# facebookresearch/unbiased-teacher-v2

Hardware: AMD Instinct MI355X
Metric: images/sec/node (labeled+unlabeled) UTv2 step, R50-FPN 1333x800 (higher is better)
Workload: dtype f16

## Files before the change

### include/utv2.h

```cpp
#ifndef UTV2_H
#define UTV2_H
#include <stdint.h>
#ifdef __cplusplus
extern "C" {
#endif

typedef struct ihipStream_t* utv2_stream_t;

int utv2_conv2d_nhwc_fwd(const float* x, const float* w, float* y, const float* scale, const float* bias,
                         const float* residual, int N, int H, int W, int C, int K, int KH, int KW, int stride, int pad,
                         int in_dil, int OH, int OW, int relu, int accumulate, int Kred, utv2_stream_t stream);
int utv2_conv2d_stem_fwd(const float* x, const float* w, void* y, int y_dtype, const float* scale, const float* bias, int N,
                         int H, int W, int K, int KH, int KW, int stride, int pad, int OH, int OW, int relu, int Kred,
                         utv2_stream_t stream);
int utv2_conv2d_wgrad_splits(int N, int OH, int OW, int K, int Kred);
int64_t utv2_conv2d_wgrad_workspace_floats(int N, int OH, int OW, int K, int Kred);
int utv2_conv2d_nhwc_wgrad(const float* x, const float* dy, float* dw, float* ws, int N, int H, int W, int C, int K,
                           int KH, int KW, int stride, int pad, int OH, int OW, int accumulate, utv2_stream_t stream);
int utv2_colsum(const float* g, float* db, float* ws, int M, int C, int accumulate, utv2_stream_t stream);
int utv2_weight_flip_transpose(const float* w, float* wt, int K, int KH, int KW, int C, utv2_stream_t stream);

int utv2_conv2d_ml_fwd(const float* x, const float* w, float* y, const float* scale, const float* bias,
                       const float* residual, int nlev, const int* H_host, const int* W_host, int N, int C, int K, int KH,
                       int KW, int pad, int relu, int accumulate, utv2_stream_t stream);
int utv2_conv2d_ml_wgrad(const float* x, const float* dy, float* dw, float* ws, int nlev, const int* H_host,
                         const int* W_host, int N, int C, int K, int KH, int KW, int pad, int accumulate,
                         utv2_stream_t stream);

#define UTV2_F32 0
#define UTV2_BF16 1
int utv2_conv2d_bf16_supported(int C, int KH, int KW);

int utv2_conv_clock_probe(double* ghz, double* lifetime_us);
int utv2_conv2d_nhwc_fwd_bf16(const void* x, int x_dtype, const void* w16, void* y, int y_dtype, const float* scale,
                              const float* bias, const void* residual, const void* mask, const void* post_mask, int N, int H, int W, int C, int K,
                              int KH, int KW, int stride, int pad, int in_dil, int OH, int OW, int relu, int accumulate,
                              utv2_stream_t stream);
int utv2_conv2d_nhwc_fwd_bf16_ri(const void* x, int x_dtype, const void* w16, void* y, int y_dtype, const float* scale,
                                 const float* bias, const void* residual, const void* mask, const void* post_mask, int N, int H, int W, int C,
                                 int K, int KH, int KW, int stride, int pad, int in_dil, int OH, int OW, int relu, int accumulate,
                                 const int* rowinfo, utv2_stream_t stream);
int utv2_conv2d_nhwc_fwd_bf16_bits(const void* x, int x_dtype, const void* w16, void* y, int y_dtype, const float* scale,
                                   const float* bias, const void* residual, const void* mask, const void* post_mask, int N, int H, int W,
                                   int C, int K, int KH, int KW, int stride, int pad, int in_dil, int OH, int OW, int relu, int accumulate,
                                   const int* rowinfo, void* relu_bits, const void* mask_bits, const void* post_mask_bits,
                                   utv2_stream_t stream);
int utv2_conv2d_ml_fwd_bf16(const void* x, int x_dtype, const void* w16, void* y, int y_dtype, const float* scale,
                            const float* bias, const void* residual, int nlev, const int* H_host, const int* W_host, int N,
                            int C, int K, int KH, int KW, int pad, int relu, int accumulate, utv2_stream_t stream);
int utv2_conv2d_ml_fwd_bf16_g(const void* x, int x_dtype, int x_pitch, const void* w16, void* y, int y_dtype, int y_pitch,
                              const float* scale, const float* bias, const void* residual, int nlev, const int* H_host,
                              const int* W_host, int N, int C, int K, int KH, int KW, int pad, int relu, int accumulate, int groups,
                              float* gn_part, const int* rowinfo, utv2_stream_t stream);
int utv2_conv2d_ml_fwd_bf16_gnb(const void* x, int x_pitch, const void* w16, void* y, int nlev, const int* H_host, const int* W_host, int N,
                                int C, int K, int KH, int KW, int pad, int groups, const int* rowinfo, const void* mask_bits,
                                const void* gnb_x, float* gnb_part, utv2_stream_t stream);
int utv2_conv2d_wgrad_bf16_splits(int M, int K, int Kred);
int64_t utv2_conv2d_wgrad_bf16_workspace_floats(int M, int K, int Kred);
int utv2_conv2d_wgrad_bf16(const void* x, int x_dtype, const void* dy, int dy_dtype, float* dw, float* db, float* ws,
                           const int* rowinfo, const float* rowscale, int M, int C, int K, int KH, int KW, int accumulate,
                           utv2_stream_t stream);
int utv2_conv2d_wgrad_bf16_g(const void* x, int x_dtype, int x_pitch, const void* dy, int dy_dtype, int dy_pitch, float* dw, float* db,
                             float* ws, const int* rowinfo, const float* rowscale, int M, int C, int K, int KH, int KW, int accumulate,
                             int groups, utv2_stream_t stream);
int utv2_conv2d_wgrad_bf16_d(const void* x, int x_dtype, int x_pitch, const void* dy, int dy_dtype, int dy_pitch, float* dw, float* db,
                             float* ws, const int* rowinfo, const float* rowscale, int M, int C, int K, int KH, int KW, int accumulate,
                             int groups, void* pending, utv2_stream_t stream);
int64_t utv2_wgrad_fold_table_bytes(void);
int utv2_wgrad_fold_pending(const void* pending);
int utv2_wgrad_fold_flush(void* pending, utv2_stream_t stream);
int utv2_conv2d_stem_fwd_bf16(const void* xpad16, const void* w16s, void* y, int y_dtype, const float* scale,
                              const float* bias, int N, int H, int W, int K, int OH, int OW, int relu, utv2_stream_t stream);
int utv2_rowinfo_nhwc(int* out, int N, int H, int W, int OH, int OW, int stride, int pad, int KH, int KW, int64_t start,
                      utv2_stream_t stream);
int utv2_f32_to_bf16(const float* src, void* dst16, int64_t n, utv2_stream_t stream);
int utv2_weight_flip_transpose_bf16(const float* w, void* wt16, const float* scale, int K, int KH, int KW, int C,
                                    utv2_stream_t stream);
int utv2_pad_cols_bf16(const void* src, int src_dtype, void* dst16, int64_t rows, int c, int cpad, utv2_stream_t stream);
int utv2_weight_flip_transpose_bf16_batched(const float* arena, const float* scales, void* bank, const void* table, int nlayers,
                                            utv2_stream_t stream);

int utv2_ema_axpby(float* teacher, const float* student, int64_t n, double keep_rate, utv2_stream_t stream);
int utv2_sgd_momentum(float* param, float* grad, float* mom_buf, int64_t n, float lr, float momentum, float weight_decay,
                      float grad_scale, int zero_grad, utv2_stream_t stream);
int utv2_amp_found_inf(const float* grad, int64_t n, float* state, utv2_stream_t stream);
int utv2_sgd_momentum_amp(float* param, const float* grad, float* mom_buf, int64_t n, float lr, float momentum, float weight_decay,
                          float grad_scale, const float* state, utv2_stream_t stream);
int utv2_amp_update_scale(float* state, float growth_factor, float backoff_factor, int growth_interval, utv2_stream_t stream);
int utv2_ema_axpby_m16(float* teacher, const float* student, void* mirror16, int64_t n, double keep_rate, utv2_stream_t stream);
int utv2_sgd_momentum_m16(float* param, float* grad, float* mom_buf, void* mirror16, int64_t n, float lr, float momentum, float weight_decay,
                          float grad_scale, int zero_grad, utv2_stream_t stream);
int utv2_sgd_momentum_amp_m16(float* param, const float* grad, float* mom_buf, void* mirror16, int64_t n, float lr, float momentum,
                              float weight_decay, float grad_scale, const float* state, utv2_stream_t stream);

int utv2_relu_bwd_scale(const void* dy, const void* y, const float* scale, void* out, int64_t M, int C, int dtype,
                        utv2_stream_t stream);
int utv2_add(const float* a, const float* b, float* out, int64_t n, utv2_stream_t stream);
int utv2_maxpool3x3s2_nhwc(const void* x, int x_dtype, void* y, int y_dtype, int N, int H, int W, int C, int OH, int OW,
                           utv2_stream_t stream);
int utv2_maxpool3x3s2_bwd_nhwc(const void* x, int x_dtype, const void* dpool, void* dx, int g_dtype, int N, int H, int W, int C, int OH,
                               int OW, int relu, utv2_stream_t stream);
int utv2_upsample2x_add_nhwc(const void* lateral, const void* top, void* out, int N, int H, int W, int C, int dtype,
                             utv2_stream_t stream);
int utv2_downsample2x_sum_nhwc(const void* g, void* dtop, int N, int TH, int TW, int C, int accumulate, int dtype,
                               utv2_stream_t stream);
int utv2_zero_interleave2x_nhwc(const void* src, const void* mask, void* dst, int N, int H, int W, int C, int dtype, utv2_stream_t stream);
int utv2_zero_interleave2x_add_nhwc(const void* src, const void* mask, const void* mask_bits, const void* add, void* dst, int N, int H, int W,
                                    int C, utv2_stream_t stream);
int utv2_preprocess_image(const void* src, int is_u8, float* dst, int H, int W, int Hp, int Wp,
                          const float* mean3_host, const float* std3_host, utv2_stream_t stream);
int utv2_preprocess_image_bf16pad(const void* src, int is_u8, void* dst16, int H, int W, int Hp, int Wp,
                                  const float* mean3_host, const float* std3_host, utv2_stream_t stream);
int utv2_preprocess_images_bf16pad(const void* const* src_host, int is_u8, void* dst16, const int* H_host, const int* W_host, int N,
                                   int Hp, int Wp, const float* mean3_host, const float* std3_host, utv2_stream_t stream);
int utv2_frozenbn_fold(const float* w, const float* b, const float* mean, const float* var, float* scale, float* shift,
                       int n, float eps, utv2_stream_t stream);
int64_t utv2_groupnorm_seg_workspace_floats(int nseg, const int* seg_rows_host, int C);
int utv2_groupnorm_relu_seg_fwd(const void* x, const float* gamma, const float* beta, void* y, float* mean, float* rstd,
                                float* ws, int nseg, const int* seg_rows_host, int C, int G, float eps, int relu, int dtype,
                                utv2_stream_t stream);
int utv2_groupnorm_relu_seg_fwd_p32(const void* x, const float* gamma, const float* beta, void* y, float* mean, float* rstd,
                                    const float* part32, int nseg, const int* seg_rows_host, int C, int G, float eps, int relu,
                                    utv2_stream_t stream);
int utv2_groupnorm_relu_seg_fwd_p32b(const void* x, const float* gamma, const float* beta, void* y, float* mean, float* rstd,
                                     const float* part32, int nseg, const int* seg_rows_host, int C, int G, float eps, int relu,
                                     void* relu_bits, utv2_stream_t stream);
int utv2_groupnorm_relu_seg_bwd(const void* dy, const void* y, const void* x, const float* mean, const float* rstd,
                                const float* gamma, const float* beta, void* dx, float* dgamma, float* dbeta, float* ws,
                                int nseg, const int* seg_rows_host, int C, int G, int relu, int dtype, utv2_stream_t stream);
int64_t utv2_groupnorm_seg_chunks(int nseg, const int* seg_rows_host);
int utv2_groupnorm_relu_seg_bwd_colsum(const void* dy, const void* y, const void* x, const float* mean, const float* rstd,
                                       const float* gamma, const float* beta, void* dx, float* dgamma, float* dbeta, float* ws,
                                       int nseg, const int* seg_rows_host, int C, int G, int relu, int dtype, float* colsum_part,
                                       utv2_stream_t stream);
int utv2_groupnorm_seg_bwd_p64(const void* g, const void* x, const float* mean, const float* rstd, const float* gamma, void* dx,
                               float* dgamma, float* dbeta, float* ws, int nseg, const int* seg_rows_host, int C, int G,
                               const float* part64, float* colsum_part, utv2_stream_t stream);
int utv2_colsum_partials(const float* partial, float* db, int nb, int K, int accumulate, utv2_stream_t stream);
int64_t utv2_groupnorm_workspace_floats(int N, int HW, int C);
int utv2_groupnorm_relu_fwd(const float* x, const float* gamma, const float* beta, float* y, float* mean, float* rstd,
                            float* ws, int N, int HW, int C, int G, float eps, int relu, utv2_stream_t stream);
int utv2_groupnorm_relu_bwd(const float* dy, const float* y, const float* x, const float* mean, const float* rstd,
                            const float* gamma, float* dx, float* dgamma, float* dbeta, float* ws, int N, int HW, int C,
                            int G, int relu, utv2_stream_t stream);

int utv2_fcos_targets(int num_levels, const int* H_host, const int* W_host, const int* strides_host,
                      const float* soi_host, int N, int MAXG, const float* gt_boxes, const int* gt_classes,
                      const unsigned char* gt_valid, const float* gt_std, int num_classes, int drop_empty,
                      float center_radius, const unsigned char* img_active, int* labels, float* reg_targets, float* bvars,
                      int* gt_inds, utv2_stream_t stream);
int utv2_fcos_targets_range(int num_levels, const int* H_host, const int* W_host, const int* strides_host, const float* soi_host, int N,
                            int MAXG, const float* gt_boxes, const int* gt_classes, const unsigned char* gt_valid, const float* gt_std,
                            int gt_img0, int gt_imgs, int num_classes, int drop_empty, float center_radius,
                            const unsigned char* img_active, int* labels, float* reg_targets, float* bvars, int* gt_inds,
                            utv2_stream_t stream);
int utv2_sigmoid_focal_fwd(const float* logits, const int* labels, int64_t P, int C, float alpha, float gamma,
                           float* loss_sum, float* ws, utv2_stream_t stream);
int utv2_sigmoid_focal_bwd(const float* logits, const int* labels, int64_t P, int C, float alpha, float gamma,
                           const float* coef, float* dlogits, utv2_stream_t stream);
int utv2_fcos_loc_terms_fwd(const int* labels, const float* box, int box_stride, const float* reg_targets,
                            const float* bvars, int64_t P, int num_classes, int reg_max, float ts_better, float ts_cert,
                            int flags, float* sums, float* ws, utv2_stream_t stream);
int utv2_fcos_loc_terms_bwd(const int* labels, const float* box, int box_stride, const float* reg_targets,
                            const float* bvars, int64_t P, int num_classes, int reg_max, float ts_better, float ts_cert,
                            int flags, const float* coef, float* dbox, utv2_stream_t stream);
int utv2_sigmoid_focal_bwd_acc(const float* logits, const int* labels, int64_t P, int C, float alpha, float gamma, const float* coef,
                               const float* gscale, float* dlogits, int accumulate, utv2_stream_t stream);
int utv2_fcos_loc_terms_bwd_acc(const int* labels, const float* box, int box_stride, const float* reg_targets, const float* bvars,
                                int64_t P, int num_classes, int reg_max, float ts_better, float ts_cert, int flags, const float* coef8,
                                const float* gscale, float* dbox, int accumulate, utv2_stream_t stream);
int utv2_fcos_loss_combine(const float* focal_sup, const float* sums_sup, const float* focal_cls, const float* sums_cls,
                           const float* sums_reg, const float* norm, float world, int flags, float kl_weight, const float* wmul_host,
                           const float* wdiv_host, float* rec, float* coef, utv2_stream_t stream);
int utv2_fcos_rank_keys(const float* logits, const float* box, int box_stride, int reg_max, int N, int HW, int C,
                        float thr, int method, long long* keys, int64_t key_row_stride, utv2_stream_t stream);
int64_t utv2_topk_rows_workspace_bytes(int rows, int k);
int utv2_topk_rows_i64(const long long* keys, const long long* row_off, int rows, int64_t max_width, int k, long long* out,
                       void* ws, utv2_stream_t stream);
int utv2_fcos_decode(const long long* topkeys, int K, const float* logits, const float* box, int box_stride, int reg_max,
                     int N, int HW, int Wl, int C, int stride, int level, int method, int MAXC, int slot0, float* oboxes,
                     float* oscores, int* ocls, float* oloc, float* octr, float* oconf, float* ostd, int* olevel,
                     unsigned char* ovalid, utv2_stream_t stream);
int utv2_scale_cols(float* y, int64_t rows, int row_stride, int ncols, const float* s, utv2_stream_t stream);
int utv2_scale_cols_bwd(float* g, const float* ypost, int64_t rows, int row_stride, int ncols, const float* s, float* dsum,
                        float* ws, utv2_stream_t stream);
int utv2_scale_cols_ml(float* y, int nlev, const int64_t* row0_host, int row_stride, int ncols, const float* const* s_host,
                       utv2_stream_t stream);
int utv2_scale_cols_bwd_ml(float* g, const float* ypost, int nlev, const int64_t* row0_host, int row_stride, int ncols,
                           const float* const* s_host, float* const* sgrad_host, float* ws, utv2_stream_t stream);
int utv2_scale_cols_bwd_ml_pad16(const float* g, const float* ypost, int nlev, const int64_t* row0_host, int row_stride, int ncols,
                                 const float* const* s_host, float* const* sgrad_host, float* ws, void* out16, int cpad, utv2_stream_t stream);

int utv2_nms_mpad(int M);
int64_t utv2_nms_workspace_bytes(int N, int M);
int utv2_nms_batched(const float* boxes, const float* scores, const int* cls, const unsigned char* valid, int N, int M,
                     float iou_thr, int class_aware, int post_topk, int max_out, int* keep, int* keep_count, void* ws,
                     utv2_stream_t stream);
int utv2_box_iou(const float* a, const float* b, int A, int B, float* out, utv2_stream_t stream);

int utv2_match_boxes(const float* boxes, int64_t box_img_stride, int N, int P, const float* gt_boxes,
                     const unsigned char* gt_valid, int G, float* max_iou, int* arg, unsigned* gt_max_bits,
                     utv2_stream_t stream);
int utv2_match_lowq(const float* boxes, int64_t box_img_stride, int N, int P, const float* gt_boxes,
                    const unsigned char* gt_valid, int G, const unsigned* gt_max_bits, unsigned char* lowq,
                    utv2_stream_t stream);
int utv2_roi_align_fwd(int num_levels, int min_level, const void* const* feats_host, const int* H_host,
                       const int* W_host, const float* scales_host, const float* rois, const int* roi_batch,
                       const unsigned char* roi_valid, int R, int C, int PH, int PW, void* out, int dtype,
                       utv2_stream_t stream);
int utv2_roi_align_bwd(int num_levels, int min_level, float* const* dfeats_host, const int* H_host, const int* W_host,
                       const float* scales_host, const float* rois, const int* roi_batch, const unsigned char* roi_valid,
                       int R, int C, int PH, int PW, const void* dy, int dtype, utv2_stream_t stream);
int utv2_roi_align_bwd_tiled(int num_levels, int min_level, void* const* dfeats_host, const int* H_host, const int* W_host,
                             const float* scales_host, const float* rois, const unsigned char* roi_valid, int N, int rois_per_image,
                             int C, int PH, int PW, const void* dy, int dy_dtype, int out_dtype, utv2_stream_t stream);
int utv2_rpn_rank_keys(const float* head, int num_levels, const int* hw_host, int N, int A, int ch, int64_t* keys, utv2_stream_t stream);
int utv2_rpn_decode(const int64_t* top, int maxk, const float* head, const float* anchors, const float* image_hw, int num_levels,
                    const int* hw_host, const int* k_host, int N, int A, int ch, const float* weights_host, float scale_clamp,
                    float min_size, float* boxes, float* scores, int* lvls, unsigned char* keep, utv2_stream_t stream);
int utv2_nms_pack(const int* kidx, const int* cnt, const float* boxes, const float* scores, int N, int M, int D, float* oboxes, float* oscores,
                  unsigned char* ovalid, utv2_stream_t stream);
int utv2_roi_infer_keys(const float* probs, const float* deltas, const float* prop, const unsigned char* valid, const float* whwh, int N, int P,
                        int K, float wx, float wy, float scale_clamp, float thr, float* boxes, int64_t* keys, utv2_stream_t stream);
int utv2_roi_infer_gather(const int64_t* top, const float* boxes, int N, int P, int K, int k, float thr, float* sc, int64_t* rows, int* cls,
                          float* cb, unsigned char* valid, utv2_stream_t stream);
int utv2_roi_infer_pack(const int* kidx, const int* cnt, const float* cb, const float* sc, const int* cls, const int64_t* rows, const float* stdl,
                        int N, int P, int k, int D, float* oboxes, float* oscores, int* ocls, float* ostd, int64_t* orows, unsigned char* ovalid,
                        utv2_stream_t stream);
int utv2_rpn_loss_fwd(const float* obj, const float* deltas, int head, int num_levels, const int* hw_host, int N, int A, int ch, int R,
                      const float* anchors, const int64_t* pos_idx, const unsigned char* pos_valid, int npos, const int64_t* neg_idx,
                      const unsigned char* neg_valid, int nneg, const int* matched, const unsigned char* has_gt, const float* gt_boxes,
                      const float* gt_scores, int G, const float* weights_host, float* sums, float* gobj, float* gdl, utv2_stream_t stream);
int utv2_rpn_loss_bwd(const float* gobj, const float* gdl, const float* gout_cls, const float* gout_loc, int head, int num_levels,
                      const int* hw_host, int N, int A, int ch, int R, const int64_t* pos_idx, const unsigned char* pos_valid, int npos,
                      const int64_t* neg_idx, const unsigned char* neg_valid, int nneg, float* grad_obj, float* grad_deltas,
                      utv2_stream_t stream);
int utv2_rpn_loss_fwd_range(const float* obj, const float* deltas, int head, int num_levels, const int* hw_host, int N, int batch, int img0,
                            int A, int ch, int R, const float* anchors, const int64_t* pos_idx, const unsigned char* pos_valid, int npos,
                            const int64_t* neg_idx, const unsigned char* neg_valid, int nneg, const int* matched,
                            const unsigned char* has_gt, const float* gt_boxes, const float* gt_scores, int G, const float* weights_host,
                            float* sums, float* gobj, float* gdl, utv2_stream_t stream);
int utv2_rpn_loss_bwd_range(const float* gobj, const float* gdl, const float* gout_cls, const float* gout_loc, int head, int num_levels,
                            const int* hw_host, int N, int batch, int img0, int A, int ch, int R, const int64_t* pos_idx,
                            const unsigned char* pos_valid, int npos, const int64_t* neg_idx, const unsigned char* neg_valid, int nneg,
                            float* grad_obj, float* grad_deltas, utv2_stream_t stream);
int utv2_rpn_sample_keys(const float* max_iou, const unsigned char* lowq, const unsigned char* gt_valid, int G, const float* keys, int N,
                         int R, float lo, float hi, int64_t* out, utv2_stream_t stream);
int utv2_rpn_sample_unpack(const int64_t* top, int k, int N, int npos_max, int nneg_max, const unsigned char* gt_valid, int G,
                           int64_t* pos_idx, unsigned char* pos_valid, int64_t* neg_idx, unsigned char* neg_valid, unsigned char* has_gt,
                           utv2_stream_t stream);
int utv2_roi_sample(const float* boxes, const unsigned char* valid, const float* max_iou, const int* argmax, const float* keys, int N, int P,
                    const float* gt_boxes, const int* gt_classes, const unsigned char* gt_valid, const float* gt_scores, const float* gt_std,
                    int G, float iou_thr, int num_classes, int batch, int nfg_max, float* out_boxes, int64_t* out_classes,
                    float* out_gt_boxes, unsigned char* out_valid, int64_t* out_idx, float* out_conf, float* out_std, utv2_stream_t stream);
int utv2_roi_box_loss(const float* deltas, const float* stdl, int64_t ld, const int64_t* cls, const float* prop, const float* gtb,
                      const float* gstd, int R, int num_classes, int mode, float wx, float wy, float scale_clamp, float ts_better,
                      float t_cert, float* sum, float* gdeltas, float* gstd_out, utv2_stream_t stream);
int utv2_softmax_focal_fwd(const float* logits, const int* target, int R, int C, float gamma, float* loss_sum, float* ws,
                           utv2_stream_t stream);
int utv2_softmax_focal_bwd(const float* logits, const int* target, int R, int C, float gamma, const float* coef,
                           float* dlogits, utv2_stream_t stream);
int utv2_rcnn_loss_combine(const float* rpn_sup, const float* rpn_uns, const float* focal_sup, const float* focal_uns, const float* box_sup,
                           const float* box_uns, const int* tgt_sup, int n_sup, const int* tgt_uns, int n_uns, float rpn_norm_sup,
                           float rpn_norm_uns, float w_rpn_cls, float w_rpn_loc, float w_box, const float* wt_host, float* rec, float* coef,
                           utv2_stream_t stream);

int utv2_stem_pool_fwd_bf16(const void* xpad16, const void* w16s, void* y, const float* scale, const float* shift, int N, int H, int W,
                            int K, utv2_stream_t stream);

int utv2_bottleneck_supported(int C, int MID, int has_shortcut);
int utv2_bottleneck_fwd_bf16(const void* x, void* y, const void* w1, const void* w2, const void* w3, const void* wsc, const float* s1,
                             const float* b1, const float* s2, const float* b2, const float* s3, const float* b3, const float* ssc,
                             const float* bsc, int N, int H, int W, int C, int MID, utv2_stream_t stream);

// ... 38 lines not shown
```

### unbiased-teacher-v2_amd/csrc/conv_bf16.hip

```cpp
#include <mutex>
#include <stdlib.h>
#include "common.h"
#include <type_traits>

__device__ uint4 g_zero64[4] = {{0, 0, 0, 0}, {0, 0, 0, 0}, {0, 0, 0, 0}, {0, 0, 0, 0}};

#define CONV_MAX_LEVELS 8
struct LevelTab {
  int n;
  int start[CONV_MAX_LEVELS + 1];
  int H[CONV_MAX_LEVELS], W[CONV_MAX_LEVELS];
};

struct ConvArgs16 {
  LevelTab lt;
  const void* x;
  const h16_t* w;
  void* y;
  const float* scale;
  const float* bias;
  const void* residual;
  const void* mask;
  const void* post_mask;
  int N, H, W, C, OH, OW, K, KH, KW, stride, pad, in_dil, relu, Kred, M, accumulate;
  int xs;
  int m_begin;
  int groups;
  int ldy;
  float* gn_part;
  int ntiles;
  EpiBits bits;
  int mtot;
  const int2* rowinfo;
};

__device__ __forceinline__ void ml_decode16(const LevelTab& lt, int m, int& pixbase, int& H, int& W, int& oh, int& ow) {
  int l = 0;
#pragma unroll
  for (int i = 1; i < CONV_MAX_LEVELS; ++i)
    if (i < lt.n && m >= lt.start[i]) l = i;
  H = lt.H[l];
  W = lt.W[l];
  const int r = m - lt.start[l], hw = H * W;
  const int n = r / hw, rem = r - n * hw;
  oh = rem / W;
  ow = rem - oh * W;
  pixbase = lt.start[l] + n * hw;
}

#ifndef UTV2_MFMA_PRIO
#define UTV2_MFMA_PRIO 0
#endif
#if UTV2_MFMA_PRIO && defined(UTV2_MFMA_PRIO_LOOSE)
#define MFMA_BURST_BEGIN __builtin_amdgcn_s_setprio(UTV2_MFMA_PRIO)
#define MFMA_BURST_END __builtin_amdgcn_s_setprio(0)
#elif UTV2_MFMA_PRIO
#define MFMA_BURST_BEGIN __builtin_amdgcn_s_setprio(UTV2_MFMA_PRIO); __builtin_amdgcn_sched_barrier(0)
#define MFMA_BURST_END __builtin_amdgcn_sched_barrier(0); __builtin_amdgcn_s_setprio(0)
#else
#define MFMA_BURST_BEGIN
#define MFMA_BURST_END
#endif

template <int BN, bool ML, typename TI, typename TO>
__global__ __launch_bounds__(256) void conv_igemm_bf16(ConvArgs16 p) {
  constexpr bool IN16 = sizeof(TI) == 2;
  constexpr int BM = 128, BK = 32, LDB = 80;
  constexpr int TM = 2, TN = BN / 64, BROWS = BN / 64;
  __shared__ __attribute__((aligned(16))) unsigned char smem[2 * (BM + BN) * LDB];
  unsigned char* As = smem;
  unsigned char* Bs = smem + 2 * BM * LDB;

  const int tid = threadIdx.x, lane = tid & 63, wid = tid >> 6;
  const int wm = wid >> 1, wn = wid & 1;
  const int tilesN = (p.K + BN - 1) / BN;
  const int nwg = gridDim.x;
  int tile;
  {
    const int bid = blockIdx.x, xcd = bid & 7, q = nwg >> 3, r = nwg & 7;
    tile = (xcd < r ? xcd * (q + 1) : r * (q + 1) + (xcd - r) * q) + (bid >> 3);
  }
  const int mt = tile / tilesN, nt = tile - mt * tilesN;
  const int m0 = mt * BM, n0 = nt * BN;
  const int lrow = tid >> 2, kg = tid & 3;

  int ih0[2], iw0[2], Hr[2], Wr[2];
  long long pixbase[2];
  bool mvalid[2];
#pragma unroll
  for (int r = 0; r < 2; ++r) {
    const int m = m0 + lrow + 64 * r;
    mvalid[r] = m < p.M;
    const int mm = mvalid[r] ? m : 0;
    if constexpr (ML) {
      int pb, oh, ow;
      ml_decode16(p.lt, mm, pb, Hr[r], Wr[r], oh, ow);
      ih0[r] = oh - p.pad;
      iw0[r] = ow - p.pad;
      pixbase[r] = pb;
    } else {
      const int hw = p.OH * p.OW;
      const int n = mm / hw, rem = mm - n * hw;
      const int oh = rem / p.OW, ow = rem - oh * p.OW;
      ih0[r] = oh * p.stride - p.pad;
      iw0[r] = ow * p.stride - p.pad;
      pixbase[r] = (long long)n * p.H * p.W;
      Hr[r] = p.H;
      Wr[r] = p.W;
    }
  }
  bool bvalid[BROWS];
  const h16_t* wrow[BROWS];
#pragma unroll
  for (int r = 0; r < BROWS; ++r) {
    const int co = n0 + lrow + 64 * r;
    bvalid[r] = co < p.K;
// ... 172 lines not shown
    *(bf16x8_t*)(dst + r * cpad + j) = o;
  }
}

__global__ void weight_flip_transpose_bf16_kernel(const float* __restrict__ w, h16_t* __restrict__ wt, const float* __restrict__ scale,
                                                  int K, int KH, int KW, int C) {
  const size_t n = (size_t)K * KH * KW * C;
  size_t i = (size_t)blockIdx.x * blockDim.x + threadIdx.x;
  const size_t stride = (size_t)gridDim.x * blockDim.x;
  for (; i < n; i += stride) {
    size_t t = i;
    const int co = (int)(t % K); t /= K;
    const int kwp = (int)(t % KW); t /= KW;
    const int khp = (int)(t % KH); t /= KH;
    const int ci = (int)t;
    float v = w[(((size_t)co * KH + (KH - 1 - khp)) * KW + (KW - 1 - kwp)) * C + ci];
    if (scale) v *= scale[co];
    wt[i] = (h16_t)v;
  }
}

struct FlipDesc {
  long long w_off;
  long long dst_off;
  long long scale_off;
  int K, KH, KW, C;
  int Kpad;
  int reserved;
};

__global__ __launch_bounds__(256) void weight_flip_transpose_bf16_batched_kernel(const float* __restrict__ arena, const float* __restrict__ scales,
                                                                               h16_t* __restrict__ bank, const FlipDesc* __restrict__ table) {
  __shared__ float tile[32][33];
  const FlipDesc d = table[blockIdx.y];
  const float* w = arena + d.w_off;
  const float* scale = d.scale_off >= 0 ? scales + d.scale_off : nullptr;
  h16_t* wt = bank + d.dst_off;
  const int T = d.KH * d.KW, tk = (d.Kpad + 31) / 32, tc = (d.C + 31) / 32;
  const int ntiles = T * tk * tc;
  const int tx = threadIdx.x & 31, ty = threadIdx.x >> 5;
  for (int t = blockIdx.x; t < ntiles; t += gridDim.x) {
    const int tap = t / (tk * tc), r = t - tap * (tk * tc);
    const int co0 = (r / tc) * 32, ci0 = (r - (r / tc) * tc) * 32;
    const int kh = tap / d.KW, kw = tap - kh * d.KW;
    const int ftap = (d.KH - 1 - kh) * d.KW + (d.KW - 1 - kw);
#pragma unroll
    for (int i = 0; i < 4; ++i) {
      const int co = co0 + ty + 8 * i, ci = ci0 + tx;
      float v = 0.f;
      if (co < d.K && ci < d.C) {
        v = w[((size_t)co * T + tap) * d.C + ci];
        if (scale) v *= scale[co];
      }
      tile[ty + 8 * i][tx] = v;
    }
    __syncthreads();
#pragma unroll
    for (int i = 0; i < 4; ++i) {
      const int ci = ci0 + ty + 8 * i, co = co0 + tx;
      if (ci < d.C && co < d.Kpad) wt[((size_t)ci * T + ftap) * d.Kpad + co] = (h16_t)tile[tx][ty + 8 * i];
    }
    __syncthreads();
  }
}

static int fill_levels16(LevelTab& lt, int nlev, int N, const int* H, const int* W) {
  lt.n = nlev;
  int off = 0;
  for (int l = 0; l < CONV_MAX_LEVELS; ++l) {
    lt.start[l] = off;
    if (l < nlev) {
      lt.H[l] = H[l];
      lt.W[l] = W[l];
      off += N * H[l] * W[l];
    } else {
      lt.H[l] = lt.W[l] = 1;
    }
  }
  lt.start[CONV_MAX_LEVELS] = off;
  return off;
}


template <int BN, bool ML, int BK, typename TO, bool TALL = false, bool GNB = false>
__global__ __launch_bounds__(256, TALL ? 3 : ((BK == 32 && BN != 96) ? 4 : 2)) void conv_igemm_bf16_v2(ConvArgs16 p) {
  static_assert(!TALL || BN == 64, "the tall layout exists for the 64-wide tile");
  constexpr int WN = (BN == 96 || TALL) ? 1 : 2, WM = 4 / WN, WCOLS = BN / WN;
  constexpr int BM = WM * 64, ROWB = BK * 2;
  constexpr int SLOTS = BK / 8, RPP = 256 / SLOTS;
  constexpr int TM = 2, TN = WCOLS / 32, AP = BM / RPP, BP = (BN + RPP - 1) / RPP, KS = BK / 16;
  constexpr int ABUF = BM * ROWB, BBUF = BP * RPP * ROWB;
  constexpr int PCOLS = WCOLS > 64 ? 64 : WCOLS;
  constexpr int STAGE = 2 * (ABUF + BBUF), PATCH = 4 * 32 * (PCOLS + 4) * 4;
  __shared__ __attribute__((aligned(16))) unsigned char smem[STAGE > PATCH ? STAGE : PATCH];
  unsigned char* As = smem;
  unsigned char* Bs = smem + 2 * ABUF;

  const int tid = threadIdx.x, lane = tid & 63, wid = tid >> 6;
  const int wm = wid / WN, wn = wid % WN;
  const int tilesN = (p.K + BN - 1) / BN;
  const int nwg = gridDim.x;
  int tile;
  {
    const int bid = blockIdx.x, xcd = bid & 7, q = nwg >> 3, r = nwg & 7;
    tile = (xcd < r ? xcd * (q + 1) : r * (q + 1) + (xcd - r) * q) + (bid >> 3);
  }
  const int mt = tile / tilesN, nt = tile - mt * tilesN;
  const int m0 = p.m_begin + mt * BM, n0 = nt * BN;
  const int lrow = tid / SLOTS, slot = tid % SLOTS;
  const int ntaps = p.KH * p.KW;
  const int goff = p.groups > 1 ? (n0 / (p.K / p.groups)) * p.C : 0;

  int aoff[AP], awc[AP];
  unsigned amask[AP];
#pragma unroll
  for (int j = 0; j < AP; ++j) {
    const int m = m0 + lrow + RPP * j;
    const bool mv = m < p.M;
    const int mm = mv ? m : 0;
    int pb, H, W, ih0, iw0;
    if (p.rowinfo) {
      const int2 ri = p.rowinfo[mm];
      aoff[j] = ri.x * p.xs + slot * 8 + goff;
      awc[j] = (ri.y >> 16) * p.xs;
      amask[j] = mv ? (unsigned)(ri.y & 0xffff) : 0u;
      continue;
    }
    if constexpr (ML) {
      int oh, ow;
      ml_decode16(p.lt, mm, pb, H, W, oh, ow);
      ih0 = oh - p.pad;
      iw0 = ow - p.pad;
    } else {
      if (p.KH * p.KW == 1 && p.stride == 1 && p.pad == 0) {
        aoff[j] = mm * p.xs + slot * 8 + goff;
        awc[j] = 0;
        amask[j] = mv ? 1u : 0u;
        continue;
      }
      const int hw = p.OH * p.OW;
      const int n = mm / hw, rem = mm - n * hw;
      const int oh = rem / p.OW, ow = rem - oh * p.OW;
      ih0 = oh * p.stride - p.pad;
      iw0 = ow * p.stride - p.pad;
      pb = n * p.H * p.W;
      H = p.H;
      W = p.W;
    }
    aoff[j] = (pb + ih0 * W + iw0) * p.xs + slot * 8 + goff;
    awc[j] = W * p.xs;
    unsigned mk = 0;
    for (int kh = 0; kh < p.KH; ++kh)
      for (int kw = 0; kw < p.KW; ++kw)
        if (mv && (unsigned)(ih0 + kh) < (unsigned)H && (unsigned)(iw0 + kw) < (unsigned)W) mk |= 1u << (kh * p.KW + kw);
    amask[j] = mk;
  }
  int boff[BP];
  bool bvalid[BP];
#pragma unroll
  for (int j = 0; j < BP; ++j) {
    const int co = n0 + lrow + RPP * j;
    bvalid[j] = co < p.K && lrow + RPP * j < BN;
    boff[j] = (bvalid[j] ? co : 0) * p.Kred + slot * 8;
  }

  f32x16 acc[TM][TN];
#pragma unroll
  for (int i = 0; i < TM; ++i)
#pragma unroll
    for (int j = 0; j < TN; ++j)
#pragma unroll
      for (int e = 0; e < 16; ++e) acc[i][j][e] = 0.f;

  const h16_t* __restrict__ xb = (const h16_t*)p.x;
  const int nchunks = ntaps * (p.C / BK);
  int kh = 0, kw = 0, c0 = 0, tap = 0;
  bf16x8_t ra[AP], rb[BP];

  constexpr int NP = AP + BP;
  int ua = 0, ub = 0, ukh = 0, utap = 0;
  auto cursor_next = [&]() {
    ua = kw * p.xs + c0;
    ub = tap * p.C + c0;
    ukh = kh;
    utap = tap;
    ++tap;
    if (++kw == p.KW) {
      kw = 0;
      if (++kh == p.KH) { kh = 0; tap = 0; c0 += BK; }
    }
  };
  const h16_t* zero = (const h16_t*)g_zero64;
  auto load_piece = [&](int q) {
    if (q < AP) {
      const h16_t* src = ((amask[q] >> utap) & 1u) ? xb + (unsigned)(aoff[q] + ukh * awc[q] + ua) : zero;
      ra[q] = *(const bf16x8_t*)src;
    } else {
      const h16_t* src = bvalid[q - AP] ? p.w + (unsigned)(boff[q - AP] + ub) : zero;
      rb[q - AP] = *(const bf16x8_t*)src;
    }
  };
  auto swizzle = [](int row) { return BK == 64 ? (row >> 1) & 7 : (row >> 2) & 3; };
  const int wslot = (slot ^ swizzle(lrow)) * 16;
  auto store_piece = [&](int buf, int q) {
    if (q < AP) *(bf16x8_t*)(As + buf * ABUF + (lrow + RPP * q) * ROWB + wslot) = ra[q];
    else *(bf16x8_t*)(Bs + buf * BBUF + (lrow + RPP * (q - AP)) * ROWB + wslot) = rb[q - AP];
  };

  const int frow = lane & 31, fh = lane >> 5;
  const int swz = swizzle(frow);
  int koff[KS];
#pragma unroll
  for (int s = 0; s < KS; ++s) koff[s] = ((2 * s + fh) ^ swz) * 16;
  const int arow = (wm * 64 + frow) * ROWB, brow = (wn * WCOLS + frow) * ROWB;

  cursor_next();
#pragma unroll
  for (int q = 0; q < NP; ++q) load_piece(q);
#pragma unroll
  for (int q = 0; q < NP; ++q) store_piece(0, q);
  if (nchunks > 1) {
    cursor_next();
#pragma unroll
    for (int q = 0; q < NP; ++q) load_piece(q);
  }
  __syncthreads();
  auto iteration = [&](int buf, auto do_store, auto do_load) {
    constexpr bool STORE = decltype(do_store)::value, LOAD = decltype(do_load)::value;
    if constexpr (LOAD) cursor_next();
    const unsigned char* ab = As + buf * ABUF + arow;
    const unsigned char* bb = Bs + buf * BBUF + brow;
#pragma unroll
    for (int s = 0; s < KS; ++s) {
      bf16x8_t a[TM], b[TN];
#pragma unroll
      for (int i = 0; i < TM; ++i) a[i] = *(const bf16x8_t*)(ab + i * 32 * ROWB + koff[s]);
#pragma unroll
      for (int j = 0; j < TN; ++j) b[j] = *(const bf16x8_t*)(bb + j * 32 * ROWB + koff[s]);
      MFMA_BURST_BEGIN;
#pragma unroll
      for (int i = 0; i < TM; ++i)
#pragma unroll
        for (int j = 0; j < TN; ++j) acc[i][j] = mfma_32x32x16(b[j], a[i], acc[i][j]);
      MFMA_BURST_END;
#pragma unroll
      for (int q = s * NP / KS; q < (s + 1) * NP / KS; ++q) {
        if constexpr (STORE) store_piece(buf ^ 1, q);
        if constexpr (LOAD) load_piece(q);
      }
      __builtin_amdgcn_sched_barrier(0);
    }
    __syncthreads();
  };
  using yes = std::integral_constant<bool, true>;
  using no = std::integral_constant<bool, false>;
  int kc = 0;
  for (; kc + 2 < nchunks; ++kc) iteration(kc & 1, yes{}, yes{});
  if (kc + 1 < nchunks) { iteration(kc & 1, yes{}, no{}); ++kc; }
  iteration(kc & 1, no{}, no{});

  if ((p.K & 3) == 0) {
    static_assert(sizeof(smem) >= 4 * 32 * (PCOLS + 4) * sizeof(float), "epilogue patches must fit the staging LDS");
    float* patch = (float*)smem + wid * (32 * (PCOLS + 4));
    if constexpr (TN == 3) {
      f32x16 lo[2][2], hi[2][1];
#pragma unroll
      for (int i = 0; i < 2; ++i) { lo[i][0] = acc[i][0]; lo[i][1] = acc[i][1]; hi[i][0] = acc[i][2]; }
      epilogue_rows<2, TO, true, true>(lo, patch, lane, (TO*)p.y, p.scale, p.bias, (const TO*)p.residual, p.relu, p.accumulate, m0 + wm * 64, n0,
                                 p.M, p.K, (const TO*)p.mask, (const TO*)p.post_mask, p.ldy, nullptr, p.bits);
      if (n0 + 64 < p.K)
        epilogue_rows<1, TO, true, true>(hi, patch, lane, (TO*)p.y, p.scale, p.bias, (const TO*)p.residual, p.relu, p.accumulate, m0 + wm * 64,
                                   n0 + 64, p.M, p.K, (const TO*)p.mask, (const TO*)p.post_mask, p.ldy, nullptr, p.bits);
    } else {
      epilogue_rows<TN, TO, (BK != 32), true, GNB>(acc, patch, lane, (TO*)p.y, p.scale, p.bias, (const TO*)p.residual, p.relu, p.accumulate,
                            m0 + wm * 64, n0 + wn * WCOLS, p.M, p.K, (const TO*)p.mask, (const TO*)p.post_mask, p.ldy, p.gn_part, p.bits);
    }
    return;
  }
  TO* yo = (TO*)p.y;
  const TO* res = (const TO*)p.residual;
  const TO* msk = (const TO*)p.mask;
#pragma unroll
  for (int j = 0; j < TN; ++j) {
#pragma unroll
    for (int i = 0; i < TM; ++i) {
#pragma unroll
      for (int e = 0; e < 16; ++e) {
        const int co = n0 + wn * WCOLS + j * 32 + (e & 3) + 8 * (e >> 2) + 4 * fh;
        if (co >= p.K) continue;
        const float sc = p.scale ? p.scale[co] : 1.f;
        const float bi = p.bias ? p.bias[co] : 0.f;
        const int m = m0 + wm * 64 + i * 32 + frow;
        if (m >= p.M) continue;
        const size_t off = (size_t)m * p.ldy + co;
        float v = acc[i][j][e] * sc + bi;
        if (msk) v = (float)msk[off] > 0.f ? v : 0.f;
        if (res) v += (float)res[off];
        if (p.post_mask) v = (float)((const TO*)p.post_mask)[off] > 0.f ? v : 0.f;
        if (p.relu & 1) v = fmaxf(v, 0.f);
        if (p.accumulate) v += (float)yo[off];
        yo[off] = (TO)v;
      }
    }
  }
}

typedef __attribute__((address_space(1))) const void* gptr_t;
typedef __attribute__((address_space(3))) void* lptr_t;

#ifdef UTV2_PP_TRACE
__device__ unsigned g_pp_trace[8 * 128];
__device__ unsigned long long g_pp_phase[2][5];
#define PP_STAMP                                                                                         \
  if (blockIdx.x == 0 && c >= 8 && c < 16) {                                                             \
    const unsigned t_ = (unsigned)__builtin_amdgcn_s_memtime();                                          \
    asm volatile("ds_write_b32 %0, %1" : : "v"(tr_addr + 4 * tn), "v"(t_) : "memory");                   \
    ++tn;                                                                                                \
  }
#else
#define PP_STAMP
#endif
#if defined(UTV2_PP_TRACE) && defined(PP_NO_DMA)
#define PP_DMA(cond) false
#else
#define PP_DMA(cond) (cond)
#endif
__device__ __attribute__((aligned(16))) unsigned long long g_pp_clock[2];
template <bool ML, typename TO>
__global__ __launch_bounds__(512) void conv_igemm_bf16_pp(ConvArgs16 p) {
#ifdef UTV2_PP_TRACE
  const unsigned long long ph_entry = __builtin_amdgcn_s_memtime();
#endif
  const bool clk_on = ML && blockIdx.x == 0 && p.ntiles > 0;
  unsigned long long clk_c0 = 0, clk_r0 = 0;
  if (clk_on) { clk_c0 = __builtin_amdgcn_s_memtime(); clk_r0 = __builtin_amdgcn_s_memrealtime(); }
  constexpr int BM = 256, BN = 256, BK = 64, SEGB = 64;
  constexpr int OPSEG = 256 * SEGB, OPB = 2 * OPSEG, STAGE = 2 * OPB;
  constexpr int TM = 4, TN = 2;
  constexpr int PATCH = 8 * 32 * (TN * 32 + 4) * 4;
  static_assert(2 * STAGE >= PATCH, "epilogue patches must fit the staging LDS");
  extern __shared__ __attribute__((aligned(16))) unsigned char smem[];

// ... 594 lines not shown
  if (clk_on && threadIdx.x == 0) {
    typedef unsigned long long u64x2 __attribute__((ext_vector_type(2)));
    const u64x2 v = {__builtin_amdgcn_s_memtime() - clk_c0, __builtin_amdgcn_s_memrealtime() - clk_r0};
    *(u64x2*)g_pp_clock = v;
  }
}

static bool env_flag_on(const char* name) {
  const char* v = getenv(name);
  return !(v && v[0] == '0');
}
static const bool g_use_w8 = env_flag_on("UTV2_W8");
static const bool g_use_wgrad_w8 = env_flag_on("UTV2_WGRAD_W8");
static int env_int(const char* name, int dflt) {
  const char* v = getenv(name);
  return v ? atoi(v) : dflt;
}
static const int g_epi_general = env_int("UTV2_EPI_PLAIN", 1) ? 0 : 2;
static const int g_use_pp = env_int("UTV2_PP", 2) == 1 ? 1 : 2;

template <int BN, bool ML>
static void launch_igemm16(const ConvArgs16& a, int tiles, int x_dtype, int y_dtype, hipStream_t stream) {
  const dim3 g(tiles), b(256);
  const int64_t xelems = ML ? (int64_t)a.M * a.xs : (int64_t)a.N * a.H * a.W * a.xs;
  if (x_dtype == UTV2_BF16 && a.C % 32 == 0 && a.in_dil == 1 && a.KH * a.KW <= 16 && xelems < (1ll << 31) &&
      (int64_t)a.K * a.Kred < (1ll << 31)) {
    const bool tail = tiles > 512 && tiles <= 768;
    const bool deep = a.C % 64 == 0 && a.Kred >= 1024 && (!tail || a.bits.gnb_part);
    static const bool use_rs = env_int("UTV2_PP_RS", 1) != 0;
    const bool rs_ok = use_rs && a.rowinfo && a.KH == 3 && a.KW == 3 && a.stride == 1 && a.pad == 1 && (ML || (a.OH == a.H && a.OW == a.W));
    const bool gnb = ML && BN == 128 && a.bits.gnb_part != nullptr;
    const bool w8 = g_use_w8 && (!gnb || rs_ok);
    if (w8 && BN == 128 && a.xs >= a.groups * a.C && (a.xs & 7) == 0 && a.C % 64 == 0 && a.Kred >= 1024 && a.K >= 256 && (a.K & 3) == 0 &&
        a.m_begin == 0 && (a.groups == 1 || (a.K / a.groups) % 256 == 0)) {
      const int tilesN = cdiv(a.K, 256), tiles_m = a.M / 256, tiles_all = cdiv(a.M, 256) * tilesN;
      int main_tiles = (tiles_m * tilesN / 256) * 256;
      if (tiles_all - main_tiles > 128) main_tiles = tiles_all;
      const int main_m = main_tiles == tiles_all ? cdiv(a.M, 256) : main_tiles / tilesN;
      if (main_m > 0) {
        ConvArgs16 m = a;
        m.M = main_tiles == tiles_all ? a.M : main_m * 256;
        const int smem = 2 * (256 + 256) * 128;
        static LdsOptIn lds_opt_in;
        lds_opt_in({(const void*)conv_igemm_bf16_pp<ML, h16_t>, (const void*)conv_igemm_bf16_pp<ML, float>}, smem);
        {
          int grid = main_m * tilesN;
          static const int pp_wgs = [] { int v = env_int("UTV2_PP_WGS", 256); return v < 8 ? 8 : (v > 256 ? 256 : v / 8 * 8); }();
          if (g_use_pp == 2 && grid > 256) { m.ntiles = grid; grid = pp_wgs; }
          if (rs_ok) {
            const int smem_rs = 4 * 272 * 64 + 4 * 256 * 64 + 256;
            static LdsOptIn rs_opt_in;
            rs_opt_in({(const void*)conv_igemm_bf16_rs<ML, h16_t>, (const void*)conv_igemm_bf16_rs<ML, float>,
                       (const void*)conv_igemm_bf16_rs<ML, h16_t, ML>}, smem_rs);
            m.mtot = a.M;
            if (gnb) hipLaunchKernelGGL((conv_igemm_bf16_rs<ML, h16_t, ML>), dim3(grid), dim3(512), smem_rs, stream, m);
            else if (y_dtype == UTV2_BF16) hipLaunchKernelGGL((conv_igemm_bf16_rs<ML, h16_t>), dim3(grid), dim3(512), smem_rs, stream, m);
            else hipLaunchKernelGGL((conv_igemm_bf16_rs<ML, float>), dim3(grid), dim3(512), smem_rs, stream, m);
          } else if (y_dtype == UTV2_BF16) hipLaunchKernelGGL((conv_igemm_bf16_pp<ML, h16_t>), dim3(grid), dim3(512), smem, stream, m);
          else hipLaunchKernelGGL((conv_igemm_bf16_pp<ML, float>), dim3(grid), dim3(512), smem, stream, m);
        }
        if (m.M == a.M) return;
        ConvArgs16 r = a;
        r.m_begin = m.M;
        launch_igemm16<BN, ML>(r, cdiv(a.M - m.M, 128) * cdiv(a.K, 128), x_dtype, y_dtype, stream);
        return;
      }
    }
    if constexpr (BN == 64) {
      static const bool use_tall = env_int("UTV2_CONV_TALL64", 1) != 0;
      if (use_tall && a.KH * a.KW > 1 && a.M - a.m_begin >= 65536 && a.K > 32) {
        const dim3 gt(cdiv(a.M - a.m_begin, 256) * cdiv(a.K, 64));
        if (y_dtype == UTV2_BF16) hipLaunchKernelGGL((conv_igemm_bf16_v2<64, ML, 32, h16_t, true>), gt, b, 0, stream, a);
        else hipLaunchKernelGGL((conv_igemm_bf16_v2<64, ML, 32, float, true>), gt, b, 0, stream, a);
        return;
      }
    }
    if constexpr (BN == 96) {
      if (y_dtype == UTV2_BF16) hipLaunchKernelGGL((conv_igemm_bf16_v2<96, ML, 32, h16_t>), g, b, 0, stream, a);
      else hipLaunchKernelGGL((conv_igemm_bf16_v2<96, ML, 32, float>), g, b, 0, stream, a);
    } else if (deep) {
      if (gnb) hipLaunchKernelGGL((conv_igemm_bf16_v2<BN, ML, 64, h16_t, false, (ML && BN == 128)>), g, b, 0, stream, a);
      else if (y_dtype == UTV2_BF16) hipLaunchKernelGGL((conv_igemm_bf16_v2<BN, ML, 64, h16_t>), g, b, 0, stream, a);
      else hipLaunchKernelGGL((conv_igemm_bf16_v2<BN, ML, 64, float>), g, b, 0, stream, a);
    } else {
      if (y_dtype == UTV2_BF16) hipLaunchKernelGGL((conv_igemm_bf16_v2<BN, ML, 32, h16_t>), g, b, 0, stream, a);
      else hipLaunchKernelGGL((conv_igemm_bf16_v2<BN, ML, 32, float>), g, b, 0, stream, a);
    }
    return;
  }
  if constexpr (BN != 96) {
    if (x_dtype == UTV2_BF16) {
      if (y_dtype == UTV2_BF16) hipLaunchKernelGGL((conv_igemm_bf16<BN, ML, h16_t, h16_t>), g, b, 0, stream, a);
      else hipLaunchKernelGGL((conv_igemm_bf16<BN, ML, h16_t, float>), g, b, 0, stream, a);
    } else {
      if (y_dtype == UTV2_BF16) hipLaunchKernelGGL((conv_igemm_bf16<BN, ML, float, h16_t>), g, b, 0, stream, a);
      else hipLaunchKernelGGL((conv_igemm_bf16<BN, ML, float, float>), g, b, 0, stream, a);
    }
  }
}

static const bool g_use_n96 = env_int("UTV2_CONV_N96", 1) != 0;
static bool n96_eligible(const ConvArgs16& a, int x_dtype) {
  return g_use_n96 && x_dtype == UTV2_BF16 && a.K > 64 && a.K <= 96 && (a.K & 3) == 0 && a.C % 32 == 0 && a.in_dil == 1 && a.KH * a.KW <= 16 &&
         a.groups == 1 && !a.gn_part && a.M >= 8192 && (int64_t)a.M * a.xs < (1ll << 31) && (int64_t)a.K * a.Kred < (1ll << 31);
}

static inline bool bad_dtype(int d) { return d != UTV2_F32 && d != UTV2_BF16; }

extern "C" {

int utv2_conv_clock_probe(double* ghz, double* lifetime_us) {
  if (!ghz || !lifetime_us) return UTV2_EARG;
  unsigned long long v[2] = {0, 0};
  hipError_t e = hipMemcpyFromSymbol(v, HIP_SYMBOL(g_pp_clock), sizeof(v));
  if (e != hipSuccess) return -(int)e;
  *ghz = v[1] ? (double)v[0] / (10.0 * (double)v[1]) : 0.0;
  *lifetime_us = (double)v[1] * 0.01;
  if (*ghz < 0.3 || *ghz > 2.6) { *ghz = 0.0; *lifetime_us = 0.0; }
  return UTV2_OK;
}

int utv2_conv2d_bf16_supported(int C, int KH, int KW) { return (C % 8 == 0) ? 1 : 0; }

int utv2_conv2d_nhwc_fwd_bf16_ri(const void* x, int x_dtype, const void* w16, void* y, int y_dtype, const float* scale,
                                 const float* bias, const void* residual, const void* mask, const void* post_mask, int N, int H, int W, int C,
                                 int K, int KH, int KW, int stride, int pad, int in_dil, int OH, int OW, int relu, int accumulate,
                                 const int* rowinfo, hipStream_t stream);

int utv2_conv2d_nhwc_fwd_bf16(const void* x, int x_dtype, const void* w16, void* y, int y_dtype, const float* scale,
                              const float* bias, const void* residual, const void* mask, const void* post_mask, int N, int H, int W, int C,
                              int K, int KH,
                              int KW, int stride, int pad, int in_dil, int OH, int OW, int relu, int accumulate, hipStream_t stream) {
  return utv2_conv2d_nhwc_fwd_bf16_ri(x, x_dtype, w16, y, y_dtype, scale, bias, residual, mask, post_mask, N, H, W, C, K, KH, KW, stride, pad,
                                      in_dil, OH, OW, relu, accumulate, nullptr, stream);
}

static int conv2d_nhwc_fwd_bf16_impl(const void* x, int x_dtype, const void* w16, void* y, int y_dtype, const float* scale,
                                     const float* bias, const void* residual, const void* mask, const void* post_mask, int N, int H, int W, int C,
                                     int K, int KH, int KW, int stride, int pad, int in_dil, int OH, int OW, int relu, int accumulate,
                                     const int* rowinfo, EpiBits bits, hipStream_t stream);

int utv2_conv2d_nhwc_fwd_bf16_ri(const void* x, int x_dtype, const void* w16, void* y, int y_dtype, const float* scale,
                                 const float* bias, const void* residual, const void* mask, const void* post_mask, int N, int H, int W, int C,
                                 int K, int KH, int KW, int stride, int pad, int in_dil, int OH, int OW, int relu, int accumulate,
                                 const int* rowinfo, hipStream_t stream) {
  return conv2d_nhwc_fwd_bf16_impl(x, x_dtype, w16, y, y_dtype, scale, bias, residual, mask, post_mask, N, H, W, C, K, KH, KW, stride, pad,
                                   in_dil, OH, OW, relu, accumulate, rowinfo, EpiBits{nullptr, nullptr, nullptr, nullptr, nullptr}, stream);
}

int utv2_conv2d_nhwc_fwd_bf16_bits(const void* x, int x_dtype, const void* w16, void* y, int y_dtype, const float* scale,
                                   const float* bias, const void* residual, const void* mask, const void* post_mask, int N, int H, int W,
                                   int C, int K, int KH, int KW, int stride, int pad, int in_dil, int OH, int OW, int relu, int accumulate,
                                   const int* rowinfo, void* relu_bits, const void* mask_bits, const void* post_mask_bits,
                                   hipStream_t stream) {
  if ((relu_bits || mask_bits || post_mask_bits) && (y_dtype != UTV2_BF16 || (K & 7))) return UTV2_EARG;
  if ((mask && mask_bits) || (post_mask && post_mask_bits)) return UTV2_EARG;
  return conv2d_nhwc_fwd_bf16_impl(x, x_dtype, w16, y, y_dtype, scale, bias, residual, mask, post_mask, N, H, W, C, K, KH, KW, stride, pad,
                                   in_dil, OH, OW, relu, accumulate, rowinfo,
                                   EpiBits{(unsigned char*)relu_bits, (const unsigned char*)mask_bits, (const unsigned char*)post_mask_bits, nullptr, nullptr},
                                   stream);
}

static int conv2d_nhwc_fwd_bf16_impl(const void* x, int x_dtype, const void* w16, void* y, int y_dtype, const float* scale,
                                     const float* bias, const void* residual, const void* mask, const void* post_mask, int N, int H, int W, int C,
                                     int K, int KH, int KW, int stride, int pad, int in_dil, int OH, int OW, int relu, int accumulate,
                                     const int* rowinfo, EpiBits bits, hipStream_t stream) {
  if (!x || !w16 || !y || (C % 8) || bad_dtype(x_dtype) || bad_dtype(y_dtype) || (rowinfo && in_dil > 1)) return UTV2_EARG;
  ConvArgs16 a;
  a.ntiles = 0;
  a.bits = bits;
  a.lt.n = 0;
  a.x = x; a.w = (const h16_t*)w16; a.y = y; a.scale = scale; a.bias = bias; a.residual = residual; a.mask = mask; a.post_mask = post_mask;
  a.N = N; a.H = H; a.W = W; a.C = C; a.OH = OH; a.OW = OW; a.K = K; a.KH = KH; a.KW = KW; a.stride = stride; a.pad = pad;
  a.in_dil = in_dil < 1 ? 1 : in_dil; a.relu = (relu ? 1 : 0) | g_epi_general; a.accumulate = accumulate; a.Kred = KH * KW * C; a.M = N * OH * OW;
  a.xs = C; a.m_begin = 0; a.groups = 1; a.ldy = K; a.gn_part = nullptr; a.rowinfo = (const int2*)rowinfo;
  const bool small = K <= 64;
  const int tiles = cdiv(a.M, 128) * cdiv(K, small ? 64 : 128);
  if (small) launch_igemm16<64, false>(a, tiles, x_dtype, y_dtype, stream);
  else launch_igemm16<128, false>(a, tiles, x_dtype, y_dtype, stream);
  return utv2_launch_status();
}

static int ml_fwd_g(const void* x, int x_dtype, int x_pitch, const void* w16, void* y, int y_dtype, int y_pitch, const float* scale,
                    const float* bias, const void* residual, int nlev, const int* H_host, const int* W_host, int N, int C, int K, int KH, int KW,
                    int pad, int relu, int accumulate, int groups, float* gn_part, const int* rowinfo, EpiBits bits, hipStream_t stream) {
  if (gn_part && (y_dtype != UTV2_BF16 || (K & 7) || (y_pitch & 7) || x_dtype != UTV2_BF16 || (C % 32) || accumulate)) return UTV2_EARG;
  if (!x || !w16 || !y || nlev < 1 || nlev > CONV_MAX_LEVELS || (C % 8) || N <= 0 || bad_dtype(x_dtype) || bad_dtype(y_dtype) || groups < 1 ||
      K % groups || x_pitch < groups * C || y_pitch < K)
    return UTV2_EARG;
  const bool plain = groups == 1 && x_pitch == C && y_pitch == K && !gn_part && !rowinfo && !bits.mask_bits;
  if (!plain && (x_dtype != UTV2_BF16 || (C % 32) || (K & 3) || KH * KW > 16 || (x_pitch & 7) || (y_pitch & 7) ||
                 (groups > 1 && (K / groups) % 128)))
    return UTV2_EARG;
  ConvArgs16 a;
  a.ntiles = 0;
  a.bits = bits;
  a.M = fill_levels16(a.lt, nlev, N, H_host, W_host);
  if (!plain && ((int64_t)a.M * x_pitch >= (1ll << 31) || (int64_t)K * KH * KW * C >= (1ll << 31))) return UTV2_EARG;
  a.x = x; a.w = (const h16_t*)w16; a.y = y; a.scale = scale; a.bias = bias; a.residual = residual; a.mask = nullptr; a.post_mask = nullptr;
  a.N = N; a.H = 0; a.W = 0; a.C = C; a.OH = 0; a.OW = 0; a.K = K; a.KH = KH; a.KW = KW; a.stride = 1; a.pad = pad; a.in_dil = 1;
  a.relu = (relu ? 1 : 0) | g_epi_general; a.accumulate = accumulate; a.Kred = KH * KW * C; a.xs = x_pitch; a.m_begin = 0; a.groups = groups; a.ldy = y_pitch; a.gn_part = gn_part; a.rowinfo = (const int2*)rowinfo;
  const bool small = K <= 64 && plain;
  const int tiles = cdiv(a.M, 128) * cdiv(K, small ? 64 : 128);
  if (n96_eligible(a, x_dtype)) launch_igemm16<96, true>(a, cdiv(a.M, 256), x_dtype, y_dtype, stream);
  else if (small) launch_igemm16<64, true>(a, tiles, x_dtype, y_dtype, stream);
  else launch_igemm16<128, true>(a, tiles, x_dtype, y_dtype, stream);
  return utv2_launch_status();
}

int utv2_conv2d_ml_fwd_bf16_g(const void* x, int x_dtype, int x_pitch, const void* w16, void* y, int y_dtype, int y_pitch,
                              const float* scale, const float* bias, const void* residual, int nlev, const int* H_host,
                              const int* W_host, int N, int C, int K, int KH, int KW, int pad, int relu, int accumulate, int groups,
                              float* gn_part, const int* rowinfo, hipStream_t stream) {
  return ml_fwd_g(x, x_dtype, x_pitch, w16, y, y_dtype, y_pitch, scale, bias, residual, nlev, H_host, W_host, N, C, K, KH, KW, pad, relu,
                  accumulate, groups, gn_part, rowinfo, EpiBits{nullptr, nullptr, nullptr, nullptr, nullptr}, stream);
}

int utv2_conv2d_ml_fwd_bf16_gnb(const void* x, int x_pitch, const void* w16, void* y, int nlev, const int* H_host, const int* W_host, int N,
                                int C, int K, int KH, int KW, int pad, int groups, const int* rowinfo, const void* mask_bits,
                                const void* gnb_x, float* gnb_part, hipStream_t stream) {
  if (!mask_bits || !gnb_x || !gnb_part || groups < 1 || K % groups || (C % 64) || KH * KW * C < 1024 || (K / groups) % 128 || (K & 7) ||
      g_epi_general)
    return UTV2_EARG;
  return ml_fwd_g(x, UTV2_BF16, x_pitch, w16, y, UTV2_BF16, K, nullptr, nullptr, nullptr, nlev, H_host, W_host, N, C, K, KH, KW, pad, 0, 0,
                  groups, nullptr, rowinfo, EpiBits{nullptr, (const unsigned char*)mask_bits, nullptr, gnb_x, gnb_part}, stream);
}

int utv2_conv2d_ml_fwd_bf16(const void* x, int x_dtype, const void* w16, void* y, int y_dtype, const float* scale,
                            const float* bias, const void* residual, int nlev, const int* H_host, const int* W_host, int N,
                            int C, int K, int KH, int KW, int pad, int relu, int accumulate, hipStream_t stream) {
  if (!x || !w16 || !y || nlev < 1 || nlev > CONV_MAX_LEVELS || (C % 8) || N <= 0 || bad_dtype(x_dtype) || bad_dtype(y_dtype))
    return UTV2_EARG;
  ConvArgs16 a;
  a.ntiles = 0;
  a.bits = EpiBits{nullptr, nullptr, nullptr, nullptr, nullptr};
  a.M = fill_levels16(a.lt, nlev, N, H_host, W_host);
  a.x = x; a.w = (const h16_t*)w16; a.y = y; a.scale = scale; a.bias = bias; a.residual = residual; a.mask = nullptr; a.post_mask = nullptr;
  a.N = N; a.H = 0; a.W = 0; a.C = C; a.OH = 0; a.OW = 0; a.K = K; a.KH = KH; a.KW = KW; a.stride = 1; a.pad = pad; a.in_dil = 1;
  a.relu = (relu ? 1 : 0) | g_epi_general; a.accumulate = accumulate; a.Kred = KH * KW * C; a.xs = C; a.m_begin = 0; a.groups = 1; a.ldy = K; a.gn_part = nullptr; a.rowinfo = nullptr;
  const bool small = K <= 64;
  const int tiles = cdiv(a.M, 128) * cdiv(K, small ? 64 : 128);
  if (n96_eligible(a, x_dtype)) launch_igemm16<96, true>(a, cdiv(a.M, 256), x_dtype, y_dtype, stream);
  else if (small) launch_igemm16<64, true>(a, tiles, x_dtype, y_dtype, stream);
  else launch_igemm16<128, true>(a, tiles, x_dtype, y_dtype, stream);
  return utv2_launch_status();
}

int utv2_conv2d_stem_fwd_bf16(const void* xpad16, const void* w16s, void* y, int y_dtype, const float* scale, const float* bias,
                              int N, int H, int W, int K, int OH, int OW, int relu, hipStream_t stream) {
  if (!xpad16 || !w16s || !y || N <= 0 || (W & 1) || (K & 3) || bad_dtype(y_dtype) || OH != (H + 6 - 7) / 2 + 1 ||
      OW != (W + 6 - 7) / 2 + 1 || (int64_t)N * (H + 6) * (W + 8) * 4 >= (1ll << 31))
    return UTV2_EARG;
  ConvArgs16 a;
  a.ntiles = 0;
  a.bits = EpiBits{nullptr, nullptr, nullptr, nullptr, nullptr};
  a.lt.n = 0;
  a.x = xpad16; a.w = (const h16_t*)w16s; a.y = y; a.scale = scale; a.bias = bias; a.residual = nullptr; a.mask = nullptr; a.post_mask = nullptr;
  a.N = N; a.H = H + 6; a.W = W + 8; a.C = 32; a.OH = OH; a.OW = OW; a.K = K; a.KH = 7; a.KW = 1; a.stride = 2; a.pad = 0;
  a.in_dil = 1; a.relu = (relu ? 1 : 0) | g_epi_general; a.accumulate = 0; a.Kred = 7 * 32; a.M = N * OH * OW; a.xs = 4; a.m_begin = 0; a.groups = 1; a.ldy = K; a.gn_part = nullptr; a.rowinfo = nullptr;
  const bool small = K <= 64;
  const int tiles = cdiv(a.M, 128) * cdiv(K, small ? 64 : 128);
  const dim3 g(tiles), b(256);
  static const bool use_tall = env_int("UTV2_CONV_TALL64", 1) != 0;
  if (small && use_tall && a.M >= 65536 && K > 32) {
    const dim3 gt(cdiv(a.M, 256));
    if (y_dtype == UTV2_BF16) hipLaunchKernelGGL((conv_igemm_bf16_v2<64, false, 32, h16_t, true>), gt, b, 0, stream, a);
    else hipLaunchKernelGGL((conv_igemm_bf16_v2<64, false, 32, float, true>), gt, b, 0, stream, a);
  } else if (small) {
    if (y_dtype == UTV2_BF16) hipLaunchKernelGGL((conv_igemm_bf16_v2<64, false, 32, h16_t>), g, b, 0, stream, a);
    else hipLaunchKernelGGL((conv_igemm_bf16_v2<64, false, 32, float>), g, b, 0, stream, a);
  } else {
    if (y_dtype == UTV2_BF16) hipLaunchKernelGGL((conv_igemm_bf16_v2<128, false, 32, h16_t>), g, b, 0, stream, a);
    else hipLaunchKernelGGL((conv_igemm_bf16_v2<128, false, 32, float>), g, b, 0, stream, a);
  }
  return utv2_launch_status();
}

__global__ __launch_bounds__(256) void rowinfo_kernel(int2* __restrict__ out, int N, int H, int W, int OH, int OW, int stride, int pad,
                                                      int KH, int KW, long long start) {
  const long long total = (long long)N * OH * OW;
  for (long long m = (long long)blockIdx.x * 256 + threadIdx.x; m < total; m += (long long)gridDim.x * 256) {
    const int ow = (int)(m % OW);
    const long long t = m / OW;
    const int oh = (int)(t % OH), n = (int)(t / OH);
    const int ih0 = oh * stride - pad, iw0 = ow * stride - pad;
    int mask = 0;
    for (int a = 0; a < KH; ++a)
      for (int b = 0; b < KW; ++b)
        if (ih0 + a >= 0 && ih0 + a < H && iw0 + b >= 0 && iw0 + b < W) mask |= 1 << (a * KW + b);
    out[m] = make_int2((int)(start + (long long)n * H * W + (long long)ih0 * W + iw0), (W << 16) | mask);
  }
}

int utv2_rowinfo_nhwc(int* out, int N, int H, int W, int OH, int OW, int stride, int pad, int KH, int KW, int64_t start,
                      hipStream_t stream) {
  if (!out || N < 1 || H < 1 || W < 1 || OH < 1 || OW < 1 || stride < 1 || pad < 0 || KH < 1 || KW < 1 || KH * KW > 16 || W >= 32768 ||
      start < 0 || start + (int64_t)N * H * W >= (1ll << 31))
    return UTV2_EARG;
  int64_t nb = ((int64_t)N * OH * OW + 255) / 256;
  if (nb > 8192) nb = 8192;
  hipLaunchKernelGGL(rowinfo_kernel, dim3((int)nb), dim3(256), 0, stream, (int2*)out, N, H, W, OH, OW, stride, pad, KH, KW, (long long)start);
  return utv2_launch_status();
}

int utv2_f32_to_bf16(const float* src, void* dst16, int64_t n, hipStream_t stream) {
  if (!src || !dst16 || (n & 3)) return UTV2_EARG;
  if (n == 0) return UTV2_OK;
  size_t nb = ((size_t)n / 4 + 255) / 256;
  if (nb > 4096) nb = 4096;
  hipLaunchKernelGGL(f32_to_bf16_kernel, dim3((int)nb), dim3(256), 0, stream, src, (h16_t*)dst16, (size_t)n / 4);
  return utv2_launch_status();
}

int utv2_pad_cols_bf16(const void* src, int src_dtype, void* dst16, int64_t rows, int c, int cpad, hipStream_t stream) {
  if (!src || !dst16 || rows < 0 || c < 8 || (c & 7) || (cpad & 7) || cpad < c || bad_dtype(src_dtype)) return UTV2_EARG;
  if (rows == 0) return UTV2_OK;
  size_t nb = ((size_t)rows * (cpad / 8) + 255) / 256;
  if (nb > 8192) nb = 8192;
  if (src_dtype == UTV2_BF16)
    hipLaunchKernelGGL(pad_cols_bf16_kernel<h16_t>, dim3((int)nb), dim3(256), 0, stream, (const h16_t*)src, (h16_t*)dst16, (size_t)rows, c, cpad);
  else
    hipLaunchKernelGGL(pad_cols_bf16_kernel<float>, dim3((int)nb), dim3(256), 0, stream, (const float*)src, (h16_t*)dst16, (size_t)rows, c, cpad);
  return utv2_launch_status();
}

int utv2_weight_flip_transpose_bf16(const float* w, void* wt16, const float* scale, int K, int KH, int KW, int C,
                                    hipStream_t stream) {
  if (!w || !wt16) return UTV2_EARG;
  const size_t n = (size_t)K * KH * KW * C;
  int nb = cdiv((int64_t)n, 256);
  if (nb > 8192) nb = 8192;
  hipLaunchKernelGGL(weight_flip_transpose_bf16_kernel, dim3(nb), dim3(256), 0, stream, w, (h16_t*)wt16, scale, K, KH, KW, C);
  return utv2_launch_status();
}

int utv2_weight_flip_transpose_bf16_batched(const float* arena, const float* scales, void* bank, const void* table, int nlayers,
                                            hipStream_t stream) {
  if (!arena || !bank || !table || nlayers < 1) return UTV2_EARG;
  static_assert(sizeof(FlipDesc) == 48, "table record layout is part of the ABI");
  hipLaunchKernelGGL(weight_flip_transpose_bf16_batched_kernel, dim3(512, nlayers), dim3(256), 0, stream, arena, scales, (h16_t*)bank,
                     (const FlipDesc*)table);
  return utv2_launch_status();
}

}

struct Wgrad16Args {
  const void* x;
  const void* dy;
  float* ws;
  const int2* rowinfo;
  float* bias_ws;
  int C, K, KH, KW, Kred, M, splits, chunks_per_split;
  int xs;
  int groups;
  int dys;
  int debug;
};

__device__ __forceinline__ bf16x4_t lds_read_tr16(const unsigned char* p) {
  typedef short s16x4 __attribute__((ext_vector_type(4)));
  const s16x4 v = __builtin_amdgcn_ds_read_tr16_b64_v4i16((__attribute__((address_space(3))) s16x4*)p);
  return __builtin_bit_cast(bf16x4_t, v);
}

template <typename TX, typename TDY>
__global__ __launch_bounds__(256) void conv_wgrad_bf16(Wgrad16Args p) {
  constexpr int BK = 32, LDR = 320;
  constexpr int OPB = BK * LDR;
  constexpr bool X16 = sizeof(TX) == 2, DY16 = sizeof(TDY) == 2;
  __shared__ __attribute__((aligned(16))) unsigned char smem[2 * 2 * OPB];
  const int tid = threadIdx.x, lane = tid & 63, wid = tid >> 6;
  const int wm = wid >> 1, wn = wid & 1;
  const int tilesN = (p.Kred + 127) / 128, tilesM = (p.K + 127) / 128;
  const int tiles = tilesM * tilesN;
  int split, bid;
  if ((p.splits & 7) == 0) {
    const int xcd = blockIdx.x & 7, idx = blockIdx.x >> 3;
    split = xcd + 8 * (idx / tiles);
    bid = idx % tiles;
  } else {
    split = blockIdx.x / tiles;
    bid = blockIdx.x - split * tiles;
  }
  const int mt = bid / tilesN, nt = bid - mt * tilesN;
  const int i0 = mt * 128, j0 = nt * 128;
  const int goff = p.groups > 1 ? (i0 / (p.K / p.groups)) * p.C : 0;

  const int cg = tid & 15, pl0 = tid >> 4;
  const int co8 = i0 + cg * 8;
  const bool aok = co8 < p.K;
  const int kk = j0 + cg * 8;
  const bool bok = kk < p.Kred;
  const int tap = bok ? kk / p.C : 0;
  const int ci = bok ? kk - tap * p.C : 0;
  const int dh = tap / p.KW, dw = tap - dh * p.KW;

  f32x16 acc[2][2];
#pragma unroll
  for (int i = 0; i < 2; ++i)
#pragma unroll
    for (int j = 0; j < 2; ++j)
#pragma unroll
      for (int e = 0; e < 16; ++e) acc[i][j][e] = 0.f;

  const int chunk_begin = split * p.chunks_per_split;
  const int total_chunks = (p.M + BK - 1) / BK;
  int chunk_end = chunk_begin + p.chunks_per_split;
  if (chunk_end > total_chunks) chunk_end = total_chunks;

  int2 ri[2];
  bf16x8_t ra[2], rb[2];
  float bsum[8];
#pragma unroll
  for (int e = 0; e < 8; ++e) bsum[e] = 0.f;
  const bool do_bias = p.bias_ws != nullptr && nt == 0;

  auto rload = [&](int chunk) {
#pragma unroll
    for (int r = 0; r < 2; ++r) {
      int m = chunk * BK + pl0 + 16 * r;
      m = m < p.M ? m : p.M - 1;
      ri[r] = p.rowinfo[m];
    }
  };
  auto load8 = [&](const void* base, size_t eoff, bool is16, bool ok) -> bf16x8_t {
    bf16x8_t v;
    if (is16) {
      const h16_t* src = ok ? (const h16_t*)base + eoff : (const h16_t*)g_zero64;
      v = *(const bf16x8_t*)src;
    } else {
      const float* src = ok ? (const float*)base + eoff : (const float*)g_zero64;
      const f32x4 v0 = *(const f32x4*)src, v1 = *(const f32x4*)(src + 4);
#pragma unroll
      for (int e = 0; e < 4; ++e) {
        v[e] = (h16_t)v0[e];
        v[4 + e] = (h16_t)v1[e];
      }
    }
    return v;
  };
  auto load_piece = [&](int chunk, int q) {
    const int r = q & 1;
    const int m = chunk * BK + pl0 + 16 * r;
    const bool mok = m < p.M;
    if (q < 2) {
      ra[r] = load8(p.dy, (size_t)m * p.dys + co8, DY16, mok && aok);
    } else {
      const int W = ri[r].y >> 16;
      const bool ok = mok && bok && ((ri[r].y >> tap) & 1);
      rb[r] = load8(p.x, (size_t)(ri[r].x + dh * W + dw) * p.xs + goff + ci, X16, ok);
    }
  };
  auto store_piece = [&](int buf, int q) {
    const int r = q & 1;
    unsigned char* dst = smem + buf * 2 * OPB + (q < 2 ? 0 : OPB) + (pl0 + 16 * r) * LDR + cg * 16;
    if (q < 2) {
      *(bf16x8_t*)dst = ra[r];
      if (do_bias) {
#pragma unroll
        for (int e = 0; e < 8; ++e) bsum[e] += (float)ra[r][e];
      }
    } else {
      *(bf16x8_t*)dst = rb[r];
    }
  };

  const int G = lane >> 4, t = lane & 15;
  const int frag_off = (8 * (G >> 1) + (t >> 2)) * LDR + (16 * (G & 1) + 4 * (t & 3)) * 2;
  auto iteration = [&](int ch, int buf, auto do_store, auto do_load) {
    constexpr bool STORE = decltype(do_store)::value, LOAD = decltype(do_load)::value;
    const unsigned char* ab = smem + buf * 2 * OPB + frag_off;
    const unsigned char* bb = ab + OPB;
#pragma unroll
    for (int s = 0; s < 2; ++s) {
      bf16x8_t a[2], b[2];
#pragma unroll
      for (int i = 0; i < 2; ++i) {
        const unsigned char* ap = ab + s * 16 * LDR + (wm * 64 + i * 32) * 2;
        const bf16x4_t a0 = lds_read_tr16(ap), a1 = lds_read_tr16(ap + 4 * LDR);
        const unsigned char* bp = bb + s * 16 * LDR + (wn * 64 + i * 32) * 2;
        const bf16x4_t b0 = lds_read_tr16(bp), b1 = lds_read_tr16(bp + 4 * LDR);
#pragma unroll
        for (int e = 0; e < 4; ++e) {
          a[i][e] = a0[e]; a[i][4 + e] = a1[e];
          b[i][e] = b0[e]; b[i][4 + e] = b1[e];
        }
      }
      MFMA_BURST_BEGIN;
#pragma unroll
      for (int i = 0; i < 2; ++i)
#pragma unroll
        for (int j = 0; j < 2; ++j) acc[i][j] = mfma_32x32x16(a[i], b[j], acc[i][j]);
      MFMA_BURST_END;
#pragma unroll
      for (int q = (s == 0 ? 2 : 0); q < (s == 0 ? 4 : 2); ++q) {
        if constexpr (STORE) store_piece(buf ^ 1, q);
        if constexpr (LOAD) load_piece(ch + 2, q);
      }
      if constexpr (LOAD) {
        if (s == 0) rload(ch + 3);
      }
      __builtin_amdgcn_sched_barrier(0);
    }
    __syncthreads();
  };
  using yes = std::integral_constant<bool, true>;
  using no = std::integral_constant<bool, false>;
  if (chunk_begin < chunk_end) {
    rload(chunk_begin);
#pragma unroll
    for (int q = 0; q < 4; ++q) load_piece(chunk_begin, q);
    rload(chunk_begin + 1);
#pragma unroll
    for (int q = 0; q < 4; ++q) store_piece(0, q);
    if (chunk_begin + 1 < chunk_end) {
#pragma unroll
      for (int q = 0; q < 4; ++q) load_piece(chunk_begin + 1, q);
      rload(chunk_begin + 2);
    }
    __syncthreads();
    int ch = chunk_begin;
    for (; ch + 2 < chunk_end; ++ch) iteration(ch, (ch - chunk_begin) & 1, yes{}, yes{});
    if (ch + 1 < chunk_end) { iteration(ch, (ch - chunk_begin) & 1, yes{}, no{}); ++ch; }
    iteration(ch, (ch - chunk_begin) & 1, no{}, no{});
  }
  if (p.bias_ws != nullptr && nt == 0) {
    float* red = (float*)smem;
#pragma unroll
    for (int e = 0; e < 8; ++e) red[tid * 8 + e] = bsum[e];
    __syncthreads();
    if (tid < 128 && i0 + tid < p.K) {
      float s = 0.f;
      for (int k = 0; k < 16; ++k) s += red[(k * 16 + (tid >> 3)) * 8 + (tid & 7)];
      p.bias_ws[(size_t)split * p.K + i0 + tid] = s;
    }
    __syncthreads();
  }

  const int frow = lane & 31, fh = lane >> 5;
  float* out = p.ws + (size_t)split * p.K * p.Kred;
#pragma unroll
  for (int j = 0; j < 2; ++j) {
    const int k = j0 + wn * 64 + j * 32 + frow;
    if (k >= p.Kred) continue;
#pragma unroll
    for (int i = 0; i < 2; ++i)
#pragma unroll
      for (int e = 0; e < 16; ++e) {
        const int co = i0 + wm * 64 + i * 32 + (e & 3) + 8 * (e >> 2) + 4 * fh;
        if (co < p.K) out[(size_t)co * p.Kred + k] = acc[i][j][e];
      }
  }
}

#define WGRAD_W8_BP 64
__global__ __launch_bounds__(512) void conv_wgrad_bf16_pp(Wgrad16Args p) {
  constexpr int BP = 32, ROWB = 512, OPB = BP * ROWB, STAGE = 2 * OPB;
  extern __shared__ __attribute__((aligned(16))) unsigned char smem[];
  const int tid = threadIdx.x, lane = tid & 63;
  const int wid = __builtin_amdgcn_readfirstlane(tid >> 6);
  const int wm = wid >> 2, wn = wid & 3;
  const int tilesN = p.Kred >> 8, tiles = (p.K >> 8) * tilesN;
  const int per = gridDim.x >> 3;
  const int wi = (blockIdx.x & 7) * per + (blockIdx.x >> 3);
  if (wi >= tiles * p.splits) return;
  const int split = wi / tiles, bid = wi - split * tiles;
  const int mt = bid / tilesN, nt = bid - mt * tilesN;
  const int i0 = mt << 8, j0 = nt << 8;
  const int tap = j0 / p.C, ci0 = j0 - tap * p.C + (p.groups > 1 ? (i0 / (p.K / p.groups)) * p.C : 0);
  const int dh = tap / p.KW, dw = tap - dh * p.KW;

  f32x16 acc[4][2];
#pragma unroll
  for (int i = 0; i < 4; ++i)
#pragma unroll
    for (int j = 0; j < 2; ++j)
#pragma unroll
      for (int e = 0; e < 16; ++e) acc[i][j][e] = 0.f;

  const int total_chunks = (p.M + BP - 1) / BP;
  const int chunk_begin = split * p.chunks_per_split * 2;
  int chunk_end = chunk_begin + p.chunks_per_split * 2;
  if (chunk_end > total_chunks) chunk_end = total_chunks;
  const int nslots = chunk_end - chunk_begin;
  if (nslots <= 0) {
    const int frow0 = lane & 31, fh0 = lane >> 5;
    float* out0 = p.ws + (size_t)split * p.K * p.Kred;
    for (int j = 0; j < 2; ++j)
      for (int i = 0; i < 4; ++i)
        for (int e = 0; e < 16; ++e)
          out0[(size_t)(i0 + wm * 128 + i * 32 + (e & 3) + 8 * (e >> 2) + 4 * fh0) * p.Kred + j0 + wn * 64 + j * 32 + frow0] = 0.f;
    return;
  }

  const int hr = lane >> 5, slot = lane & 31;
  int choff[2];
#pragma unroll
  for (int o = 0; o < 2; ++o) choff[o] = (((slot >> 2) ^ ((2 * o + hr) & 3)) << 5) + ((slot & 3) << 3);
  const h16_t* __restrict__ xb = (const h16_t*)p.x;
  const h16_t* __restrict__ dyb = (const h16_t*)p.dy;
  const h16_t* zero = (const h16_t*)g_zero64;
  typedef int i32x2 __attribute__((ext_vector_type(2)));
  i32x2 ri[2][2];
  const int rowl = 4 * wid + hr;
#define WGP_RLOAD(SET)                                                                             \
  [&](int chunk) {                                                                                 \
    _Pragma("unroll") for (int q = 0; q < 2; ++q) {                                                \
// ... 332 lines not shown
      if (f.rowscale) v *= f.rowscale[c];
      f.dst[c] = f.accumulate ? f.dst[c] + v : v;
    }
  }
}

static int slab_fold_add(SlabFoldTable* t, int kind, const float* ws, float* dst, const float* rowscale, size_t n, int splits, int accumulate,
                         int rowlen) {
  if (t->count < 0 || t->count >= SLAB_FOLD_MAX) return UTV2_EARG;
  for (int i = 0; i < t->count; ++i)
    if (t->e[i].dst == dst) return UTV2_EARG;
  SlabFold& f = t->e[t->count];
  f.kind = kind; f.ws = ws; f.dst = dst; f.rowscale = rowscale; f.n = n; f.splits = splits; f.accumulate = accumulate; f.rowlen = rowlen;
  int nb;
  if (kind == 0) { nb = cdiv((int64_t)n / 4, 256); if (nb > 2048) nb = 2048; }
  else if (kind == 1) nb = cdiv((int64_t)n, 256);
  else nb = cdiv((int64_t)n, 32);
  if (nb < 1) nb = 1;
  f.blk0 = t->count == 0 ? 0 : t->e[t->count - 1].blk0 + t->e[t->count - 1].nblk;
  f.nblk = nb;
  t->total_blocks = f.blk0 + nb;
  ++t->count;
  return UTV2_OK;
}

extern "C" {

static int wgrad16_small_splits(int M, int K, int Kred) {
  const int chunks = cdiv(M, 32);
  const int tiles = cdiv(K, 128) * cdiv(Kred, 128);
  const double flop = 2.0 * M * K * Kred;
  int splits = cdiv(flop > 512 * 2.0e8 ? 1024 : 512, tiles);
  const int max_by_chunks = chunks / 8 > 0 ? chunks / 8 : 1;
  if (splits > max_by_chunks) splits = max_by_chunks;
  if (splits < 1) splits = 1;
  if (splits > 256) splits = 256;
  if (splits >= 8) splits = (splits + 7) / 8 * 8 <= max_by_chunks ? (splits + 7) / 8 * 8 : splits / 8 * 8;
  return splits;
}

#define WGRAD_W8_MAX_NB 1024
static int wgrad16_w8_budget() {
  static const int w = [] {
    int v = env_int("UTV2_WGRAD_W8_WGS", 256);
    v = (v / 8) * 8;
    return v < 8 ? 8 : (v > 256 ? 256 : v);
  }();
  return w;
}
static int wgrad16_w8_splits(int M, int K, int Kred) {
  const int tiles = (K >> 8) * (Kred >> 8), chunks = cdiv(M, WGRAD_W8_BP);
  int splits = wgrad16_w8_budget() / tiles;
  if (splits > chunks / 8) splits = chunks / 8;
  return splits < 1 ? 1 : splits;
}
static bool wgrad16_w8_shape_ok(int M, int C, int K, int KH, int KW, int xs, int groups) {
  const int Kred = KH * KW * C, tiles = (K >> 8) * (Kred >> 8), chunks = cdiv(M, WGRAD_W8_BP);
  if ((K & 255) || (C & 255) || KH * KW > 16 || K > 2048 || tiles > wgrad16_w8_budget() || chunks < 16 || (int64_t)M * K >= (1ll << 31) ||
      (int64_t)M * xs >= (1ll << 31) || (xs & 7) || ((K / groups) & 255))
    return false;
  if (KH * KW == 1 && chunks < 16 * (256 / tiles)) return false;
  return true;
}

int utv2_conv2d_wgrad_bf16_splits(int M, int K, int Kred) { return wgrad16_small_splits(M, K, Kred); }

int utv2_colsum_partials(const float* partial, float* db, int nb, int K, int accumulate, hipStream_t stream) {
  if (!partial || !db || nb < 1 || K < 1) return UTV2_EARG;
  hipLaunchKernelGGL(colsum_final_f32, dim3(cdiv(K, 32)), dim3(256), 0, stream, partial, db, nb, K, accumulate, (const float*)nullptr);
  return utv2_launch_status();
}

int64_t utv2_conv2d_wgrad_bf16_workspace_floats(int M, int K, int Kred) {
  int64_t n = (int64_t)wgrad16_small_splits(M, K, Kred) * ((int64_t)K * Kred + K);
  if ((K & 255) == 0 && (Kred & 255) == 0) {
    const int64_t n8 = (int64_t)wgrad16_w8_splits(M, K, Kred) * K * Kred + (int64_t)WGRAD_W8_MAX_NB * K;
    if (n8 > n) n = n8;
  }
  return n;
}

static int wgrad_bf16_impl(const void* x, int x_dtype, int x_pitch, const void* dy, int dy_dtype, int dy_pitch, float* dw, float* db,
                           float* ws, const int* rowinfo, const float* rowscale, int M, int C, int K, int KH, int KW, int accumulate,
                           int groups, hipStream_t stream, SlabFoldTable* pending = nullptr);

int utv2_conv2d_wgrad_bf16(const void* x, int x_dtype, const void* dy, int dy_dtype, float* dw, float* db, float* ws,
                           const int* rowinfo, const float* rowscale, int M, int C, int K, int KH, int KW, int accumulate,
                           hipStream_t stream) {
  return wgrad_bf16_impl(x, x_dtype, C, dy, dy_dtype, K, dw, db, ws, rowinfo, rowscale, M, C, K, KH, KW, accumulate, 1, stream);
}

int utv2_conv2d_wgrad_bf16_g(const void* x, int x_dtype, int x_pitch, const void* dy, int dy_dtype, int dy_pitch, float* dw, float* db,
                             float* ws, const int* rowinfo, const float* rowscale, int M, int C, int K, int KH, int KW, int accumulate,
                             int groups, hipStream_t stream) {
  return wgrad_bf16_impl(x, x_dtype, x_pitch, dy, dy_dtype, dy_pitch, dw, db, ws, rowinfo, rowscale, M, C, K, KH, KW, accumulate, groups,
                         stream);
}

int utv2_conv2d_wgrad_bf16_d(const void* x, int x_dtype, int x_pitch, const void* dy, int dy_dtype, int dy_pitch, float* dw, float* db,
                             float* ws, const int* rowinfo, const float* rowscale, int M, int C, int K, int KH, int KW, int accumulate,
                             int groups, void* pending, hipStream_t stream) {
  if (!pending) return UTV2_EARG;
  SlabFoldTable* t = (SlabFoldTable*)pending;
  if (t->count < 0 || t->count + 3 > SLAB_FOLD_MAX) return UTV2_EARG;
  return wgrad_bf16_impl(x, x_dtype, x_pitch, dy, dy_dtype, dy_pitch, dw, db, ws, rowinfo, rowscale, M, C, K, KH, KW, accumulate, groups,
                         stream, t);
}

int64_t utv2_wgrad_fold_table_bytes(void) { return (int64_t)sizeof(SlabFoldTable); }

int utv2_wgrad_fold_pending(const void* pending) { return pending ? ((const SlabFoldTable*)pending)->count : -1; }

int utv2_wgrad_fold_flush(void* pending, hipStream_t stream) {
  if (!pending) return UTV2_EARG;
  SlabFoldTable* t = (SlabFoldTable*)pending;
  if (t->count < 0 || t->count > SLAB_FOLD_MAX) return UTV2_EARG;
  if (t->count == 0) return UTV2_OK;
  hipLaunchKernelGGL(reduce_slabs_table, dim3(t->total_blocks), dim3(256), 0, stream, *t);
  t->count = 0;
  t->total_blocks = 0;
  return utv2_launch_status();
}

static int wgrad_bf16_impl(const void* x, int x_dtype, int x_pitch, const void* dy, int dy_dtype, int dy_pitch, float* dw, float* db,
                           float* ws, const int* rowinfo, const float* rowscale, int M, int C, int K, int KH, int KW, int accumulate,
                           int groups, hipStream_t stream, SlabFoldTable* pending) {
  if (!x || !dy || !dw || !ws || !rowinfo || (C & 7) || (K & 7) || M <= 0 || KH * KW > 16 || bad_dtype(x_dtype) ||
      bad_dtype(dy_dtype) || groups < 1 || K % groups || x_pitch < groups * C || (groups > 1 && (K / groups) % 128) ||
      (x_pitch != C && (x_pitch & (x_dtype == UTV2_BF16 ? 7 : 3))) || dy_pitch < K || (dy_pitch != K && (dy_pitch & (dy_dtype == UTV2_BF16 ? 7 : 3))))
    return UTV2_EARG;
  Wgrad16Args a;
  a.x = x; a.dy = dy; a.ws = ws; a.rowinfo = (const int2*)rowinfo;
  a.C = C; a.K = K; a.KH = KH; a.KW = KW; a.Kred = KH * KW * C; a.M = M; a.debug = 0; a.xs = x_pitch; a.groups = groups; a.dys = dy_pitch;
  if (g_use_wgrad_w8 && x_dtype == UTV2_BF16 && dy_dtype == UTV2_BF16 && dy_pitch == K && wgrad16_w8_shape_ok(M, C, K, KH, KW, x_pitch, groups)) {
    a.splits = wgrad16_w8_splits(M, K, a.Kred);
    a.chunks_per_split = cdiv(cdiv(M, WGRAD_W8_BP), a.splits);
    a.bias_ws = nullptr;
    const size_t n = (size_t)K * a.Kred;
    const int smem = 2 * 2 * WGRAD_W8_BP * 512;
    static LdsOptIn pp_opt_in;
    pp_opt_in({(const void*)conv_wgrad_bf16_pp}, smem);
    hipLaunchKernelGGL(conv_wgrad_bf16_pp, dim3(wgrad16_w8_budget()), dim3(512), smem, stream, a);
    int rb = cdiv((int64_t)n / 4, 256);
    if (rb > 8192) rb = 8192;
    if (pending) {
      if (int rc = slab_fold_add(pending, 0, ws, dw, rowscale, n, a.splits, accumulate, a.Kred)) return rc;
    } else
      hipLaunchKernelGGL(reduce_slabs16_f32, dim3(rb), dim3(256), 0, stream, (const float*)ws, dw, n, a.splits, accumulate, rowscale,
                         a.Kred);
    if (db) {
      float* part = ws + (size_t)a.splits * n;
      int nb = cdiv(M, 64);
      if (nb > WGRAD_W8_MAX_NB) nb = WGRAD_W8_MAX_NB;
      const int rows = cdiv(M, nb);
      nb = cdiv(M, rows);
      hipLaunchKernelGGL(colsum_bf16_partial, dim3(nb), dim3(256), 0, stream, (const h16_t*)dy, part, M, K, rows);
      if (pending) {
        if (int rc = slab_fold_add(pending, 2, part, db, rowscale, (size_t)K, nb, accumulate, 1)) return rc;
      } else
        hipLaunchKernelGGL(colsum_final_f32, dim3(cdiv(K, 32)), dim3(256), 0, stream, (const float*)part, db, nb, K, accumulate, rowscale);
    }
    return utv2_launch_status();
  }
  a.splits = utv2_conv2d_wgrad_bf16_splits(M, K, a.Kred);
  a.chunks_per_split = cdiv(cdiv(M, 32), a.splits);
  const size_t n = (size_t)K * a.Kred;
  a.bias_ws = db ? ws + (size_t)a.splits * n : nullptr;
  const int tiles = cdiv(K, 128) * cdiv(a.Kred, 128);
  const dim3 g(tiles * a.splits), b(256);
  if (x_dtype == UTV2_BF16) {
    if (dy_dtype == UTV2_BF16) hipLaunchKernelGGL((conv_wgrad_bf16<h16_t, h16_t>), g, b, 0, stream, a);
    else hipLaunchKernelGGL((conv_wgrad_bf16<h16_t, float>), g, b, 0, stream, a);
  } else {
    if (dy_dtype == UTV2_BF16) hipLaunchKernelGGL((conv_wgrad_bf16<float, h16_t>), g, b, 0, stream, a);
    else hipLaunchKernelGGL((conv_wgrad_bf16<float, float>), g, b, 0, stream, a);
  }
  int rb = cdiv((int64_t)n / 4, 256);
  if (rb > 8192) rb = 8192;
  if (pending) {
    if (int rc = slab_fold_add(pending, 0, ws, dw, rowscale, n, a.splits, accumulate, a.Kred)) return rc;
    if (db)
      if (int rc = slab_fold_add(pending, 1, a.bias_ws, db, rowscale, (size_t)K, a.splits, accumulate, 1)) return rc;
    return utv2_launch_status();
  }
  hipLaunchKernelGGL(reduce_slabs16_f32, dim3(rb), dim3(256), 0, stream, (const float*)ws, dw, n, a.splits, accumulate, rowscale,
                       a.Kred);
  if (db)
    hipLaunchKernelGGL(reduce_slabs16_scalar_f32, dim3(cdiv(K, 256)), dim3(256), 0, stream, (const float*)a.bias_ws, db, (size_t)K,
                       a.splits, accumulate, rowscale);
  return utv2_launch_status();
}

}
```

### unbiased-teacher-v2_amd/csrc/fcos.hip

```cpp
#include "common.h"

#define MAX_LEVELS 8

struct LevelTable {
  int num_levels;
  int H[MAX_LEVELS], W[MAX_LEVELS], stride[MAX_LEVELS];
  int off[MAX_LEVELS + 1];
  float soi_lo[MAX_LEVELS], soi_hi[MAX_LEVELS];
};

__device__ __forceinline__ int level_of(const LevelTable& t, int loc) {
  int l = 0;
#pragma unroll
  for (int i = 1; i < MAX_LEVELS; ++i)
    if (i < t.num_levels && loc >= t.off[i]) l = i;
  return l;
}

#define TG_MAXG 256
__global__ __launch_bounds__(256) void fcos_targets_kernel(LevelTable lt, int N, int MAXG, const float* __restrict__ gt_boxes,
                                                         const int* __restrict__ gt_classes,
                                                         const unsigned char* __restrict__ gt_valid,
                                                         const float* __restrict__ gt_std, int num_classes, int drop_empty,
                                                         float center_radius, const unsigned char* __restrict__ img_active,
// ... 529 lines not shown
  size_t i = (size_t)blockIdx.x * blockDim.x + threadIdx.x;
  const size_t stride = (size_t)gridDim.x * blockDim.x;
  const float k = s[0];
  for (; i < total; i += stride) {
    const size_t r = i / ncols;
    const int c = (int)(i - r * ncols);
    y[r * BS + c] *= k;
  }
}

__global__ __launch_bounds__(256) void scale_cols_bwd_kernel(float* __restrict__ g, const float* __restrict__ ypost, size_t rows, int BS,
                                                           int ncols, const float* __restrict__ s, float* __restrict__ partial) {
  __shared__ float red[4];
  const size_t total = rows * (size_t)ncols;
  size_t i = (size_t)blockIdx.x * blockDim.x + threadIdx.x;
  const size_t stride = (size_t)gridDim.x * blockDim.x;
  const float k = s[0];
  float acc = 0.f;
  for (; i < total; i += stride) {
    const size_t r = i / ncols;
    const int c = (int)(i - r * ncols);
    const float gv = g[r * BS + c];
    acc += gv * ypost[r * BS + c];
    g[r * BS + c] = gv * k;
  }
  const float t = block_reduce_sum(acc, red);
  if (threadIdx.x == 0) partial[blockIdx.x] = t;
}

#define SC_MAXL 8
struct ScaleLevels {
  long long row0[SC_MAXL + 1];
  const float* s[SC_MAXL];
  float* sgrad[SC_MAXL];
  int nlev;
};

__global__ __launch_bounds__(256) void scale_cols_ml_kernel(float* __restrict__ y, ScaleLevels L, int BS, int ncols) {
  const int l = blockIdx.y;
  float* yl = y + (size_t)L.row0[l] * BS;
  const size_t total = (size_t)(L.row0[l + 1] - L.row0[l]) * (size_t)ncols;
  const float k = L.s[l][0];
  for (size_t i = (size_t)blockIdx.x * blockDim.x + threadIdx.x; i < total; i += (size_t)gridDim.x * blockDim.x) {
    const size_t r = i / ncols;
    const int c = (int)(i - r * ncols);
    yl[r * BS + c] *= k;
  }
}

template <bool VEC4>
__global__ __launch_bounds__(256) void scale_cols_bwd_ml_kernel(float* __restrict__ g, const float* __restrict__ ypost, ScaleLevels L, int BS,
                                                              int ncols, float* __restrict__ partial) {
  __shared__ float red[4];
  const int l = blockIdx.y;
  float* gl = g + (size_t)L.row0[l] * BS;
  const float* yl = ypost + (size_t)L.row0[l] * BS;
  const float k = L.s[l][0];
  float acc = 0.f;
  if constexpr (VEC4) {
    const unsigned q = (unsigned)BS >> 2, qn = (unsigned)ncols >> 2;
    const unsigned total = (unsigned)(L.row0[l + 1] - L.row0[l]) * q;
    for (unsigned i = blockIdx.x * blockDim.x + threadIdx.x; i < total; i += gridDim.x * blockDim.x) {
      if (i % q >= qn) continue;
      f32x4 gv = *(const f32x4*)(gl + (size_t)i * 4);
      const f32x4 yv = *(const f32x4*)(yl + (size_t)i * 4);
      acc += ((gv[0] * yv[0] + gv[1] * yv[1]) + (gv[2] * yv[2] + gv[3] * yv[3]));
      gv[0] *= k; gv[1] *= k; gv[2] *= k; gv[3] *= k;
      *(f32x4*)(gl + (size_t)i * 4) = gv;
    }
  } else {
    const size_t total = (size_t)(L.row0[l + 1] - L.row0[l]) * (size_t)ncols;
    for (size_t i = (size_t)blockIdx.x * blockDim.x + threadIdx.x; i < total; i += (size_t)gridDim.x * blockDim.x) {
      const size_t r = i / ncols;
      const int c = (int)(i - r * ncols);
      const float gv = gl[r * BS + c];
      acc += gv * yl[r * BS + c];
      gl[r * BS + c] = gv * k;
    }
  }
  const float t = block_reduce_sum(acc, red);
  if (threadIdx.x == 0) partial[(size_t)l * gridDim.x + blockIdx.x] = t;
}

__global__ __launch_bounds__(256) void scale_cols_bwd_ml_pad16_kernel(const float* __restrict__ g, const float* __restrict__ ypost, ScaleLevels L,
                                                                    int BS, int ncols, float* __restrict__ partial, h16_t* __restrict__ out,
                                                                    int cpad) {
  __shared__ float red[4];
  const int l = blockIdx.y;
  const float* gl = g + (size_t)L.row0[l] * BS;
  const float* yl = ypost + (size_t)L.row0[l] * BS;
  h16_t* ol = out + (size_t)L.row0[l] * cpad;
  const float k = L.s[l][0];
  float acc = 0.f;
  const unsigned q = (unsigned)BS >> 2, qn = (unsigned)ncols >> 2, qp = (unsigned)cpad >> 2;
  const unsigned total = (unsigned)(L.row0[l + 1] - L.row0[l]) * qp;
  typedef h16_t h16x4 __attribute__((ext_vector_type(4)));
  for (unsigned i = blockIdx.x * blockDim.x + threadIdx.x; i < total; i += gridDim.x * blockDim.x) {
    const unsigned r = i / qp, c4 = i - r * qp;
    f32x4 gv = {0.f, 0.f, 0.f, 0.f};
    if (c4 < q) {
      gv = *(const f32x4*)(gl + ((size_t)r * q + c4) * 4);
      if (c4 < qn) {
        const f32x4 yv = *(const f32x4*)(yl + ((size_t)r * q + c4) * 4);
        acc += ((gv[0] * yv[0] + gv[1] * yv[1]) + (gv[2] * yv[2] + gv[3] * yv[3]));
        gv[0] *= k; gv[1] *= k; gv[2] *= k; gv[3] *= k;
      }
    }
    h16x4 o = {(h16_t)gv[0], (h16_t)gv[1], (h16_t)gv[2], (h16_t)gv[3]};
    *(h16x4*)(ol + (size_t)i * 4) = o;
  }
  const float t = block_reduce_sum(acc, red);
  if (threadIdx.x == 0) partial[(size_t)l * gridDim.x + blockIdx.x] = t;
}

__global__ __launch_bounds__(256) void scale_cols_bwd_ml_final(ScaleLevels L, const float* __restrict__ partial, int nb) {
  __shared__ float red[4];
  const int l = blockIdx.x;
  float acc = 0.f;
  for (int i = threadIdx.x; i < nb; i += blockDim.x) acc += partial[(size_t)l * nb + i];
  const float t = block_reduce_sum(acc, red);
  if (threadIdx.x == 0) L.sgrad[l][0] += t / L.s[l][0];
}

static LevelTable make_table(int num_levels, const int* H, const int* W, const int* strides, const float* soi) {
  LevelTable t;
  t.num_levels = num_levels;
  int off = 0;
  for (int l = 0; l < MAX_LEVELS; ++l) {
    if (l < num_levels) {
      t.H[l] = H[l]; t.W[l] = W[l]; t.stride[l] = strides[l];
      t.soi_lo[l] = soi ? soi[2 * l] : 0.f; t.soi_hi[l] = soi ? soi[2 * l + 1] : 0.f;
      t.off[l] = off;
      off += H[l] * W[l];
    } else {
      t.H[l] = t.W[l] = t.stride[l] = 0; t.soi_lo[l] = t.soi_hi[l] = 0.f; t.off[l] = off;
    }
  }
  t.off[num_levels] = off;
  for (int l = num_levels + 1; l <= MAX_LEVELS; ++l) t.off[l] = off;
  return t;
}

struct FcosCombineArgs {
  const float* focal_sup;
  const float* sums_sup;
  const float* focal_cls;
  const float* sums_cls;
  const float* sums_reg;
  const float* norm;
  float world, kl_weight;
  int flags;
  float wmul[6], wdiv[6];
};

__global__ void fcos_loss_combine_kernel(FcosCombineArgs a, float* __restrict__ rec, float* __restrict__ coef) {
  if (threadIdx.x != 0 || blockIdx.x != 0) return;
  for (int i = 0; i < 26; ++i) coef[i] = 0.f;
  const bool kl = a.flags & 1, kl4 = a.flags & 2, unify = a.flags & 4, tsb = a.flags & 8;
  float g[6];
  for (int k = 0; k < 6; ++k) g[k] = a.wmul[k] / a.wdiv[k];
  const float* S = a.sums_sup;
  const float npa_s = fmaxf((a.norm ? a.norm[0] : S[0]) / a.world, 1.f), den_s = fmaxf((a.norm ? a.norm[1] : S[1]) / a.world, 1e-6f);
  const float cls = a.focal_sup[0] / npa_s, ctr = S[2] / npa_s;
  float loc = S[3] / den_s;
  coef[0] = g[0] / npa_s;
  coef[1 + 2] = g[2] / npa_s;
  coef[1 + 3] = g[1] / den_s;
  if (kl) {
    const float n = fmaxf(S[0], 1.f), dn = kl4 ? 4.f * n : n, w = a.kl_weight;
    loc = w * (w * (S[4] / dn)) + loc;
    coef[1 + 4] = g[1] * (w * w) / dn;
  }
  const float* C = a.sums_cls;
  const float npa_c = fmaxf((a.norm ? a.norm[2] : C[0]) / a.world, 1.f);
  const float cls_p = a.focal_cls[0] / npa_c;
  float ctr_p = C[2] / npa_c;
  coef[9] = g[3] / npa_c;
  if (unify) ctr_p = ctr_p * 0.f;
  else coef[10 + 2] = g[4] / npa_c;
  const float* R = a.sums_reg;
  float loc_p, tbs = 0.f;
  if (tsb) {
    const float d = fmaxf(R[5], 1.f);
    loc_p = R[6] / d;
    tbs = R[5];
    coef[18 + 6] = g[5] / d;
  } else {
    const float n = fmaxf(R[0], 1.f), dn = kl4 ? 4.f * n : n;
    loc_p = a.kl_weight * (R[4] / dn);
    coef[18 + 4] = g[5] * a.kl_weight / dn;
  }
  rec[0] = cls; rec[1] = loc; rec[2] = ctr; rec[3] = cls_p; rec[4] = ctr_p; rec[5] = loc_p; rec[6] = tbs;
// ... 86 lines not shown
}

int utv2_fcos_rank_keys(const float* logits, const float* box, int box_stride, int reg_max, int N, int HW, int C, float thr,
                        int method, long long* keys, int64_t key_row_stride, hipStream_t stream) {
  if (!logits || !box || !keys || method < 0 || method > 3 || key_row_stride < (int64_t)HW * C) return UTV2_EARG;
  int gx = cdiv((int64_t)HW * C, 256);
  if (gx > 4096) gx = 4096;
  hipLaunchKernelGGL(fcos_rank_keys_kernel, dim3(gx, N), dim3(256), 0, stream, logits, box, box_stride, 4 * (reg_max + 1), HW, C,
                     thr, method, keys, (size_t)key_row_stride);
  return utv2_launch_status();
}

int utv2_fcos_decode(const long long* topkeys, int K, const float* logits, const float* box, int box_stride, int reg_max,
                     int N, int HW, int Wl, int C, int stride, int level, int method, int MAXC, int slot0, float* oboxes,
                     float* oscores, int* ocls, float* oloc, float* octr, float* oconf, float* ostd, int* olevel,
                     unsigned char* ovalid, hipStream_t stream) {
  if (!topkeys || !logits || !box || reg_max != 16 || slot0 + K > MAXC) return UTV2_EARG;
  hipLaunchKernelGGL((fcos_decode_kernel<17>), dim3(cdiv(K, 128), N), dim3(128), 0, stream, topkeys, K, logits, box, box_stride,
                     HW, Wl, C, stride, level, method, MAXC, slot0, oboxes, oscores, ocls, oloc, octr, oconf, ostd, olevel,
                     ovalid);
  return utv2_launch_status();
}

int utv2_scale_cols(float* y, int64_t rows, int row_stride, int ncols, const float* s, hipStream_t stream) {
  if (!y || !s) return UTV2_EARG;
  int g = cdiv(rows * ncols, 256);
  if (g > 4096) g = 4096;
  hipLaunchKernelGGL(scale_cols_kernel, dim3(g), dim3(256), 0, stream, y, (size_t)rows, row_stride, ncols, s);
  return utv2_launch_status();
}

int utv2_scale_cols_bwd(float* g, const float* ypost, int64_t rows, int row_stride, int ncols, const float* s, float* dsum,
                        float* ws, hipStream_t stream) {
  if (!g || !ypost || !s || !dsum || !ws) return UTV2_EARG;
  int nb = cdiv(rows * ncols, 256);
  if (nb > 1024) nb = 1024;
  hipLaunchKernelGGL(scale_cols_bwd_kernel, dim3(nb), dim3(256), 0, stream, g, ypost, (size_t)rows, row_stride, ncols, s, ws);
  hipLaunchKernelGGL(sum_partials_kernel, dim3(1), dim3(256), 0, stream, (const float*)ws, nb, 1, dsum);
  return utv2_launch_status();
}

static int fill_scale_levels(ScaleLevels& L, int nlev, const int64_t* row0_host, const float* const* s_host, float* const* sgrad_host) {
  if (nlev < 1 || nlev > SC_MAXL || !row0_host || !s_host) return UTV2_EARG;
  L.nlev = nlev;
  for (int l = 0; l <= SC_MAXL; ++l) L.row0[l] = row0_host[l <= nlev ? l : nlev];
  for (int l = 0; l < SC_MAXL; ++l) {
    L.s[l] = l < nlev ? s_host[l] : nullptr;
    L.sgrad[l] = (l < nlev && sgrad_host) ? sgrad_host[l] : nullptr;
    if (l < nlev && (!L.s[l] || L.row0[l + 1] < L.row0[l])) return UTV2_EARG;
  }
  return UTV2_OK;
}

int utv2_scale_cols_ml(float* y, int nlev, const int64_t* row0_host, int row_stride, int ncols, const float* const* s_host,
                       hipStream_t stream) {
  ScaleLevels L;
  if (!y || fill_scale_levels(L, nlev, row0_host, s_host, nullptr) != UTV2_OK) return UTV2_EARG;
  int64_t most = 0;
  for (int l = 0; l < nlev; ++l) most = L.row0[l + 1] - L.row0[l] > most ? L.row0[l + 1] - L.row0[l] : most;
  int gx = cdiv(most * ncols, 256 * 4);
  if (gx > 1024) gx = 1024;
  if (gx < 1) gx = 1;
  hipLaunchKernelGGL(scale_cols_ml_kernel, dim3(gx, nlev), dim3(256), 0, stream, y, L, row_stride, ncols);
  return utv2_launch_status();
}

int utv2_scale_cols_bwd_ml(float* g, const float* ypost, int nlev, const int64_t* row0_host, int row_stride, int ncols,
                           const float* const* s_host, float* const* sgrad_host, float* ws, hipStream_t stream) {
  ScaleLevels L;
  if (!g || !ypost || !ws || !sgrad_host || fill_scale_levels(L, nlev, row0_host, s_host, sgrad_host) != UTV2_OK) return UTV2_EARG;
  for (int l = 0; l < nlev; ++l)
    if (!L.sgrad[l]) return UTV2_EARG;
  const int nb = 1024;
  int64_t rows_max = 0;
  for (int l = 0; l < nlev; ++l) rows_max = rows_max > row0_host[l + 1] - row0_host[l] ? rows_max : row0_host[l + 1] - row0_host[l];
  const bool vec4 = (row_stride & 3) == 0 && (ncols & 3) == 0 && (((uintptr_t)g | (uintptr_t)ypost) & 15) == 0 &&
                    rows_max * (row_stride >> 2) < (int64_t)1 << 31;
  if (vec4) hipLaunchKernelGGL(scale_cols_bwd_ml_kernel<true>, dim3(nb, nlev), dim3(256), 0, stream, g, ypost, L, row_stride, ncols, ws);
  else hipLaunchKernelGGL(scale_cols_bwd_ml_kernel<false>, dim3(nb, nlev), dim3(256), 0, stream, g, ypost, L, row_stride, ncols, ws);
  hipLaunchKernelGGL(scale_cols_bwd_ml_final, dim3(nlev), dim3(256), 0, stream, L, (const float*)ws, nb);
  return utv2_launch_status();
}

int utv2_scale_cols_bwd_ml_pad16(const float* g, const float* ypost, int nlev, const int64_t* row0_host, int row_stride, int ncols,
                                 const float* const* s_host, float* const* sgrad_host, float* ws, void* out16, int cpad, hipStream_t stream) {
  ScaleLevels L;
  if (!g || !ypost || !ws || !sgrad_host || !out16 || fill_scale_levels(L, nlev, row0_host, s_host, sgrad_host) != UTV2_OK) return UTV2_EARG;
  for (int l = 0; l < nlev; ++l)
    if (!L.sgrad[l]) return UTV2_EARG;
  int64_t rows_max = 0;
  for (int l = 0; l < nlev; ++l) rows_max = rows_max > row0_host[l + 1] - row0_host[l] ? rows_max : row0_host[l + 1] - row0_host[l];
  if ((row_stride & 3) || (ncols & 3) || (cpad & 3) || cpad < row_stride || ncols > row_stride || ((((uintptr_t)g | (uintptr_t)ypost) & 15) != 0) ||
      (((uintptr_t)out16) & 7) != 0 || rows_max * (cpad >> 2) >= (int64_t)1 << 31)
    return UTV2_EARG;
  const int nb = 1024;
  hipLaunchKernelGGL(scale_cols_bwd_ml_pad16_kernel, dim3(nb, nlev), dim3(256), 0, stream, g, ypost, L, row_stride, ncols, ws, (h16_t*)out16, cpad);
  hipLaunchKernelGGL(scale_cols_bwd_ml_final, dim3(nlev), dim3(256), 0, stream, L, (const float*)ws, nb);
  return utv2_launch_status();
}

int utv2_fcos_loss_combine(const float* focal_sup, const float* sums_sup, const float* focal_cls, const float* sums_cls,
                           const float* sums_reg, const float* norm, float world, int flags, float kl_weight, const float* wmul_host,
                           const float* wdiv_host, float* rec, float* coef, hipStream_t stream) {
  if (!focal_sup || !sums_sup || !focal_cls || !sums_cls || !sums_reg || !wmul_host || !wdiv_host || !rec || !coef || !(world >= 1.f))
    return UTV2_EARG;
  FcosCombineArgs a;
  a.focal_sup = focal_sup; a.sums_sup = sums_sup; a.focal_cls = focal_cls; a.sums_cls = sums_cls; a.sums_reg = sums_reg; a.norm = norm;
  a.world = world; a.kl_weight = kl_weight; a.flags = flags;
  for (int k = 0; k < 6; ++k) { a.wmul[k] = wmul_host[k]; a.wdiv[k] = wdiv_host[k]; }
  hipLaunchKernelGGL(fcos_loss_combine_kernel, dim3(1), dim3(64), 0, stream, a, rec, coef);
  return utv2_launch_status();
}

}
```

### unbiased-teacher-v2_amd/ubteacher/hip.py

```python
import ctypes
import os

import torch

_HERE = os.path.dirname(os.path.abspath(__file__))
_LIB_DIR = os.environ.get("UTV2_LIB_DIR") or os.path.join(os.path.dirname(_HERE), "lib")
LIB_PATH = os.path.join(_LIB_DIR, "libutv2_hip.so")
LIB_PATHS = {"bf16": LIB_PATH, "fp16": os.path.join(_LIB_DIR, "libutv2_hip_f16.so")}
H16 = ["bf16"]


_H16_DT = [torch.bfloat16]


def set_h16(kind):
    assert kind in LIB_PATHS
    H16[0] = kind
    _H16_DT[0] = torch.bfloat16 if kind == "bf16" else torch.float16


def h16_dtype():
    return _H16_DT[0]

_lib = None
# ... 477 lines not shown

def fcos_loc_terms_fwd(labels, box, reg_targets, bvars, num_classes, reg_max, ts_better, ts_cert, flags=0):
    P, BS = box.shape
    sums = torch.empty(8, dtype=torch.float32, device=box.device)
    ws = workspace(4096, box.device, "loss")
    call("utv2_fcos_loc_terms_fwd", _p(labels), _p(box), BS, _p(reg_targets), _p(bvars), P, num_classes, reg_max,
         float(ts_better), float(ts_cert), int(flags), _p(sums), _p(ws), _stream())
    return sums


def fcos_loss_combine(focal_sup, sums_sup, focal_cls, sums_cls, sums_reg, norm, world, flags, kl_weight, wmul, wdiv):
    dev = sums_sup.device
    rec = torch.empty(8, dtype=torch.float32, device=dev)
    coef = torch.empty(26, dtype=torch.float32, device=dev)
    call("utv2_fcos_loss_combine", _p(focal_sup), _p(sums_sup), _p(focal_cls), _p(sums_cls), _p(sums_reg), _p(norm), float(world), int(flags),
         float(kl_weight), ctypes.cast(_farr(wmul), c_p), ctypes.cast(_farr(wdiv), c_p), _p(rec), _p(coef), _stream())
    return rec, coef


def fcos_loc_terms_bwd(labels, box, reg_targets, bvars, num_classes, reg_max, ts_better, ts_cert, coef, out=None, flags=0):
    P, BS = box.shape
    if out is None:
        out = torch.empty_like(box)
    call("utv2_fcos_loc_terms_bwd", _p(labels), _p(box), BS, _p(reg_targets), _p(bvars), P, num_classes, reg_max,
         float(ts_better), float(ts_cert), int(flags), _p(coef), _p(out), _stream())
    return out


def fcos_rank_keys(logits, box, reg_max, N, HW, thr, method, out=None, row_stride=None):
    C = logits.shape[-1]
    BS = box.shape[-1]
    if out is None:
        out = torch.empty((N, HW * C), dtype=torch.int64, device=logits.device)
        row_stride = HW * C
    assert out.stride(1) == 1 and out.stride(0) == row_stride and out.shape[0] == N and out.shape[1] >= HW * C
    call("utv2_fcos_rank_keys", _p_any(logits), _p_any(box), BS, reg_max, N, HW, C, float(thr), method, c_p(out.data_ptr()),
         int(row_stride), _stream())
    return out


def topk_rows(keys_flat, row_off, rows, max_width, k):
    out = torch.empty((rows, k), dtype=torch.int64, device=keys_flat.device)
    nbytes = load().utv2_topk_rows_workspace_bytes(rows, int(k))
    ws = workspace((nbytes + 3) // 4, keys_flat.device, "topk")
    call("utv2_topk_rows_i64", _p(keys_flat), _p(row_off), rows, int(max_width), int(k), _p(out), _p(ws), _stream())
    return out


def fcos_decode(topkeys, logits, box, reg_max, N, HW, Wl, stride, level, method, slot0, outs):
    K = topkeys.shape[1]
    C = logits.shape[-1]
    BS = box.shape[-1]
    MAXC = outs["scores"].shape[1]
    call("utv2_fcos_decode", _p(topkeys), K, _p(logits), _p(box), BS, reg_max, N, HW, Wl, C, stride, level, method, MAXC,
         slot0, _p(outs["boxes"]), _p(outs["scores"]), _p(outs["classes"]), _p(outs["locations"]), _p(outs["centerness"]),
         _p(outs["cls_confid"]), _p(outs["reg_pred_std"]), _p(outs["fpn_levels"]), _p(outs["valid"]), _stream())


def scale_cols(y2d, ncols, s):
    rows, BS = y2d.shape
    call("utv2_scale_cols", _p(y2d), rows, BS, ncols, _p(s), _stream())


def _i64arr(vals):
    return (ctypes.c_int64 * len(vals))(*[int(v) for v in vals])


def scale_cols_ml(y2d, rows, ncols, scales):
    assert len(rows) == len(scales) <= 8 and all(rows[i][1] == rows[i + 1][0] for i in range(len(rows) - 1))
    r0 = _i64arr([r[0] for r in rows] + [rows[-1][1]])
    sp = _ptr_array(scales)
    call("utv2_scale_cols_ml", _p(y2d), len(rows), ctypes.cast(r0, c_p), y2d.shape[1], ncols, ctypes.cast(sp, c_p), _stream())


def scale_cols_bwd_ml(g2d, ypost2d, rows, ncols, scales, sgrads):
    assert len(rows) == len(scales) == len(sgrads) <= 8 and all(rows[i][1] == rows[i + 1][0] for i in range(len(rows) - 1))
    r0 = _i64arr([r[0] for r in rows] + [rows[-1][1]])
    sp, gp = _ptr_array(scales), _ptr_array(sgrads)
    ws = workspace(8 * 1024, g2d.device, "loss")
    call("utv2_scale_cols_bwd_ml", _p(g2d), _p(ypost2d), len(rows), ctypes.cast(r0, c_p), g2d.shape[1], ncols, ctypes.cast(sp, c_p),
         ctypes.cast(gp, c_p), _p(ws), _stream())


def scale_cols_bwd_ml_pad16(g2d, ypost2d, rows, ncols, scales, sgrads, cpad):
    assert len(rows) == len(scales) == len(sgrads) <= 8 and all(rows[i][1] == rows[i + 1][0] for i in range(len(rows) - 1))
    r0 = _i64arr([r[0] for r in rows] + [rows[-1][1]])
    sp, gp = _ptr_array(scales), _ptr_array(sgrads)
    ws = workspace(8 * 1024, g2d.device, "loss")
    out = torch.empty((g2d.shape[0], cpad), dtype=h16_dtype(), device=g2d.device)
    call("utv2_scale_cols_bwd_ml_pad16", _p(g2d), _p(ypost2d), len(rows), ctypes.cast(r0, c_p), g2d.shape[1], ncols, ctypes.cast(sp, c_p),
         ctypes.cast(gp, c_p), _p(ws), _p(out), int(cpad), _stream())
    return out


def scale_cols_bwd(g2d, ypost2d, ncols, s):
    rows, BS = g2d.shape
    dsum = torch.empty(1, dtype=torch.float32, device=g2d.device)
    ws = workspace(4096, g2d.device, "loss")
    call("utv2_scale_cols_bwd", _p(g2d), _p(ypost2d), rows, BS, ncols, _p(s), _p(dsum), _p(ws), _stream())
    return dsum


def nms_batched(boxes, scores, classes, valid, iou_thr, class_aware=True, post_topk=-1, max_out=128):
    N, M = scores.shape
    keep = torch.empty((N, max_out), dtype=torch.int32, device=boxes.device)
    cnt = torch.empty(N, dtype=torch.int32, device=boxes.device)
    nbytes = load().utv2_nms_workspace_bytes(N, M)
    ws = workspace((nbytes + 3) // 4, boxes.device, "nms")
    call("utv2_nms_batched", _p(boxes), _p(scores), _p(classes), _p(valid), N, M, float(iou_thr), int(class_aware),
         int(post_topk), max_out, _p(keep), _p(cnt), _p(ws), _stream())
    return keep, cnt


def box_iou(a, b):
    A, B = a.shape[0], b.shape[0]
    out = torch.empty((A, B), dtype=torch.float32, device=a.device)
    call("utv2_box_iou", _p(a), _p(b), A, B, _p(out), _stream())
    return out


def match_boxes(boxes, gt_boxes, gt_valid, want_gt_max=False):
    N, G = gt_valid.shape
    shared = boxes.dim() == 2
    P = boxes.shape[-2]
    dev = gt_boxes.device
    mx = torch.empty((N, P), dtype=torch.float32, device=dev)
    arg = torch.empty((N, P), dtype=torch.int32, device=dev)
    gmax = torch.zeros((N, G), dtype=torch.int32, device=dev) if want_gt_max else None
    call("utv2_match_boxes", _p(boxes), 0 if shared else P * 4, N, P, _p(gt_boxes), _p(gt_valid), G, _p(mx), _p(arg),
         _p(gmax), _stream())
    return mx, arg, gmax


def match_lowq(boxes, gt_boxes, gt_valid, gmax):
    N, G = gt_valid.shape
    shared = boxes.dim() == 2
    P = boxes.shape[-2]
    out = torch.empty((N, P), dtype=torch.uint8, device=gt_boxes.device)
    call("utv2_match_lowq", _p(boxes), 0 if shared else P * 4, N, P, _p(gt_boxes), _p(gt_valid), G, _p(gmax), _p(out),
         _stream())
    return out


def _ptr_array(tensors):
    arr = (ctypes.c_void_p * len(tensors))(*[t.data_ptr() for t in tensors])
    return arr


def roi_align_fwd(feats, scales, min_level, rois, roi_batch, roi_valid, out_size):
    R = rois.shape[0]
    C = feats[0].shape[-1]
    out = torch.empty((R, out_size, out_size, C), dtype=feats[0].dtype, device=rois.device)
    fp = _ptr_array(feats)
    H = _iarr([f.shape[1] for f in feats]); W = _iarr([f.shape[2] for f in feats]); S = _farr(scales)
    call("utv2_roi_align_fwd", len(feats), min_level, ctypes.cast(fp, c_p), ctypes.cast(H, c_p), ctypes.cast(W, c_p),
         ctypes.cast(S, c_p), _p(rois), _p(roi_batch), _p(roi_valid), R, C, out_size, out_size, _p(out), _same_dt(*feats), _stream())
    return out


def roi_align_bwd(dfeats, scales, min_level, rois, roi_batch, roi_valid, dy):
    R, PH, PW, C = dy.shape
    fp = _ptr_array(dfeats)
    H = _iarr([f.shape[1] for f in dfeats]); W = _iarr([f.shape[2] for f in dfeats]); S = _farr(scales)
    call("utv2_roi_align_bwd", len(dfeats), min_level, ctypes.cast(fp, c_p), ctypes.cast(H, c_p), ctypes.cast(W, c_p),
         ctypes.cast(S, c_p), _p(rois), _p(roi_batch), _p(roi_valid), R, C, PH, PW, _p(dy), _dt(dy), _stream())


def roi_align_bwd_tiled(shapes, out_dtype, scales, min_level, rois, roi_valid, dy, rois_per_image, outs=None):
    R, PH, PW, C = dy.shape
    N = shapes[0][0]
    assert R == N * rois_per_image
    if outs is None:
# ... 259 lines not shown
    return bits


def conv2d_fwd_bf16(x, w16, scale=None, bias=None, residual=None, stride=1, pad=0, relu=False, kh=1, kw=1, out=None,
                    in_dil=1, out_hw=None, accumulate=False, out_dtype=None, mask=None, post_mask=None, relu_bits=None):
    N, H, W, C = x.shape
    K = w16.shape[0]
    assert w16.dtype == h16_dtype() and C % 8 == 0
    if out_hw is None:
        OH, OW = conv_out_size(H, kh, stride, pad), conv_out_size(W, kw, stride, pad)
    else:
        OH, OW = out_hw
    if out is None:
        out = torch.empty((N, OH, OW, K), dtype=_act_dtype(x, out_dtype), device=x.device)
    ri = None
    if _CONV_ROWINFO and kh * kw > 1 and in_dil == 1 and x.dtype == h16_dtype() and C % 32 == 0 and kh * kw <= 16 and W < 32768:
        ri = rowinfo_nhwc(N, H, W, OH, OW, stride, pad, kh, kw, x.device)
    if relu_bits is not None:
        assert out.dtype == h16_dtype()
        call("utv2_conv2d_nhwc_fwd_bf16_bits", _p(x), _dt(x), _p(w16), _p(out), _same_dt(out, residual, mask, post_mask), _p(scale), _p(bias),
             _p(residual), _p(mask), _p(post_mask), N, H, W, C, K, kh, kw, stride, pad, in_dil, OH, OW, int(relu), int(accumulate), _p(ri),
             _p(_bits_ok(relu_bits, out.shape)), c_p(0), c_p(0), _stream())
        return out
    call("utv2_conv2d_nhwc_fwd_bf16_ri", _p(x), _dt(x), _p(w16), _p(out), _same_dt(out, residual, mask, post_mask), _p(scale), _p(bias),
         _p(residual), _p(mask), _p(post_mask), N, H, W, C, K, kh, kw, stride, pad, in_dil, OH, OW, int(relu), int(accumulate), _p(ri), _stream())
    return out


def bottleneck_fwd_bf16(x, w1, w2, w3, s1, b1, s2, b2, s3, b3, wsc=None, ssc=None, bsc=None, out=None):
    N, H, W, C = x.shape
    MID, K = w1.shape[0], w3.shape[0]
    assert x.dtype == h16_dtype() and w1.dtype == w2.dtype == w3.dtype == h16_dtype() and K == 256
    assert tuple(w1.shape) == (MID, C) and tuple(w2.shape) == (MID, 9 * MID) and tuple(w3.shape) == (K, MID)
    assert wsc is None or (tuple(wsc.shape) == (K, C) and wsc.dtype == h16_dtype())
    if out is None:
        out = torch.empty((N, H, W, K), dtype=x.dtype, device=x.device)
    call("utv2_bottleneck_fwd_bf16", _p(x), _p(out), _p(w1), _p(w2), _p(w3), _p(wsc), _p(s1), _p(b1), _p(s2), _p(b2), _p(s3), _p(b3),
         _p(ssc), _p(bsc), N, H, W, C, MID, _stream())
    return out


def bottleneck_supported(C, MID, has_shortcut):
    return bool(load().utv2_bottleneck_supported(C, MID, int(has_shortcut)))


def conv2d_dgrad_bf16(dy, wt16, in_shape, stride, pad, kh, kw, out=None, out_dtype=None, mask=None, residual=None, post_mask=None,
                      mask_bits=None, post_mask_bits=None):
    N, H, W, C = in_shape
    _, OH, OW, K = dy.shape
    if out is None:
        out = torch.empty((N, H, W, C), dtype=_act_dtype(dy, out_dtype), device=dy.device)
    ri = None
    if _CONV_ROWINFO and kh * kw > 1 and stride == 1 and dy.dtype == h16_dtype() and K % 32 == 0 and kh * kw <= 16 and OW < 32768:
        ri = rowinfo_nhwc(N, OH, OW, H, W, 1, kh - 1 - pad, kh, kw, dy.device)
    if mask_bits is not None or post_mask_bits is not None:
        assert out.dtype == h16_dtype() and (mask is None or mask_bits is None) and (post_mask is None or post_mask_bits is None)
        call("utv2_conv2d_nhwc_fwd_bf16_bits", _p(dy), _dt(dy), _p(wt16), _p(out), _same_dt(out, residual, mask, post_mask), c_p(0), c_p(0),
             _p(residual), _p(mask), _p(post_mask), N, OH, OW, K, C, kh, kw, 1, kh - 1 - pad, stride, H, W, 0, 0, _p(ri), c_p(0),
             _p(_bits_ok(mask_bits, out.shape)) if mask_bits is not None else c_p(0),
             _p(_bits_ok(post_mask_bits, out.shape)) if post_mask_bits is not None else c_p(0), _stream())
        return out
    call("utv2_conv2d_nhwc_fwd_bf16_ri", _p(dy), _dt(dy), _p(wt16), _p(out), _same_dt(out, residual, mask, post_mask), c_p(0), c_p(0),
         _p(residual), _p(mask), _p(post_mask), N, OH, OW, K, C, kh, kw, 1, kh - 1 - pad, stride, H, W, 0, 0, _p(ri), _stream())
    return out


def _rows_ptr(t):
    assert t.is_cuda and t.dim() == 2 and t.stride(1) == 1 and t.stride(0) >= t.shape[1], "row-major matrix (or a column slice of one) expected"
    return c_p(t.data_ptr()), int(t.stride(0))


def gnb_eligible(x2d, w16, k, pad, groups):
    C = x2d.shape[1] // groups
    K = w16.shape[0]
    return (x2d.dtype == h16_dtype() and C % 64 == 0 and k * k * C >= 1024 and K % groups == 0 and (K // groups) % 128 == 0
            and x2d.stride(1) == 1 and x2d.stride(0) % 8 == 0 and x2d.shape[0] * x2d.stride(0) < (1 << 31))


def gnb_part_buffer(P, K, device):
    return torch.empty(((P + 63) // 64, K, 2), dtype=torch.float32, device=device)


def conv2d_ml_fwd_bf16(x2d, w16, level_hw, N, scale=None, bias=None, residual=None, k=3, pad=1, relu=False, out=None,
                       out_dtype=None, groups=1, gn_part=None, gnb=None):
    P = x2d.shape[0]
    C = x2d.shape[1] // groups
    K = w16.shape[0]
    assert w16.shape[1] == k * k * C, (tuple(w16.shape), k, C)
    if out is None:
        out = torch.empty((P, K), dtype=_act_dtype(x2d, out_dtype), device=x2d.device)
    H = _iarr([h for h, _ in level_hw]); W = _iarr([w_ for _, w_ in level_hw])
    xp, xpitch = _rows_ptr(x2d)
    yp, ypitch = _rows_ptr(out)
    if gnb is not None:
        bits, gx, part = gnb
        assert (scale is None and bias is None and residual is None and not relu and gn_part is None and out.dtype == h16_dtype()
                and ypitch == K and gx.dtype == h16_dtype() and gx.is_contiguous() and tuple(gx.shape) == (P, K)
                and bits.numel() * bits.element_size() * 8 == P * K and tuple(part.shape) == ((P + 63) // 64, K, 2))
        ri = rowinfo_ml(N, level_hw, pad, k, x2d.device) if (_CONV_ROWINFO and k > 1) else None
        call("utv2_conv2d_ml_fwd_bf16_gnb", xp, xpitch, _p(w16), yp, len(level_hw), ctypes.cast(H, c_p), ctypes.cast(W, c_p), N, C, K, k, k,
             pad, int(groups), _p(ri), _p(bits), _p(gx), _p(part), _stream())
        return out
    ri = None
    if (_CONV_ROWINFO and k > 1 and x2d.dtype == h16_dtype() and C % 32 == 0 and K % 4 == 0 and xpitch % 8 == 0 and ypitch % 8 == 0
            and (groups == 1 or (K // groups) % 128 == 0) and P * xpitch < (1 << 31)):
        ri = rowinfo_ml(N, level_hw, pad, k, x2d.device)
    if groups == 1 and xpitch == C and ypitch == K and gn_part is None and ri is None:
        call("utv2_conv2d_ml_fwd_bf16", xp, _dt(x2d), _p(w16), yp, _same_dt(out, residual), _p(scale), _p(bias), _p(residual),
             len(level_hw), ctypes.cast(H, c_p), ctypes.cast(W, c_p), N, C, K, k, k, pad, int(relu), 0, _stream())
    else:
        assert residual is None or (residual.stride(0) == ypitch and residual.stride(1) == 1)
        call("utv2_conv2d_ml_fwd_bf16_g", xp, _dt(x2d), xpitch, _p(w16), yp, _same_dt(out, residual), ypitch, _p(scale), _p(bias),
             c_p(residual.data_ptr()) if residual is not None else c_p(0), len(level_hw), ctypes.cast(H, c_p), ctypes.cast(W, c_p), N, C, K,
             k, k, pad, int(relu), 0, int(groups), _p(gn_part), _p(ri), _stream())
    return out


def gn_part_buffer(P, K, device):
    return torch.empty(((P + 31) // 32, K // 8, 2), dtype=torch.float32, device=device)


def groupnorm_relu_seg_fwd_p32(x2d, seg_rows, gamma, beta, part32, G, eps=1e-5, relu=True, relu_bits=None):
    rows, C = x2d.shape
    assert sum(seg_rows) == rows and x2d.dtype == h16_dtype() and C == 8 * G
    y = torch.empty_like(x2d)
    S = len(seg_rows)
    mean = torch.empty((S, G), dtype=torch.float32, device=x2d.device)
    rstd = torch.empty((S, G), dtype=torch.float32, device=x2d.device)
    sr = _iarr(seg_rows)
    if relu_bits is not None:
        assert relu_bits.dtype == torch.uint8 and relu_bits.numel() * 8 == rows * C and C % 32 == 0
        call("utv2_groupnorm_relu_seg_fwd_p32b", _p(x2d), _p(gamma), _p(beta), _p(y), _p(mean), _p(rstd), _p(part32), S, ctypes.cast(sr, c_p),
             C, G, float(eps), int(relu), _p(relu_bits), _stream())
    else:
        call("utv2_groupnorm_relu_seg_fwd_p32", _p(x2d), _p(gamma), _p(beta), _p(y), _p(mean), _p(rstd), _p(part32), S, ctypes.cast(sr, c_p),
             C, G, float(eps), int(relu), _stream())
    return y, mean, rstd


_rowinfo_cache = {}
_CONV_ROWINFO = os.environ.get("UTV2_CONV_ROWINFO", "1") != "0"


def _rowinfo_build(parts, device):
    total = sum(p[0] * p[3] * p[4] for p in parts)
    t = torch.empty((total, 2), dtype=torch.int32, device=device)
    off = 0
    for (N, H, W, OH, OW, stride, pad, kh, kw, start) in parts:
        call("utv2_rowinfo_nhwc", c_p(t.data_ptr() + 8 * off), N, H, W, OH, OW, stride, pad, kh, kw, start, _stream())
        off += N * OH * OW
    if torch.cuda.is_current_stream_capturing():
        raise RuntimeError("a conv geometry table was built inside a hipGraph capture: run the step eagerly once for every canvas first")
    torch.cuda.current_stream(t.device).synchronize()
    return t


def rowinfo_nhwc(N, H, W, OH, OW, stride, pad, kh, kw, device):
    assert kh * kw <= 16 and W < 32768
    key = ("nhwc", N, H, W, OH, OW, stride, pad, kh, kw, str(device))
    t = _rowinfo_cache.get(key)
    if t is None:
        t = _rowinfo_cache[key] = _rowinfo_build([(N, H, W, OH, OW, stride, pad, kh, kw, 0)], device)
    return t


def rowinfo_ml(N, level_hw, pad, k, device):
    key = ("ml", N, tuple(level_hw), pad, k, str(device))
    t = _rowinfo_cache.get(key)
    if t is None:
        parts, start = [], 0
        for (h, w) in level_hw:
            parts.append((N, h, w, h, w, 1, pad, k, k, start))
            start += N * h * w
        t = _rowinfo_cache[key] = _rowinfo_build(parts, device)
    return t


class WgradFoldLane:
    CAP = max(1, min(8, int(os.environ.get("UTV2_WGRAD_FOLD_CAP", "8"))))

    def __init__(self):
        self.table = ctypes.create_string_buffer(int(load().utv2_wgrad_fold_table_bytes()))
        self.arena = None
        self.off = 0
        self.n = 0
        self.dsts = set()

    def take(self, nfloats, device, dsts):
        nfl = (int(nfloats) + 63) // 64 * 64
        if self.n >= self.CAP or any(d in self.dsts for d in dsts) or (self.arena is not None and self.off + nfl > self.arena.numel()):
            self.flush()
        if self.arena is None or nfl > self.arena.numel():
            self.flush()
            self.arena = torch.empty(max(4 * nfl, 1 << 24), dtype=torch.float32, device=device)
            self.off = 0
        v = self.arena[self.off:self.off + nfl]
        self.off += nfl
        self.n += 1
        self.dsts.update(dsts)
        return v

    def flush(self):
        if self.n:
            call("utv2_wgrad_fold_flush", ctypes.cast(self.table, c_p), _stream())
        self.n = 0
        self.off = 0
        self.dsts.clear()


WGRAD_FOLD = [None]


def conv2d_wgrad_bf16(x, dy2d, dw, rowinfo, C, kh, kw, accumulate=True, db=None, rowscale=None, groups=1, x_pitch=None):
    M, K = dy2d.shape
    assert dy2d.stride(1) == 1
    dy_pitch = int(dy2d.stride(0))
    nws = load().utv2_conv2d_wgrad_bf16_workspace_floats(M, K, kh * kw * C)
    lane = WGRAD_FOLD[0]
    if lane is not None:
        ws = lane.take(nws, dy2d.device, [dw.data_ptr()] + ([db.data_ptr()] if db is not None else []))
        pitch = int(x_pitch) if x_pitch is not None else groups * C
        call("utv2_conv2d_wgrad_bf16_d", c_p(x.data_ptr()), _dt(x), pitch, c_p(dy2d.data_ptr()), _dt(dy2d), dy_pitch, _p(dw), _p(db), _p(ws),
             _p(rowinfo), _p(rowscale), M, C, K, kh, kw, int(accumulate), int(groups), ctypes.cast(lane.table, c_p), _stream())
        return dw
    ws = workspace(nws, dy2d.device, "wgrad")
    if groups == 1 and (x_pitch is None or x_pitch == C) and dy_pitch == K:
        call("utv2_conv2d_wgrad_bf16", _p(x), _dt(x), _p(dy2d), _dt(dy2d), _p(dw), _p(db), _p(ws), _p(rowinfo), _p(rowscale), M, C, K, kh,
             kw, int(accumulate), _stream())
    else:
        xp = c_p(x.data_ptr())
        pitch = int(x_pitch) if x_pitch is not None else groups * C
        call("utv2_conv2d_wgrad_bf16_g", xp, _dt(x), pitch, c_p(dy2d.data_ptr()), _dt(dy2d), dy_pitch, _p(dw), _p(db), _p(ws), _p(rowinfo),
             _p(rowscale), M, C, K, kh, kw, int(accumulate), int(groups), _stream())
    return dw


def gconv3x3_supported(C, groups):
    return bool(load().utv2_gconv3x3_supported(C, groups))


def _gconv_check(t, w, groups):
    C = t.shape[-1]
    assert t.dim() == 4 and t.dtype == w.dtype and tuple(w.shape) == (C, 9 * C // groups), (tuple(t.shape), tuple(w.shape), groups)
    assert gconv3x3_supported(C, groups), (C, groups)
    return C


def gconv3x3_fwd(x, w, groups, stride=1, scale=None, shift=None, relu=False, out_dtype=None, out=None):
    N, H, W, C = x.shape
    _gconv_check(x, w, groups)
    OH, OW = conv_out_size(H, 3, stride, 1), conv_out_size(W, 3, stride, 1)
    if out is None:
        out = torch.empty((N, OH, OW, C), dtype=out_dtype or x.dtype, device=x.device)
    assert tuple(out.shape) == (N, OH, OW, C)
    call("utv2_gconv3x3_fwd", _p(x), _p(w), _dt(x), _p(out), _dt(out), _p(scale), _p(shift), N, H, W, C, groups, stride, OH, OW,
         int(relu), _stream())
    return out


def gconv3x3_dgrad(dy, w, groups, stride, in_shape, scale=None, mask=None, residual=None, out_dtype=None):
    N, OH, OW, C = dy.shape
    _gconv_check(dy, w, groups)
    N_, H, W, C_ = in_shape
    assert (N_, C_) == (N, C) and (OH, OW) == (conv_out_size(H, 3, stride, 1), conv_out_size(W, 3, stride, 1))
    out = torch.empty((N, H, W, C), dtype=out_dtype or dy.dtype, device=dy.device)
    for t in (mask, residual):
        assert t is None or (t.dtype == out.dtype and tuple(t.shape) == tuple(out.shape))
    call("utv2_gconv3x3_dgrad", _p(dy), _p(w), _dt(dy), _p(out), _dt(out), _p(scale), _p(mask), _p(residual), N, H, W, C, groups, stride,
         OH, OW, _stream())
    return out


def gconv3x3_wgrad(x, dy, dw, groups, stride, scale=None, accumulate=True):
    N, H, W, C = x.shape
    _, OH, OW, _ = dy.shape
    assert x.dtype == dy.dtype and dw.dtype == torch.float32 and tuple(dw.shape) == (C, 9 * C // groups)
    assert gconv3x3_supported(C, groups) and tuple(dy.shape) == (N, conv_out_size(H, 3, stride, 1), conv_out_size(W, 3, stride, 1), C)
    ws = workspace(load().utv2_gconv3x3_wgrad_workspace_floats(N, OH, OW, C, groups), x.device, "gconv_wgrad")
    call("utv2_gconv3x3_wgrad", _p(x), _p(dy), _same_dt(x, dy), _p(dw), _p(ws), _p(scale), N, H, W, C, groups, stride, OH, OW,
         int(accumulate), _stream())
    return dw


def groupnorm_relu_seg_fwd(x2d, seg_rows, gamma, beta, G=32, eps=1e-5, relu=True):
    rows, C = x2d.shape
    assert sum(seg_rows) == rows
    y = torch.empty_like(x2d)
    S = len(seg_rows)
    mean = torch.empty((S, G), dtype=torch.float32, device=x2d.device)
    rstd = torch.empty((S, G), dtype=torch.float32, device=x2d.device)
    sr = _iarr(seg_rows)
    ws = workspace(load().utv2_groupnorm_seg_workspace_floats(S, ctypes.cast(sr, c_p), C), x2d.device, "gn")
    call("utv2_groupnorm_relu_seg_fwd", _p(x2d), _p(gamma), _p(beta), _p(y), _p(mean), _p(rstd), _p(ws), S, ctypes.cast(sr, c_p), C, G,
         float(eps), int(relu), _dt(x2d), _stream())
    return y, mean, rstd


def groupnorm_relu_seg_bwd(dy, y, x2d, seg_rows, mean, rstd, gamma, dgamma, dbeta, G=32, relu=True, beta=None, want_colsum=False):
    rows, C = x2d.shape
    S = len(seg_rows)
    dx = torch.empty_like(x2d)
# ... 173 lines not shown
```

### unbiased-teacher-v2_amd/ubteacher/ops.py

```python
import os

import torch

from . import hip

_HOOKS = {}
PRECISION = ["fp32"]


def set_precision(p):
    assert p in ("fp32", "bf16", "fp16")
    PRECISION[0] = p
    hip.set_h16("fp16" if p == "fp16" else "bf16")


def amp():
    return PRECISION[0] != "fp32"


def act_dtype():
    return hip.h16_dtype() if amp() else torch.float32


_VERSION = [0]
# ... 79 lines not shown
            t.record_stream(side)
    _WGRAD["pending"].add(dev)


def _fold_on():
    return os.environ.get("UTV2_WGRAD_FOLD", "0") == "1"


def flush_wgrad_folds(dev=None):
    for side, fl in _WGRAD.get("folds", {}).items():
        if fl.n and (dev is None or side.device == dev):
            with torch.cuda.stream(side):
                fl.flush()


def wgrad_stream_behind_main(dev):
    if not _WGRAD["on"] or dev.type != "cuda":
        return None
    lanes = _WGRAD["streams"].get(dev)
    if lanes is None:
        return None
    flush_wgrad_folds(dev)
    side = lanes[0]
    side.wait_stream(torch.cuda.current_stream(dev))
    for other in lanes[1:]:
        side.wait_stream(other)
    return side


def join_wgrad_stream():
    flush_deferred_wgrads()
    flush_wgrad_folds()
    for dev in list(_WGRAD["pending"]):
        for side in _WGRAD["streams"][dev]:
            torch.cuda.current_stream(dev).wait_stream(side)
    _WGRAD["pending"].clear()


def _sync_handles(layer, cs=None):
    from .utils.grad_sync import param_handles
    hs = param_handles(layer)
    if cs is not None:
        hs = hs + (list(cs) if isinstance(cs, (list, tuple)) else [cs])
    return hs


def hook(device):
    key = str(device)
    h = _HOOKS.get(key)
    if h is None:
        h = torch.zeros(1, device=device, requires_grad=True)
        _HOOKS[key] = h
    return h


def bump_version():
    _VERSION[0] += 1


class LevelMeta:

    def __init__(self, N, level_hw):
        self.N = N
        self.level_hw = [tuple(x) for x in level_hw]
        self.rows = []
        r = 0
        for h, w in self.level_hw:
            self.rows.append((r, r + N * h * w))
            r += N * h * w
        self.P = r
        self.seg_rows = [h * w for (h, w) in self.level_hw for _ in range(N)]

    def level_view(self, t2d, l):
        r0, r1 = self.rows[l]
        h, w = self.level_hw[l]
        return t2d[r0:r1].view(self.N, h, w, t2d.shape[1])

    def alias_view(self, t2d, l):
        r0, r1 = self.rows[l]
        h, w = self.level_hw[l]
        C = t2d.shape[1]
        return torch.empty((0,), dtype=t2d.dtype, device=t2d.device).set_(
            t2d.untyped_storage(), t2d.storage_offset() + r0 * C, (self.N, h, w, C), (h * w * C, w * C, C, 1))


def _scale_ml_on():
    return os.environ.get("UTV2_SCALE_ML", "1") != "0"


class FlipBank:

    def __init__(self, store):
        self.store = store
        self.layers = []
        self.slot = {}
        self.dirty = False
        self.version = None
        self.bank = None
        self.views = []
        self.single = {}

    def _current(self):
        return (_VERSION[0], self.store.version, hip.H16[0])

    def _rebuild(self):
        import struct
        self.h16 = hip.H16[0]
        dev = self.store.flat.device
        offs, total = [], 0
        for layer, _ in self.layers:
            offs.append(total)
            total += (layer.dgrad_cout() * layer.k * layer.k * layer.cin + 7) // 8 * 8
        self.bank = torch.empty(total, dtype=hip.h16_dtype(), device=dev)
        self.scales = None
        rec = bytearray()
        self.nrec = 0
        for (layer, sc), o in zip(self.layers, offs):
            so = -1
            if sc is not None:
                if self.scales is None:
                    self.scales = torch.empty(0, dtype=torch.float32, device=dev).set_(sc.untyped_storage())
                assert sc.untyped_storage().data_ptr() == self.scales.untyped_storage().data_ptr()
                so = sc.storage_offset()
            G = layer.groups
            if G == 1:
                rec += struct.pack("<qqqiiiiii", layer.w.offset, o, so, layer.cout, layer.k, layer.k, layer.cin, layer.dgrad_cout(), 0)
                self.nrec += 1
            else:
                assert sc is None and layer.dgrad_cout() == layer.cout
                Kg = layer.cout // G
                for gi in range(G):
                    rec += struct.pack("<qqqiiiiii", layer.w.offset + gi * Kg * layer.kred, o + gi * layer.cin * layer.k * layer.k * Kg, -1,
                                       Kg, layer.k, layer.k, layer.cin, Kg, 0)
                    self.nrec += 1
        self.table = torch.frombuffer(rec, dtype=torch.uint8).clone().to(dev)
        self.views = [self.bank[o:o + l.dgrad_cout() * l.k * l.k * l.cin].view(l.groups * l.cin, l.k * l.k * l.dgrad_cout() // l.groups)
                      for (l, _), o in zip(self.layers, offs)]
        self.dirty = False
        self.single.clear()

    def refresh_ahead(self):
        cur = self._current()
        if (self.bank is None or self.dirty or self.version == cur or self.h16 != hip.H16[0] or os.environ.get("UTV2_FLIP_AHEAD", "1") == "0"
                or STEP_GRAPH[0]):
            return
        dev = self.store.flat.device
        if dev.type != "cuda":
            return
        side = self.__dict__.get("_side")
        if side is None:
            side = self._side = torch.cuda.Stream(dev)
        side.wait_stream(torch.cuda.current_stream(dev))
        with torch.cuda.stream(side):
            hip.weight_flip_transpose_bf16_batched(self.store.flat, self.scales, self.bank, self.table, self.nrec)
            self._ahead = torch.cuda.Event()
            self._ahead.record(side)
        self.version = cur

    def _join_ahead(self):
        ev = self.__dict__.pop("_ahead", None)
        if ev is not None:
            torch.cuda.current_stream(self.store.flat.device).wait_event(ev)

    def get(self, layer, scale):
        cur = self._current()
        if "_ahead" in self.__dict__:
# ... 120 lines not shown
        else:
            assert x.dtype == torch.float32, "the fp32 conv kernels take fp32 activations (layer cin=%d)" % self.cin
        if not b16 and not x.is_contiguous():
            x = x.contiguous()
        if self.groups > 1:
            assert meta is not None and self.k > 1 and residual is None and out is None and cs is None
        if meta is not None and self.k > 1:
            assert self.stride == 1 and self.pad == (self.k - 1) // 2
            if b16:
                part = None
                if self.gn_stats_fused() and out is None and residual is None and kw["out_dtype"] == hip.h16_dtype() and self.cin % 32 == 0:
                    part = hip.gn_part_buffer(x.shape[0], self.cout, x.device)
                y = hip.conv2d_ml_fwd_bf16(x, w, meta.level_hw, meta.N, scale=sc, bias=sh, residual=residual, k=self.k, pad=self.pad,
                                           relu=self.relu, out=out, groups=self.groups, gn_part=part, **kw)
                self._gn_part = (y.data_ptr(), part) if part is not None else None
            elif self.groups > 1:
                Kg = self.cout // self.groups
                y = torch.cat([hip.conv2d_ml_fwd(x[:, gi * self.cin:(gi + 1) * self.cin].contiguous(), w[gi * Kg:(gi + 1) * Kg], meta.level_hw,
                                                 meta.N, scale=None, bias=None if sh is None else sh[gi * Kg:(gi + 1) * Kg], k=self.k,
                                                 pad=self.pad, relu=self.relu) for gi in range(self.groups)], dim=1)
            else:
                y = hip.conv2d_ml_fwd(x, w, meta.level_hw, meta.N, scale=sc, bias=sh, residual=residual, k=self.k, pad=self.pad,
                                      relu=self.relu, out=out, **kw)
        elif meta is not None:
            fn = hip.conv2d_fwd_bf16 if b16 else hip.conv2d_fwd
            y = fn(x.view(1, x.shape[0], 1, x.shape[1]), w, scale=sc, bias=sh,
                   residual=None if residual is None else residual.view(1, x.shape[0], 1, -1), relu=self.relu,
                   out=None if out is None else out.view(1, x.shape[0], 1, -1), **kw).view(x.shape[0], self.cout)
        else:
            fn = hip.conv2d_fwd_bf16 if b16 else hip.conv2d_fwd
            if relu_bits is not None:
                kw["relu_bits"] = relu_bits
            y = fn(x, w, scale=sc, bias=sh, residual=residual, stride=self.stride, pad=self.pad, relu=self.relu, kh=self.k,
                   kw=self.k, out=out, **kw)
        if cs is not None:
            assert y.dtype == torch.float32
            if meta is not None and _scale_ml_on() and y.is_contiguous():
                hip.scale_cols_ml(y, meta.rows, self.colscale, [h.t for h in cs])
            elif meta is not None:
                for l, h in enumerate(cs):
                    r0, r1 = meta.rows[l]
                    hip.scale_cols(y[r0:r1], self.colscale, h.t)
            else:
                hip.scale_cols(y.view(-1, self.cout), self.colscale, cs.t)
        return y


class _ConvFn(torch.autograd.Function):
    @staticmethod
    def forward(ctx, x, residual, hk, layer, out_holder, cs, meta):
        out = out_holder[0]
        y = layer._forward(x, residual, out, cs, meta)
        ctx.layer = layer
        ctx.cs = cs
        ctx.meta = meta
        ctx.has_res = residual is not None
        ctx.x_bits = _bits_of(x) if (layer.premask_input and meta is None) else None
        ctx.handoff = getattr(x, "_utv2_handoff", None) if (layer.premask_input and meta is None and grad_handoff_on()) else None
        if GRAD_SYNC[0] is not None:
            GRAD_SYNC[0].on_forward(_sync_handles(layer, cs))
        ctx.save_for_backward(x, y if (layer.relu or cs is not None) else None)
        ctx.xshape = tuple(x.shape)
        ctx.gnb = None
        src = layer.gnb_src
        if src is not None and src._gnb_fwd is not None:
            gf, src._gnb_fwd = src._gnb_fwd, None
            if gf[0] == x.data_ptr() and x.is_contiguous() and tuple(gf[1].shape) == tuple(x.shape) and residual is None:
                ctx.gnb = (src, gf[1], gf[2])
        ctx.fanin = out_holder[1] if len(out_holder) > 1 else None
        ctx.pair = out_holder[2] if len(out_holder) > 2 else None
        return y

    @staticmethod
    def backward(ctx, dy):
        layer = ctx.layer
        if layer.gconv:
            return _ConvFn._backward_grouped(ctx, dy)
        x, y = ctx.saved_tensors
        dy = dy.contiguous()
        if not x.is_contiguous() and not (layer.use_bf16_wgrad() and layer.use_bf16_dgrad()):
            x = x.contiguous()
        sc, _ = layer.scale_shift()
        meta = ctx.meta
        gp_ready = None
        if (ctx.cs is not None and meta is not None and _scale_ml_on() and y.is_contiguous() and dy.dtype == torch.float32
                and layer.k > 1 and ctx.needs_input_grad[0] and layer.use_bf16_dgrad() and layer.use_bf16_wgrad()
                and layer.dgrad_cout() != layer.cout and not layer.relu and sc is None and not ctx.has_res
                and os.environ.get("UTV2_SCALE_BWD_PAD16", "1") != "0"):
            gp_ready = hip.scale_cols_bwd_ml_pad16(dy, y, meta.rows, layer.colscale, [h.t for h in ctx.cs], [h.g for h in ctx.cs],
                                                   layer.dgrad_cout())
        elif ctx.cs is not None:
            g = dy.clone()
            if meta is not None and _scale_ml_on() and y.is_contiguous():
                hip.scale_cols_bwd_ml(g, y, meta.rows, layer.colscale, [h.t for h in ctx.cs], [h.g for h in ctx.cs])
            elif meta is not None:
                for l, h in enumerate(ctx.cs):
                    r0, r1 = meta.rows[l]
                    dsum = hip.scale_cols_bwd(g[r0:r1], y[r0:r1], layer.colscale, h.t)
                    h.g.add_(dsum / h.t.view(-1))
            else:
                dsum = hip.scale_cols_bwd(g.view(-1, layer.cout), y.view(-1, layer.cout), layer.colscale, ctx.cs.t)
                ctx.cs.g.add_(dsum / ctx.cs.t.view(-1))
            dy = g
        gres = None
        d16 = layer.use_bf16_dgrad()
        fold = sc is not None and d16 and layer.use_bf16_wgrad() and layer.bias is None
        wsc = sc if fold else None
        relu = layer.relu and not (layer.grad_premasked and premask_on())
        if fold:
            g = hip.relu_bwd_scale(dy, y, None) if relu else dy
            gres = g if ctx.has_res else None
        elif ctx.has_res:
            gm = hip.relu_bwd_scale(dy, y if relu else None, None) if relu else dy
            gres = gm
            g = hip.relu_bwd_scale(gm, None, sc) if sc is not None else gm
        else:
            if relu or sc is not None:
                g = hip.relu_bwd_scale(dy, y if relu else None, sc)
            else:
                g = dy
        dx = None
        bias_done = False
        if meta is not None and layer.k > 1:
            G = layer.groups
            Kg = layer.cout // G
            if ctx.needs_input_grad[0]:
                if d16:
                    gp = gp_ready if gp_ready is not None else (g if layer.dgrad_cout() == layer.cout else hip.pad_cols_bf16(g, layer.dgrad_cout()))
                    other = ctx.fanin.take() if ctx.fanin is not None else None
                    if other is not None and (other.dtype != x.dtype or tuple(other.shape) != tuple(x.shape)):
                        raise RuntimeError("FanIn: stored gradient does not match the conv input")
                    dest = ctx.pair[0].grad_half(ctx.pair[1], x) if (ctx.pair is not None and other is None) else None
                    wt = layer.wt16(wsc)
                    if (ctx.gnb is not None and other is None and dest is None and x.dtype == hip.h16_dtype()
                            and hip.gnb_eligible(gp, wt, layer.k, layer.k - 1 - layer.pad, G)):
                        src, gx, bits = ctx.gnb
                        part = hip.gnb_part_buffer(x.shape[0], x.shape[1], x.device)
                        dx = hip.conv2d_ml_fwd_bf16(gp, wt, meta.level_hw, meta.N, k=layer.k, pad=layer.k - 1 - layer.pad, out_dtype=x.dtype,
                                                    groups=G, gnb=(bits, gx, part))
                        src._gnb_bwd = (dx.data_ptr(), part)
                    else:
                        dx = hip.conv2d_ml_fwd_bf16(gp, wt, meta.level_hw, meta.N, k=layer.k, pad=layer.k - 1 - layer.pad,
                                                    residual=other, out_dtype=x.dtype, out=dest, groups=G)
                elif G > 1:
                    dx = torch.cat([hip.conv2d_ml_dgrad(g[:, gi * Kg:(gi + 1) * Kg].contiguous(),
                                                        hip.weight_flip_transpose(layer.w.t[gi * Kg:(gi + 1) * Kg], Kg, layer.k, layer.k, layer.cin),
                                                        meta.level_hw, meta.N, layer.k, layer.pad) for gi in range(G)], dim=1)
                else:
                    dx = hip.conv2d_ml_dgrad(g, layer.wt(), meta.level_hw, meta.N, layer.k, layer.pad)
            if layer.use_bf16_wgrad():
                gw = gp[:, :layer.cout] if (d16 and ctx.needs_input_grad[0] and gp is not g) else g
                _wgrad_launch(lambda: hip.conv2d_wgrad_bf16(
                    x, gw, layer.w.g, hip.rowinfo_ml(meta.N, meta.level_hw, layer.pad, layer.k, x.device), layer.cin, layer.k, layer.k,
                    accumulate=True, db=layer.bias.g if (layer.bias is not None and not layer.bias_grad_from_gn()) else None, rowscale=wsc,
                    groups=G, x_pitch=x.stride(0)), x, gw, key=layer)
                bias_done = True
            elif G > 1:
                for gi in range(G):
                    xg, gg = x[:, gi * layer.cin:(gi + 1) * layer.cin].contiguous(), g[:, gi * Kg:(gi + 1) * Kg].contiguous()
                    _wgrad_launch(lambda xg=xg, gg=gg, gi=gi: hip.conv2d_ml_wgrad(xg, gg, layer.w.g[gi * Kg:(gi + 1) * Kg], meta.level_hw, meta.N,
                                                                                   layer.k, layer.pad, accumulate=True), xg, gg, key=layer)
            else:
                _wgrad_launch(lambda: hip.conv2d_ml_wgrad(x, g, layer.w.g, meta.level_hw, meta.N, layer.k, layer.pad, accumulate=True), x, g, key=layer)
        else:
            x4 = x.view(1, x.shape[0], 1, x.shape[1]) if meta is not None else x
            g4 = g.view(1, g.shape[0], 1, g.shape[1]) if meta is not None else g
            if ctx.needs_input_grad[0]:
                pm = x4 if (layer.premask_input and premask_on()) else None
                if d16 and layer.k == 1 and layer.stride == 2 and layer.pad == 0:
                    dxc = hip.conv2d_fwd_bf16(g4, layer.wt16(wsc), out_dtype=x.dtype)
                    dx = hip.zero_interleave2x(dxc, x4.shape[1], x4.shape[2], mask=pm)
                elif (d16 and layer.k == 3 and layer.stride == 2 and layer.pad == 1 and g4.shape[-1] % 32 == 0
                      and x4.shape[0] * x4.shape[1] * x4.shape[2] <= 65536):
                    gd = hip.zero_interleave2x(g4.contiguous(), x4.shape[1], x4.shape[2])
                    dx = hip.conv2d_fwd_bf16(gd, layer.wt16(wsc), pad=1, kh=3, kw=3, out_dtype=x.dtype, mask=pm)
                elif d16:
                    gd = g4
                    if layer.dgrad_cout() != layer.cout:
                        gd = hip.pad_cols_bf16(g4.reshape(-1, layer.cout), layer.dgrad_cout()).view(g4.shape[:-1] + (layer.dgrad_cout(),))
                    pb = ctx.x_bits if (pm is not None and relu_bits_on() and x.dtype == hip.h16_dtype()) else None
                    BITS_STATS["reads"] += pb is not None
                    dx = hip.conv2d_dgrad_bf16(gd, layer.wt16(wsc), tuple(x4.shape), layer.stride, layer.pad, layer.k, layer.k,
                                               out_dtype=x.dtype, mask=None if pb is not None else pm, mask_bits=pb)
                else:
                    dx = hip.conv2d_dgrad(g4, layer.wt(), tuple(x4.shape), layer.stride, layer.pad, layer.k, layer.k)
                    if pm is not None:
                        dx = hip.relu_bwd_scale(dx, x4, None)
                if meta is not None:
                    dx = dx.view(x.shape)
                elif ctx.handoff is not None and pm is not None and dx.dtype == hip.h16_dtype() and ctx.handoff.park(dx):
                    dx = None
            if layer.use_bf16_wgrad():
                n_, h_, w_, _ = x4.shape
                ri = hip.rowinfo_nhwc(n_, h_, w_, g4.shape[1], g4.shape[2], layer.stride, layer.pad, layer.k, layer.k, x.device)
                _wgrad_launch(lambda: hip.conv2d_wgrad_bf16(
                    x4, g4.reshape(-1, layer.cout), layer.w.g, ri, layer.cin, layer.k, layer.k, accumulate=True,
                    db=layer.bias.g if (layer.bias is not None and not layer.bias_grad_from_gn()) else None, rowscale=wsc), x4, g4, key=layer)
                bias_done = True
            else:
                _wgrad_launch(lambda: hip.conv2d_wgrad(x4, g4, layer.w.g, layer.stride, layer.pad, layer.k, layer.k, accumulate=True), x4, g4, key=layer)
        if layer.bias is not None and not bias_done:
            _wgrad_launch(lambda: hip.colsum(g.view(-1, layer.cout), layer.bias.g, accumulate=True), g, key=layer)
        if GRAD_SYNC[0] is not None:
            GRAD_SYNC[0].on_backward_done(_sync_handles(layer, ctx.cs))
        return dx, gres, None, None, None, None, None

    @staticmethod
    def _backward_grouped(ctx, dy):
        layer = ctx.layer
        x, y = ctx.saved_tensors
        w = layer.gconv_weight()
        g = dy.contiguous()
        if g.dtype != w.dtype:
            g = g.to(w.dtype)
        relu = layer.relu and not (layer.grad_premasked and premask_on())
        if relu:
            g = hip.relu_bwd_scale(g, y if y.dtype == g.dtype else y.to(g.dtype), None)
        sc, _ = layer.scale_shift()
        dx = None
        if ctx.needs_input_grad[0]:
            pm = x if (layer.premask_input and premask_on()) else None
            dx = hip.gconv3x3_dgrad(g, w, layer.groups, layer.stride, tuple(x.shape), scale=sc, mask=pm, out_dtype=x.dtype)
        _wgrad_launch(lambda: hip.gconv3x3_wgrad(x, g, layer.w.g, layer.groups, layer.stride, scale=sc, accumulate=True), x, g, key=layer)
        if GRAD_SYNC[0] is not None:
            GRAD_SYNC[0].on_backward_done(_sync_handles(layer))
        return dx, None, None, None, None, None, None


def _wgrad16(layer, x4, g4):
    if layer.gconv:
        _wgrad_launch(lambda: hip.gconv3x3_wgrad(x4, g4, layer.w.g, layer.groups, layer.stride, scale=layer.bn.scale, accumulate=True),
                      x4, g4, key=layer)
        return
    n_, h_, w_, _ = x4.shape
    ri = hip.rowinfo_nhwc(n_, h_, w_, g4.shape[1], g4.shape[2], layer.stride, layer.pad, layer.k, layer.k, x4.device)
    _wgrad_launch(lambda: hip.conv2d_wgrad_bf16(x4, g4.reshape(-1, layer.cout), layer.w.g, ri, layer.cin, layer.k, layer.k, accumulate=True,
                                                rowscale=layer.bn.scale), x4, g4, key=layer)

# ... 650 lines not shown
```

Baseline: 345.3.

## Skip all-zero gradient tiles in box-head conv dgrad and wgrad

The scale-cols backward pass now also emits a bitmap marking which 32-row chunks of the padded gradient hold nonzeros. A new flags kernel turns that bitmap into per-128-row tile flags, which let the implicit-GEMM dgrad kernel skip the main loop for dead tiles. The wgrad kernel walks only the set chunks through a sparse pipelined loop. This aims to cut work on sparse head gradients, at the cost of an extra bitmap pass, a flags kernel, and a less regular pipeline.

```diff
diff --git a/include/utv2.h b/include/utv2.h
--- a/include/utv2.h
+++ b/include/utv2.h
@@ -52,6 +52,11 @@
                               const float* scale, const float* bias, const void* residual, int nlev, const int* H_host,
                               const int* W_host, int N, int C, int K, int KH, int KW, int pad, int relu, int accumulate, int groups,
                               float* gn_part, const int* rowinfo, utv2_stream_t stream);
+int utv2_conv2d_ml_fwd_bf16_gs(const void* x, int x_dtype, int x_pitch, const void* w16, void* y, int y_dtype, int y_pitch,
+                               const float* scale, const float* bias, const void* residual, int nlev, const int* H_host,
+                               const int* W_host, int N, int C, int K, int KH, int KW, int pad, int relu, int accumulate, int groups,
+                               float* gn_part, const int* rowinfo, const int* tile_flags, utv2_stream_t stream);
+int utv2_conv_tile_flags(const void* chunk_bits, const int* rowinfo, int M, int KH, int KW, int* flags, utv2_stream_t stream);
 int utv2_conv2d_ml_fwd_bf16_gnb(const void* x, int x_pitch, const void* w16, void* y, int nlev, const int* H_host, const int* W_host, int N,
                                 int C, int K, int KH, int KW, int pad, int groups, const int* rowinfo, const void* mask_bits,
                                 const void* gnb_x, float* gnb_part, utv2_stream_t stream);
@@ -66,6 +71,9 @@
 int utv2_conv2d_wgrad_bf16_d(const void* x, int x_dtype, int x_pitch, const void* dy, int dy_dtype, int dy_pitch, float* dw, float* db,
                              float* ws, const int* rowinfo, const float* rowscale, int M, int C, int K, int KH, int KW, int accumulate,
                              int groups, void* pending, utv2_stream_t stream);
+int utv2_conv2d_wgrad_bf16_s(const void* x, int x_dtype, int x_pitch, const void* dy, int dy_dtype, int dy_pitch, float* dw, float* db,
+                             float* ws, const int* rowinfo, const float* rowscale, int M, int C, int K, int KH, int KW, int accumulate,
+                             int groups, const void* chunk_bits, void* pending, utv2_stream_t stream);
 int64_t utv2_wgrad_fold_table_bytes(void);
 int utv2_wgrad_fold_pending(const void* pending);
 int utv2_wgrad_fold_flush(void* pending, utv2_stream_t stream);
@@ -190,6 +198,9 @@
                            const float* const* s_host, float* const* sgrad_host, float* ws, utv2_stream_t stream);
 int utv2_scale_cols_bwd_ml_pad16(const float* g, const float* ypost, int nlev, const int64_t* row0_host, int row_stride, int ncols,
                                  const float* const* s_host, float* const* sgrad_host, float* ws, void* out16, int cpad, utv2_stream_t stream);
+int utv2_scale_cols_bwd_ml_pad16_bits(const float* g, const float* ypost, int nlev, const int64_t* row0_host, int row_stride, int ncols,
+                                      const float* const* s_host, float* const* sgrad_host, float* ws, void* out16, int cpad,
+                                      void* chunk_bits, utv2_stream_t stream);
 
 int utv2_nms_mpad(int M);
 int64_t utv2_nms_workspace_bytes(int N, int M);
diff --git a/unbiased-teacher-v2_amd/csrc/conv_bf16.hip b/unbiased-teacher-v2_amd/csrc/conv_bf16.hip
--- a/unbiased-teacher-v2_amd/csrc/conv_bf16.hip
+++ b/unbiased-teacher-v2_amd/csrc/conv_bf16.hip
@@ -32,6 +32,7 @@
   EpiBits bits;
   int mtot;
   const int2* rowinfo;
+  const int* tile_flags = nullptr;
 };
 
 __device__ __forceinline__ void ml_decode16(const LevelTab& lt, int m, int& pixbase, int& H, int& W, int& oh, int& ow) {
@@ -370,7 +371,7 @@
 }
 
 
-template <int BN, bool ML, int BK, typename TO, bool TALL = false, bool GNB = false>
+template <int BN, bool ML, int BK, typename TO, bool TALL = false, bool GNB = false, bool SKIP = false>
 __global__ __launch_bounds__(256, TALL ? 3 : ((BK == 32 && BN != 96) ? 4 : 2)) void conv_igemm_bf16_v2(ConvArgs16 p) {
   static_assert(!TALL || BN == 64, "the tall layout exists for the 64-wide tile");
   constexpr int WN = (BN == 96 || TALL) ? 1 : 2, WM = 4 / WN, WCOLS = BN / WN;
@@ -502,17 +503,21 @@
   for (int s = 0; s < KS; ++s) koff[s] = ((2 * s + fh) ^ swz) * 16;
   const int arow = (wm * 64 + frow) * ROWB, brow = (wn * WCOLS + frow) * ROWB;
 
-  cursor_next();
-#pragma unroll
-  for (int q = 0; q < NP; ++q) load_piece(q);
-#pragma unroll
-  for (int q = 0; q < NP; ++q) store_piece(0, q);
-  if (nchunks > 1) {
+  bool live = true;
+  if constexpr (SKIP) live = p.tile_flags[mt] != 0;
+  if (live) {
     cursor_next();
 #pragma unroll
     for (int q = 0; q < NP; ++q) load_piece(q);
-  }
-  __syncthreads();
+#pragma unroll
+    for (int q = 0; q < NP; ++q) store_piece(0, q);
+    if (nchunks > 1) {
+      cursor_next();
+#pragma unroll
+      for (int q = 0; q < NP; ++q) load_piece(q);
+    }
+    __syncthreads();
+  }
   auto iteration = [&](int buf, auto do_store, auto do_load) {
     constexpr bool STORE = decltype(do_store)::value, LOAD = decltype(do_load)::value;
     if constexpr (LOAD) cursor_next();
@@ -542,10 +547,12 @@
   };
   using yes = std::integral_constant<bool, true>;
   using no = std::integral_constant<bool, false>;
-  int kc = 0;
-  for (; kc + 2 < nchunks; ++kc) iteration(kc & 1, yes{}, yes{});
-  if (kc + 1 < nchunks) { iteration(kc & 1, yes{}, no{}); ++kc; }
-  iteration(kc & 1, no{}, no{});
+  if (live) {
+    int kc = 0;
+    for (; kc + 2 < nchunks; ++kc) iteration(kc & 1, yes{}, yes{});
+    if (kc + 1 < nchunks) { iteration(kc & 1, yes{}, no{}); ++kc; }
+    iteration(kc & 1, no{}, no{});
+  }
 
   if ((p.K & 3) == 0) {
     static_assert(sizeof(smem) >= 4 * 32 * (PCOLS + 4) * sizeof(float), "epilogue patches must fit the staging LDS");
@@ -1306,6 +1313,9 @@
       if (gnb) hipLaunchKernelGGL((conv_igemm_bf16_v2<BN, ML, 64, h16_t, false, (ML && BN == 128)>), g, b, 0, stream, a);
       else if (y_dtype == UTV2_BF16) hipLaunchKernelGGL((conv_igemm_bf16_v2<BN, ML, 64, h16_t>), g, b, 0, stream, a);
       else hipLaunchKernelGGL((conv_igemm_bf16_v2<BN, ML, 64, float>), g, b, 0, stream, a);
+    } else if (ML && BN == 128 && a.tile_flags && a.m_begin == 0) {
+      if (y_dtype == UTV2_BF16) hipLaunchKernelGGL((conv_igemm_bf16_v2<BN, ML, 32, h16_t, false, false, (ML && BN == 128)>), g, b, 0, stream, a);
+      else hipLaunchKernelGGL((conv_igemm_bf16_v2<BN, ML, 32, float, false, false, (ML && BN == 128)>), g, b, 0, stream, a);
     } else {
       if (y_dtype == UTV2_BF16) hipLaunchKernelGGL((conv_igemm_bf16_v2<BN, ML, 32, h16_t>), g, b, 0, stream, a);
       else hipLaunchKernelGGL((conv_igemm_bf16_v2<BN, ML, 32, float>), g, b, 0, stream, a);
@@ -1407,7 +1417,8 @@
 
 static int ml_fwd_g(const void* x, int x_dtype, int x_pitch, const void* w16, void* y, int y_dtype, int y_pitch, const float* scale,
                     const float* bias, const void* residual, int nlev, const int* H_host, const int* W_host, int N, int C, int K, int KH, int KW,
-                    int pad, int relu, int accumulate, int groups, float* gn_part, const int* rowinfo, EpiBits bits, hipStream_t stream) {
+                    int pad, int relu, int accumulate, int groups, float* gn_part, const int* rowinfo, EpiBits bits, hipStream_t stream,
+                    const int* tile_flags = nullptr) {
   if (gn_part && (y_dtype != UTV2_BF16 || (K & 7) || (y_pitch & 7) || x_dtype != UTV2_BF16 || (C % 32) || accumulate)) return UTV2_EARG;
   if (!x || !w16 || !y || nlev < 1 || nlev > CONV_MAX_LEVELS || (C % 8) || N <= 0 || bad_dtype(x_dtype) || bad_dtype(y_dtype) || groups < 1 ||
       K % groups || x_pitch < groups * C || y_pitch < K)
@@ -1424,6 +1435,7 @@
   a.x = x; a.w = (const h16_t*)w16; a.y = y; a.scale = scale; a.bias = bias; a.residual = residual; a.mask = nullptr; a.post_mask = nullptr;
   a.N = N; a.H = 0; a.W = 0; a.C = C; a.OH = 0; a.OW = 0; a.K = K; a.KH = KH; a.KW = KW; a.stride = 1; a.pad = pad; a.in_dil = 1;
   a.relu = (relu ? 1 : 0) | g_epi_general; a.accumulate = accumulate; a.Kred = KH * KW * C; a.xs = x_pitch; a.m_begin = 0; a.groups = groups; a.ldy = y_pitch; a.gn_part = gn_part; a.rowinfo = (const int2*)rowinfo;
+  a.tile_flags = tile_flags;
   const bool small = K <= 64 && plain;
   const int tiles = cdiv(a.M, 128) * cdiv(K, small ? 64 : 128);
   if (n96_eligible(a, x_dtype)) launch_igemm16<96, true>(a, cdiv(a.M, 256), x_dtype, y_dtype, stream);
@@ -1438,6 +1450,15 @@
                               float* gn_part, const int* rowinfo, hipStream_t stream) {
   return ml_fwd_g(x, x_dtype, x_pitch, w16, y, y_dtype, y_pitch, scale, bias, residual, nlev, H_host, W_host, N, C, K, KH, KW, pad, relu,
                   accumulate, groups, gn_part, rowinfo, EpiBits{nullptr, nullptr, nullptr, nullptr, nullptr}, stream);
+}
+
+int utv2_conv2d_ml_fwd_bf16_gs(const void* x, int x_dtype, int x_pitch, const void* w16, void* y, int y_dtype, int y_pitch,
+                               const float* scale, const float* bias, const void* residual, int nlev, const int* H_host,
+                               const int* W_host, int N, int C, int K, int KH, int KW, int pad, int relu, int accumulate, int groups,
+                               float* gn_part, const int* rowinfo, const int* tile_flags, hipStream_t stream) {
+  if (!tile_flags || !rowinfo) return UTV2_EARG;
+  return ml_fwd_g(x, x_dtype, x_pitch, w16, y, y_dtype, y_pitch, scale, bias, residual, nlev, H_host, W_host, N, C, K, KH, KW, pad, relu,
+                  accumulate, groups, gn_part, rowinfo, EpiBits{nullptr, nullptr, nullptr, nullptr, nullptr}, stream, tile_flags);
 }
 
 int utv2_conv2d_ml_fwd_bf16_gnb(const void* x, int x_pitch, const void* w16, void* y, int nlev, const int* H_host, const int* W_host, int N,
@@ -1516,6 +1537,24 @@
   }
 }
 
+__global__ __launch_bounds__(128) void conv_tile_flags_kernel(const unsigned* __restrict__ bits, const int2* __restrict__ rowinfo, int M, int KH,
+                                                              int KW, int* __restrict__ flags) {
+  const int m = blockIdx.x * 128 + threadIdx.x;
+  int any = 0;
+  if (m < M) {
+    const int2 ri = rowinfo[m];
+    const int W = ri.y >> 16;
+    for (int kh = 0; kh < KH; ++kh)
+      for (int kw = 0; kw < KW; ++kw)
+        if ((ri.y >> (kh * KW + kw)) & 1) {
+          const int src = ri.x + kh * W + kw;
+          if ((unsigned)src < (unsigned)M) any |= (bits[src >> 10] >> ((src >> 5) & 31)) & 1;
+        }
+  }
+  any = __syncthreads_or(any);
+  if (threadIdx.x == 0) flags[blockIdx.x] = any ? 1 : 0;
+}
+
 int utv2_rowinfo_nhwc(int* out, int N, int H, int W, int OH, int OW, int stride, int pad, int KH, int KW, int64_t start,
                       hipStream_t stream) {
   if (!out || N < 1 || H < 1 || W < 1 || OH < 1 || OW < 1 || stride < 1 || pad < 0 || KH < 1 || KW < 1 || KH * KW > 16 || W >= 32768 ||
@@ -1524,6 +1563,13 @@
   int64_t nb = ((int64_t)N * OH * OW + 255) / 256;
   if (nb > 8192) nb = 8192;
   hipLaunchKernelGGL(rowinfo_kernel, dim3((int)nb), dim3(256), 0, stream, (int2*)out, N, H, W, OH, OW, stride, pad, KH, KW, (long long)start);
+  return utv2_launch_status();
+}
+
+int utv2_conv_tile_flags(const void* chunk_bits, const int* rowinfo, int M, int KH, int KW, int* flags, hipStream_t stream) {
+  if (!chunk_bits || !rowinfo || !flags || M <= 0 || KH < 1 || KW < 1 || KH * KW > 16) return UTV2_EARG;
+  hipLaunchKernelGGL(conv_tile_flags_kernel, dim3(cdiv(M, 128)), dim3(128), 0, stream, (const unsigned*)chunk_bits, (const int2*)rowinfo, M,
+                     KH, KW, flags);
   return utv2_launch_status();
 }
 
@@ -1580,6 +1626,7 @@
   int groups;
   int dys;
   int debug;
+  const unsigned* chunk_bits = nullptr;
 };
 
 __device__ __forceinline__ bf16x4_t lds_read_tr16(const unsigned char* p) {
@@ -1588,7 +1635,7 @@
   return __builtin_bit_cast(bf16x4_t, v);
 }
 
-template <typename TX, typename TDY>
+template <typename TX, typename TDY, bool SPARSE = false>
 __global__ __launch_bounds__(256) void conv_wgrad_bf16(Wgrad16Args p) {
   constexpr int BK = 32, LDR = 320;
   constexpr int OPB = BK * LDR;
@@ -1692,7 +1739,7 @@
 
   const int G = lane >> 4, t = lane & 15;
   const int frag_off = (8 * (G >> 1) + (t >> 2)) * LDR + (16 * (G & 1) + 4 * (t & 3)) * 2;
-  auto iteration = [&](int ch, int buf, auto do_store, auto do_load) {
+  auto iteration = [&](int ld, int rl, int buf, auto do_store, auto do_load) {
     constexpr bool STORE = decltype(do_store)::value, LOAD = decltype(do_load)::value;
     const unsigned char* ab = smem + buf * 2 * OPB + frag_off;
     const unsigned char* bb = ab + OPB;
@@ -1720,10 +1767,10 @@
 #pragma unroll
       for (int q = (s == 0 ? 2 : 0); q < (s == 0 ? 4 : 2); ++q) {
         if constexpr (STORE) store_piece(buf ^ 1, q);
-        if constexpr (LOAD) load_piece(ch + 2, q);
+        if constexpr (LOAD) load_piece(ld, q);
       }
       if constexpr (LOAD) {
-        if (s == 0) rload(ch + 3);
+        if (s == 0) rload(rl);
       }
       __builtin_amdgcn_sched_barrier(0);
     }
@@ -1731,7 +1778,46 @@
   };
   using yes = std::integral_constant<bool, true>;
   using no = std::integral_constant<bool, false>;
-  if (chunk_begin < chunk_end) {
+  if constexpr (SPARSE) {
+    auto next_set = [&](int c) -> int {
+      while (c < chunk_end) {
+        const unsigned w = p.chunk_bits[c >> 5] >> (c & 31);
+        if (w) {
+          c += __builtin_ctz(w);
+          break;
+        }
+        c = (c | 31) + 1;
+      }
+      return __builtin_amdgcn_readfirstlane(c < chunk_end ? c : chunk_end);
+    };
+    const int c0 = next_set(chunk_begin);
+    if (c0 < chunk_end) {
+      rload(c0);
+#pragma unroll
+      for (int q = 0; q < 4; ++q) load_piece(c0, q);
+      int c1 = next_set(c0 + 1), c2 = chunk_end;
+      rload(c1);
+#pragma unroll
+      for (int q = 0; q < 4; ++q) store_piece(0, q);
+      if (c1 < chunk_end) {
+#pragma unroll
+        for (int q = 0; q < 4; ++q) load_piece(c1, q);
+        c2 = next_set(c1 + 1);
+        rload(c2);
+      }
+      __syncthreads();
+      int buf = 0;
+      while (c2 < chunk_end) {
+        const int c3 = next_set(c2 + 1);
+        iteration(c2, c3, buf, yes{}, yes{});
+        c1 = c2;
+        c2 = c3;
+        buf ^= 1;
+      }
+      if (c1 < chunk_end) { iteration(0, 0, buf, yes{}, no{}); buf ^= 1; }
+      iteration(0, 0, buf, no{}, no{});
+    }
+  } else if (chunk_begin < chunk_end) {
     rload(chunk_begin);
 #pragma unroll
     for (int q = 0; q < 4; ++q) load_piece(chunk_begin, q);
@@ -1745,9 +1831,9 @@
     }
     __syncthreads();
     int ch = chunk_begin;
-    for (; ch + 2 < chunk_end; ++ch) iteration(ch, (ch - chunk_begin) & 1, yes{}, yes{});
-    if (ch + 1 < chunk_end) { iteration(ch, (ch - chunk_begin) & 1, yes{}, no{}); ++ch; }
-    iteration(ch, (ch - chunk_begin) & 1, no{}, no{});
+    for (; ch + 2 < chunk_end; ++ch) iteration(ch + 2, ch + 3, (ch - chunk_begin) & 1, yes{}, yes{});
+    if (ch + 1 < chunk_end) { iteration(0, 0, (ch - chunk_begin) & 1, yes{}, no{}); ++ch; }
+    iteration(0, 0, (ch - chunk_begin) & 1, no{}, no{});
   }
   if (p.bias_ws != nullptr && nt == 0) {
     float* red = (float*)smem;
@@ -2246,7 +2332,7 @@
 
 static int wgrad_bf16_impl(const void* x, int x_dtype, int x_pitch, const void* dy, int dy_dtype, int dy_pitch, float* dw, float* db,
                            float* ws, const int* rowinfo, const float* rowscale, int M, int C, int K, int KH, int KW, int accumulate,
-                           int groups, hipStream_t stream, SlabFoldTable* pending = nullptr);
+                           int groups, hipStream_t stream, SlabFoldTable* pending = nullptr, const unsigned* chunk_bits = nullptr);
 
 int utv2_conv2d_wgrad_bf16(const void* x, int x_dtype, const void* dy, int dy_dtype, float* dw, float* db, float* ws,
                            const int* rowinfo, const float* rowscale, int M, int C, int K, int KH, int KW, int accumulate,
@@ -2269,6 +2355,16 @@
   if (t->count < 0 || t->count + 3 > SLAB_FOLD_MAX) return UTV2_EARG;
   return wgrad_bf16_impl(x, x_dtype, x_pitch, dy, dy_dtype, dy_pitch, dw, db, ws, rowinfo, rowscale, M, C, K, KH, KW, accumulate, groups,
                          stream, t);
+}
+
+int utv2_conv2d_wgrad_bf16_s(const void* x, int x_dtype, int x_pitch, const void* dy, int dy_dtype, int dy_pitch, float* dw, float* db,
+                             float* ws, const int* rowinfo, const float* rowscale, int M, int C, int K, int KH, int KW, int accumulate,
+                             int groups, const void* chunk_bits, void* pending, hipStream_t stream) {
+  if (!chunk_bits) return UTV2_EARG;
+  SlabFoldTable* t = (SlabFoldTable*)pending;
+  if (t && (t->count < 0 || t->count + 3 > SLAB_FOLD_MAX)) return UTV2_EARG;
+  return wgrad_bf16_impl(x, x_dtype, x_pitch, dy, dy_dtype, dy_pitch, dw, db, ws, rowinfo, rowscale, M, C, K, KH, KW, accumulate, groups,
+                         stream, t, (const unsigned*)chunk_bits);
 }
 
 int64_t utv2_wgrad_fold_table_bytes(void) { return (int64_t)sizeof(SlabFoldTable); }
@@ -2288,7 +2384,7 @@
 
 static int wgrad_bf16_impl(const void* x, int x_dtype, int x_pitch, const void* dy, int dy_dtype, int dy_pitch, float* dw, float* db,
                            float* ws, const int* rowinfo, const float* rowscale, int M, int C, int K, int KH, int KW, int accumulate,
-                           int groups, hipStream_t stream, SlabFoldTable* pending) {
+                           int groups, hipStream_t stream, SlabFoldTable* pending, const unsigned* chunk_bits) {
   if (!x || !dy || !dw || !ws || !rowinfo || (C & 7) || (K & 7) || M <= 0 || KH * KW > 16 || bad_dtype(x_dtype) ||
       bad_dtype(dy_dtype) || groups < 1 || K % groups || x_pitch < groups * C || (groups > 1 && (K / groups) % 128) ||
       (x_pitch != C && (x_pitch & (x_dtype == UTV2_BF16 ? 7 : 3))) || dy_pitch < K || (dy_pitch != K && (dy_pitch & (dy_dtype == UTV2_BF16 ? 7 : 3))))
@@ -2332,7 +2428,10 @@
   a.bias_ws = db ? ws + (size_t)a.splits * n : nullptr;
   const int tiles = cdiv(K, 128) * cdiv(a.Kred, 128);
   const dim3 g(tiles * a.splits), b(256);
-  if (x_dtype == UTV2_BF16) {
+  if (chunk_bits && x_dtype == UTV2_BF16 && dy_dtype == UTV2_BF16) {
+    a.chunk_bits = chunk_bits;
+    hipLaunchKernelGGL((conv_wgrad_bf16<h16_t, h16_t, true>), g, b, 0, stream, a);
+  } else if (x_dtype == UTV2_BF16) {
     if (dy_dtype == UTV2_BF16) hipLaunchKernelGGL((conv_wgrad_bf16<h16_t, h16_t>), g, b, 0, stream, a);
     else hipLaunchKernelGGL((conv_wgrad_bf16<h16_t, float>), g, b, 0, stream, a);
   } else {
diff --git a/unbiased-teacher-v2_amd/csrc/fcos.hip b/unbiased-teacher-v2_amd/csrc/fcos.hip
--- a/unbiased-teacher-v2_amd/csrc/fcos.hip
+++ b/unbiased-teacher-v2_amd/csrc/fcos.hip
@@ -635,9 +635,10 @@
   if (threadIdx.x == 0) partial[(size_t)l * gridDim.x + blockIdx.x] = t;
 }
 
+template <bool BITS>
 __global__ __launch_bounds__(256) void scale_cols_bwd_ml_pad16_kernel(const float* __restrict__ g, const float* __restrict__ ypost, ScaleLevels L,
                                                                     int BS, int ncols, float* __restrict__ partial, h16_t* __restrict__ out,
-                                                                    int cpad) {
+                                                                    int cpad, unsigned* __restrict__ bits) {
   __shared__ float red[4];
   const int l = blockIdx.y;
   const float* gl = g + (size_t)L.row0[l] * BS;
@@ -661,6 +662,16 @@
     }
     h16x4 o = {(h16_t)gv[0], (h16_t)gv[1], (h16_t)gv[2], (h16_t)gv[3]};
     *(h16x4*)(ol + (size_t)i * 4) = o;
+    if constexpr (BITS) {
+      const bool nz = (float)o[0] != 0.f || (float)o[1] != 0.f || (float)o[2] != 0.f || (float)o[3] != 0.f;
+      const int chunk = nz ? (int)((L.row0[l] + r) >> 5) : -1;
+      const int prev = __shfl_up(chunk, 1);
+      if (nz && ((threadIdx.x & 63) == 0 || prev != chunk)) {
+        unsigned* wp = bits + (chunk >> 5);
+        const unsigned b = 1u << (chunk & 31);
+        if (!(__atomic_load_n(wp, __ATOMIC_RELAXED) & b)) atomicOr(wp, b);
+      }
+    }
   }
   const float t = block_reduce_sum(acc, red);
   if (threadIdx.x == 0) partial[(size_t)l * gridDim.x + blockIdx.x] = t;
@@ -913,8 +924,26 @@
   return utv2_launch_status();
 }
 
+static int scale_cols_bwd_ml_pad16_impl(const float* g, const float* ypost, int nlev, const int64_t* row0_host, int row_stride, int ncols,
+                                       const float* const* s_host, float* const* sgrad_host, float* ws, void* out16, int cpad,
+                                       unsigned* chunk_bits, hipStream_t stream);
+
 int utv2_scale_cols_bwd_ml_pad16(const float* g, const float* ypost, int nlev, const int64_t* row0_host, int row_stride, int ncols,
                                  const float* const* s_host, float* const* sgrad_host, float* ws, void* out16, int cpad, hipStream_t stream) {
+  return scale_cols_bwd_ml_pad16_impl(g, ypost, nlev, row0_host, row_stride, ncols, s_host, sgrad_host, ws, out16, cpad, nullptr, stream);
+}
+
+int utv2_scale_cols_bwd_ml_pad16_bits(const float* g, const float* ypost, int nlev, const int64_t* row0_host, int row_stride, int ncols,
+                                      const float* const* s_host, float* const* sgrad_host, float* ws, void* out16, int cpad,
+                                      void* chunk_bits, hipStream_t stream) {
+  if (!chunk_bits) return UTV2_EARG;
+  return scale_cols_bwd_ml_pad16_impl(g, ypost, nlev, row0_host, row_stride, ncols, s_host, sgrad_host, ws, out16, cpad, (unsigned*)chunk_bits,
+                                      stream);
+}
+
+static int scale_cols_bwd_ml_pad16_impl(const float* g, const float* ypost, int nlev, const int64_t* row0_host, int row_stride, int ncols,
+                                       const float* const* s_host, float* const* sgrad_host, float* ws, void* out16, int cpad,
+                                       unsigned* chunk_bits, hipStream_t stream) {
   ScaleLevels L;
   if (!g || !ypost || !ws || !sgrad_host || !out16 || fill_scale_levels(L, nlev, row0_host, s_host, sgrad_host) != UTV2_OK) return UTV2_EARG;
   for (int l = 0; l < nlev; ++l)
@@ -925,7 +954,15 @@
       (((uintptr_t)out16) & 7) != 0 || rows_max * (cpad >> 2) >= (int64_t)1 << 31)
     return UTV2_EARG;
   const int nb = 1024;
-  hipLaunchKernelGGL(scale_cols_bwd_ml_pad16_kernel, dim3(nb, nlev), dim3(256), 0, stream, g, ypost, L, row_stride, ncols, ws, (h16_t*)out16, cpad);
+  if (chunk_bits) {
+    const int64_t chunks = (row0_host[nlev] + 31) / 32;
+    if (hipError_t e = hipMemsetAsync(chunk_bits, 0, (size_t)((chunks + 31) / 32) * 4, stream); e != hipSuccess) return -(int)e;
+    hipLaunchKernelGGL(scale_cols_bwd_ml_pad16_kernel<true>, dim3(nb, nlev), dim3(256), 0, stream, g, ypost, L, row_stride, ncols, ws,
+                       (h16_t*)out16, cpad, chunk_bits);
+  } else {
+    hipLaunchKernelGGL(scale_cols_bwd_ml_pad16_kernel<false>, dim3(nb, nlev), dim3(256), 0, stream, g, ypost, L, row_stride, ncols, ws,
+                       (h16_t*)out16, cpad, (unsigned*)nullptr);
+  }
   hipLaunchKernelGGL(scale_cols_bwd_ml_final, dim3(nlev), dim3(256), 0, stream, L, (const float*)ws, nb);
   return utv2_launch_status();
 }
diff --git a/unbiased-teacher-v2_amd/ubteacher/hip.py b/unbiased-teacher-v2_amd/ubteacher/hip.py
--- a/unbiased-teacher-v2_amd/ubteacher/hip.py
+++ b/unbiased-teacher-v2_amd/ubteacher/hip.py
@@ -583,12 +583,21 @@
          ctypes.cast(gp, c_p), _p(ws), _stream())
 
 
-def scale_cols_bwd_ml_pad16(g2d, ypost2d, rows, ncols, scales, sgrads, cpad):
+def chunk_bits_buffer(rows, device):
+    return torch.empty(((rows + 31) // 32 + 31) // 32, dtype=torch.int32, device=device)
+
+
+def scale_cols_bwd_ml_pad16(g2d, ypost2d, rows, ncols, scales, sgrads, cpad, want_bits=False):
     assert len(rows) == len(scales) == len(sgrads) <= 8 and all(rows[i][1] == rows[i + 1][0] for i in range(len(rows) - 1))
     r0 = _i64arr([r[0] for r in rows] + [rows[-1][1]])
     sp, gp = _ptr_array(scales), _ptr_array(sgrads)
     ws = workspace(8 * 1024, g2d.device, "loss")
     out = torch.empty((g2d.shape[0], cpad), dtype=h16_dtype(), device=g2d.device)
+    if want_bits:
+        bits = chunk_bits_buffer(g2d.shape[0], g2d.device)
+        call("utv2_scale_cols_bwd_ml_pad16_bits", _p(g2d), _p(ypost2d), len(rows), ctypes.cast(r0, c_p), g2d.shape[1], ncols,
+             ctypes.cast(sp, c_p), ctypes.cast(gp, c_p), _p(ws), _p(out), int(cpad), _p(bits), _stream())
+        return out, bits
     call("utv2_scale_cols_bwd_ml_pad16", _p(g2d), _p(ypost2d), len(rows), ctypes.cast(r0, c_p), g2d.shape[1], ncols, ctypes.cast(sp, c_p),
          ctypes.cast(gp, c_p), _p(ws), _p(out), int(cpad), _stream())
     return out
@@ -1014,7 +1023,7 @@
 
 
 def conv2d_ml_fwd_bf16(x2d, w16, level_hw, N, scale=None, bias=None, residual=None, k=3, pad=1, relu=False, out=None,
-                       out_dtype=None, groups=1, gn_part=None, gnb=None):
+                       out_dtype=None, groups=1, gn_part=None, gnb=None, tile_flags=None):
     P = x2d.shape[0]
     C = x2d.shape[1] // groups
     K = w16.shape[0]
@@ -1034,10 +1043,18 @@
              pad, int(groups), _p(ri), _p(bits), _p(gx), _p(part), _stream())
         return out
     ri = None
-    if (_CONV_ROWINFO and k > 1 and x2d.dtype == h16_dtype() and C % 32 == 0 and K % 4 == 0 and xpitch % 8 == 0 and ypitch % 8 == 0
+    if ((_CONV_ROWINFO or tile_flags is not None) and k > 1 and x2d.dtype == h16_dtype() and C % 32 == 0 and K % 4 == 0 and xpitch % 8 == 0 and ypitch % 8 == 0
             and (groups == 1 or (K // groups) % 128 == 0) and P * xpitch < (1 << 31)):
         ri = rowinfo_ml(N, level_hw, pad, k, x2d.device)
-    if groups == 1 and xpitch == C and ypitch == K and gn_part is None and ri is None:
+    if tile_flags is not None:
+        if ri is None or gnb is not None:
+            raise RuntimeError("conv2d_ml_fwd_bf16: tile_flags need the geometry-table path (16-bit x, C % 32 == 0, k > 1)")
+        assert residual is None or (residual.stride(0) == ypitch and residual.stride(1) == 1)
+        assert tile_flags.dtype == torch.int32 and tile_flags.numel() == (P + 127) // 128
+        call("utv2_conv2d_ml_fwd_bf16_gs", xp, _dt(x2d), xpitch, _p(w16), yp, _same_dt(out, residual), ypitch, _p(scale), _p(bias),
+             c_p(residual.data_ptr()) if residual is not None else c_p(0), len(level_hw), ctypes.cast(H, c_p), ctypes.cast(W, c_p), N, C, K,
+             k, k, pad, int(relu), 0, int(groups), _p(gn_part), _p(ri), _p(tile_flags), _stream())
+    elif groups == 1 and xpitch == C and ypitch == K and gn_part is None and ri is None:
         call("utv2_conv2d_ml_fwd_bf16", xp, _dt(x2d), _p(w16), yp, _same_dt(out, residual), _p(scale), _p(bias), _p(residual),
              len(level_hw), ctypes.cast(H, c_p), ctypes.cast(W, c_p), N, C, K, k, k, pad, int(relu), 0, _stream())
     else:
@@ -1108,6 +1125,14 @@
     return t
 
 
+def conv_tile_flags(chunk_bits, rowinfo, k):
+    M = rowinfo.shape[0]
+    assert chunk_bits.dtype == torch.int32 and chunk_bits.numel() == ((M + 31) // 32 + 31) // 32
+    flags = torch.empty((M + 127) // 128, dtype=torch.int32, device=rowinfo.device)
+    call("utv2_conv_tile_flags", _p(chunk_bits), _p(rowinfo), M, k, k, _p(flags), _stream())
+    return flags
+
+
 class WgradFoldLane:
     CAP = max(1, min(8, int(os.environ.get("UTV2_WGRAD_FOLD_CAP", "8"))))
 
@@ -1143,12 +1168,22 @@
 WGRAD_FOLD = [None]
 
 
-def conv2d_wgrad_bf16(x, dy2d, dw, rowinfo, C, kh, kw, accumulate=True, db=None, rowscale=None, groups=1, x_pitch=None):
+def conv2d_wgrad_bf16(x, dy2d, dw, rowinfo, C, kh, kw, accumulate=True, db=None, rowscale=None, groups=1, x_pitch=None, chunk_bits=None):
     M, K = dy2d.shape
     assert dy2d.stride(1) == 1
     dy_pitch = int(dy2d.stride(0))
     nws = load().utv2_conv2d_wgrad_bf16_workspace_floats(M, K, kh * kw * C)
     lane = WGRAD_FOLD[0]
+    if chunk_bits is not None:
+        assert chunk_bits.dtype == torch.int32 and chunk_bits.numel() == ((M + 31) // 32 + 31) // 32
+        if lane is not None:
+            ws = lane.take(nws, dy2d.device, [dw.data_ptr()] + ([db.data_ptr()] if db is not None else []))
+        else:
+            ws = workspace(nws, dy2d.device, "wgrad")
+        call("utv2_conv2d_wgrad_bf16_s", c_p(x.data_ptr()), _dt(x), int(x_pitch) if x_pitch is not None else groups * C, c_p(dy2d.data_ptr()),
+             _dt(dy2d), dy_pitch, _p(dw), _p(db), _p(ws), _p(rowinfo), _p(rowscale), M, C, K, kh, kw, int(accumulate), int(groups),
+             _p(chunk_bits), ctypes.cast(lane.table, c_p) if lane is not None else None, _stream())
+        return dw
     if lane is not None:
         ws = lane.take(nws, dy2d.device, [dw.data_ptr()] + ([db.data_ptr()] if db is not None else []))
         pitch = int(x_pitch) if x_pitch is not None else groups * C
diff --git a/unbiased-teacher-v2_amd/ubteacher/ops.py b/unbiased-teacher-v2_amd/ubteacher/ops.py
--- a/unbiased-teacher-v2_amd/ubteacher/ops.py
+++ b/unbiased-teacher-v2_amd/ubteacher/ops.py
@@ -185,6 +185,13 @@
         C = t2d.shape[1]
         return torch.empty((0,), dtype=t2d.dtype, device=t2d.device).set_(
             t2d.untyped_storage(), t2d.storage_offset() + r0 * C, (self.N, h, w, C), (h * w * C, w * C, C, 1))
+
+
+SPARSE_BWD_STATS = {"dgrad": 0, "wgrad": 0}
+
+
+def box_head_sparse_bwd_on():
+    return os.environ.get("UTV2_BOX_HEAD_SPARSE_BWD", "1") != "0"
 
 
 def _scale_ml_on():
@@ -471,13 +478,17 @@
             x = x.contiguous()
         sc, _ = layer.scale_shift()
         meta = ctx.meta
-        gp_ready = None
+        gp_ready = gp_bits = None
         if (ctx.cs is not None and meta is not None and _scale_ml_on() and y.is_contiguous() and dy.dtype == torch.float32
                 and layer.k > 1 and ctx.needs_input_grad[0] and layer.use_bf16_dgrad() and layer.use_bf16_wgrad()
                 and layer.dgrad_cout() != layer.cout and not layer.relu and sc is None and not ctx.has_res
                 and os.environ.get("UTV2_SCALE_BWD_PAD16", "1") != "0"):
-            gp_ready = hip.scale_cols_bwd_ml_pad16(dy, y, meta.rows, layer.colscale, [h.t for h in ctx.cs], [h.g for h in ctx.cs],
-                                                   layer.dgrad_cout())
+            if box_head_sparse_bwd_on() and layer.groups == 1:
+                gp_ready, gp_bits = hip.scale_cols_bwd_ml_pad16(dy, y, meta.rows, layer.colscale, [h.t for h in ctx.cs], [h.g for h in ctx.cs],
+                                                                layer.dgrad_cout(), want_bits=True)
+            else:
+                gp_ready = hip.scale_cols_bwd_ml_pad16(dy, y, meta.rows, layer.colscale, [h.t for h in ctx.cs], [h.g for h in ctx.cs],
+                                                       layer.dgrad_cout())
         elif ctx.cs is not None:
             g = dy.clone()
             if meta is not None and _scale_ml_on() and y.is_contiguous():
@@ -529,8 +540,12 @@
                                                     groups=G, gnb=(bits, gx, part))
                         src._gnb_bwd = (dx.data_ptr(), part)
                     else:
+                        tf = None
+                        if gp_bits is not None and layer.k - 1 - layer.pad == layer.pad:
+                            tf = hip.conv_tile_flags(gp_bits, hip.rowinfo_ml(meta.N, meta.level_hw, layer.pad, layer.k, x.device), layer.k)
+                            SPARSE_BWD_STATS["dgrad"] += 1
                         dx = hip.conv2d_ml_fwd_bf16(gp, wt, meta.level_hw, meta.N, k=layer.k, pad=layer.k - 1 - layer.pad,
-                                                    residual=other, out_dtype=x.dtype, out=dest, groups=G)
+                                                    residual=other, out_dtype=x.dtype, out=dest, groups=G, tile_flags=tf)
                 elif G > 1:
                     dx = torch.cat([hip.conv2d_ml_dgrad(g[:, gi * Kg:(gi + 1) * Kg].contiguous(),
                                                         hip.weight_flip_transpose(layer.w.t[gi * Kg:(gi + 1) * Kg], Kg, layer.k, layer.k, layer.cin),
@@ -539,10 +554,12 @@
                     dx = hip.conv2d_ml_dgrad(g, layer.wt(), meta.level_hw, meta.N, layer.k, layer.pad)
             if layer.use_bf16_wgrad():
                 gw = gp[:, :layer.cout] if (d16 and ctx.needs_input_grad[0] and gp is not g) else g
+                wb = gp_bits if (gp_bits is not None and gw.data_ptr() == gp_ready.data_ptr()) else None
+                SPARSE_BWD_STATS["wgrad"] += wb is not None
                 _wgrad_launch(lambda: hip.conv2d_wgrad_bf16(
                     x, gw, layer.w.g, hip.rowinfo_ml(meta.N, meta.level_hw, layer.pad, layer.k, x.device), layer.cin, layer.k, layer.k,
                     accumulate=True, db=layer.bias.g if (layer.bias is not None and not layer.bias_grad_from_gn()) else None, rowscale=wsc,
-                    groups=G, x_pitch=x.stride(0)), x, gw, key=layer)
+                    groups=G, x_pitch=x.stride(0), chunk_bits=wb), x, gw, wb, key=layer)
                 bias_done = True
             elif G > 1:
                 for gi in range(G):
```

Result: no change. 344.1 (-0.3%).
